# little-little-point-cloud-group/buildingSegment

Hardware: AMD Instinct MI355X
Metric: Mpoints/s segmented (kNN+normal+label) (higher is better)
Workload: dtype int32 coordinates / f64 normals; 1 GPU; urban_50m; points_per_gpu=50000000, k=16, max_nn=50, rg_mode=0, largest_plane=135921, seed_attempts=6951, fallback_queries=0, rg_rounds=25, validation_rejects=0, tie_rows=971975, parallelism=1 GPU, whole path

## Files before the change

### buildingsegment_amd/_lib.py

```python
from __future__ import annotations

import ctypes as C
import os

HERE = os.path.dirname(os.path.abspath(__file__))
LIB_PATH = os.environ.get("BS_LIB_PATH") or os.path.join(HERE, "libbuildingsegment_hip.so")

BS_OK = 0
STATUS = {0: "BS_OK", -1: "BS_ERR_INVALID", -2: "BS_ERR_RANGE", -3: "BS_ERR_NOMEM", -4: "BS_ERR_HIP",
          -5: "BS_ERR_NO_DEVICE", -6: "BS_ERR_INTERNAL", -7: "BS_ERR_UNCERTIFIED"}

EXPORTS = ["bs_api_version", "bs_sizeof_timings", "bs_strerror", "bs_params_default", "bs_create", "bs_destroy", "bs_last_error",
           "bs_set_stream", "bs_get_timings", "bs_knn_normals", "bs_knn_normals_halo", "bs_region_grow", "bs_segment",
           "bs_planes_free", "bs_plane_colors", "bs_knn_normals_dev", "bs_region_grow_dev",
           "bs_segment_dev", "bs_planes_fetch", "bs_shift_to_origin_dev", "bs_plane_colors_dev",
           "bs_selftest_center_div", "bs_selftest_forge_next", "bs_set_audit", "bs_selftest_grow_limits",
           "bs_get_grow_counters", "bs_ingest_dev", "bs_grid_dims", "bs_grid_picture", "bs_grid_picture_dev",
           "bs_cc_hook_dev", "bs_owner_fetch_dev", "bs_labels_from_owner_dev", "bs_remap_rows_dev",
           "bs_plane_seeds_dev", "bs_stream_sync", "bs_comm_rccl", "bs_comm_rccl_unique_id", "bs_comm_rccl_init",
           "bs_comm_rccl_destroy", "bs_comm_local_create", "bs_comm_local_destroy", "bs_segment_sharded",
           "bs_sharded_planes_fetch", "bs_footprints_dev", "bs_footprints", "bs_contours_free",
           "bs_contours_write_obj", "bs_segment_batch", "bs_segment_batch_dev", "bs_batch_planes_fetch",
           "bs_shift_tiles_to_origin_dev", "bs_tile_boxes_dev", "bs_grid_dims_batch", "bs_grid_picture_batch_dev",
           "bs_grid_picture_batch", "bs_footprints_batch_dev", "bs_footprints_batch", "bs_building_map_dev",
           "bs_building_map", "bs_buildings_free", "bs_assign_buildings_dev", "bs_assign_buildings",
           "bs_plane_buildings_dev", "bs_plane_buildings", "bs_buildings_write_obj", "bs_roof_homes", "bs_roofs_dev",
           "bs_roofs", "bs_roofs_free", "bs_roofs_write_obj"]


class Params(C.Structure):
    _fields_ = [("k", C.c_int32), ("max_nn", C.c_int32), ("radius", C.c_double),
                ("th_thickness", C.c_int32), ("th_point_count", C.c_int32), ("cos_th", C.c_double),
                ("cell_size", C.c_int32), ("rg_mode", C.c_int32)]


class Planes(C.Structure):
    _fields_ = [("n_planes", C.c_int32), ("id", C.POINTER(C.c_int32)), ("normal", C.POINTER(C.c_double)),
                ("center", C.POINTER(C.c_int32)), ("offset", C.POINTER(C.c_int64)),
                ("point_idx", C.POINTER(C.c_int32))]


class Timings(C.Structure):
    _fields_ = [("grid_ms", C.c_double), ("knn_ms", C.c_double), ("grow_ms", C.c_double),
                ("total_ms", C.c_double), ("largest_plane", C.c_int64), ("n_seed_attempts", C.c_int64),
                ("n_fallback_queries", C.c_int64), ("rg_rounds", C.c_int64), ("grow_kernel_ms", C.c_double),
                ("grow_kernel_launches", C.c_int64), ("grow_setup_ms", C.c_double),
                ("validation_rejects", C.c_int64), ("forged_seed", C.c_int64), ("forged_refused", C.c_int64),
                ("audit_attempts", C.c_int64), ("audit_mismatches", C.c_int64), ("audit_ms", C.c_double),
                ("tie_rows", C.c_int64), ("rej_v1_robbed", C.c_int64), ("rej_v1_tag", C.c_int64), ("rej_v1_dup", C.c_int64),
                ("rej_v3_state", C.c_int64), ("incons_seed", C.c_int64), ("incons_list", C.c_int64),
                ("incons_log", C.c_int64)]


class GrowLimits(C.Structure):
    _fields_ = [("max_waves", C.c_int64), ("pool_cap", C.c_int64), ("max_pending", C.c_int64), ("pstore_cap", C.c_int64),
                ("retry_max_list", C.c_int32), ("retry_big_round", C.c_int32), ("full_refresh", C.c_int32),
                ("reserved", C.c_int32)]


class GrowCounters(C.Structure):
    _fields_ = [(k, C.c_int64) for k in
                ("rounds", "rounds_capped", "rounds_big", "attempts_nomem", "waves_cut", "max_waves_end", "attempts_stolen",
                 "dropped_pend_count", "dropped_pend_store", "dropped_other", "full_refreshes", "pool_cap")]


API_VERSION = 5


class CommOps(C.Structure):
    _fields_ = [("handle", C.c_void_p), ("rank", C.c_int32), ("world", C.c_int32),
                ("all_reduce", C.c_void_p), ("all_gather", C.c_void_p), ("all_to_all_v", C.c_void_p)]


class ShardInfo(C.Structure):
    _fields_ = [("n_own", C.c_int64), ("n_local", C.c_int64), ("n_grow", C.c_int64), ("components", C.c_int64),
                ("planes_total", C.c_int64), ("cc_iterations", C.c_int32), ("halo_retries", C.c_int32),
                ("halo_mm", C.c_double), ("ms_partition", C.c_double), ("ms_halo", C.c_double), ("ms_knn", C.c_double),
                ("ms_components", C.c_double), ("ms_redistribute", C.c_double), ("ms_grow", C.c_double),
                ("ms_labels", C.c_double)]


class Contours(C.Structure):
    _fields_ = [("n_contours", C.c_int32), ("width", C.c_int32), ("height", C.c_int32),
                ("offset", C.POINTER(C.c_int64)), ("xy", C.POINTER(C.c_int32)), ("area", C.POINTER(C.c_double)),
                ("perimeter", C.POINTER(C.c_double))]


class FootprintInfo(C.Structure):
    _fields_ = [("ms_mask", C.c_double), ("ms_close", C.c_double), ("ms_label", C.c_double), ("ms_trace", C.c_double),
                ("ms_total", C.c_double), ("fg_pixels", C.c_int64), ("border_states", C.c_int64),
                ("components", C.c_int64), ("jump_rounds", C.c_int64)]


class Buildings(C.Structure):
    _fields_ = [("n_buildings", C.c_int32), ("width", C.c_int32), ("height", C.c_int32),
                ("start_xy", C.POINTER(C.c_int32)), ("bbox", C.POINTER(C.c_int32)), ("pixels", C.POINTER(C.c_int64)),
                ("fg_pixels", C.POINTER(C.c_int64)), ("n_points", C.POINTER(C.c_int64)),
                ("n_above", C.POINTER(C.c_int64)), ("z_min", C.POINTER(C.c_int32)), ("z_max", C.POINTER(C.c_int32)),
                ("z_sum", C.POINTER(C.c_int64)), ("ms_label_mask", C.c_double), ("ms_label_fill", C.c_double),
                ("ms_number", C.c_double), ("ms_map", C.c_double), ("ms_assign", C.c_double)]


class Roofs(C.Structure):
    _fields_ = [("n_planes", C.c_int32), ("width", C.c_int32), ("height", C.c_int32), ("fill_rounds", C.c_int32),
                ("seeded_pixels", C.c_int64), ("filled_pixels", C.c_int64), ("unroofed_pixels", C.c_int64),
                ("pixels", C.POINTER(C.c_int64)), ("seed_pixels", C.POINTER(C.c_int64)), ("bbox", C.POINTER(C.c_int32)),
                ("n_support", C.POINTER(C.c_int64)), ("z_min", C.POINTER(C.c_int32)), ("z_max", C.POINTER(C.c_int32)),
                ("z_sum", C.POINTER(C.c_int64)), ("ms_vote", C.c_double), ("ms_fill", C.c_double),
                ("ms_figures", C.c_double), ("ms_height", C.c_double)]


class BsError(RuntimeError):
    def __init__(self, status, detail=""):
        self.status = status
        super().__init__(f"{STATUS.get(status, status)}: {detail}")


_LIB = None


def load():
    global _LIB
    if _LIB is not None:
        return _LIB
    if not os.path.exists(LIB_PATH):
        raise ImportError(f"{LIB_PATH} is missing: build it with `python -m buildingsegment_amd.build` "
                          "(hipcc --offload-arch=gfx950); there is no CPU fallback")
    L = C.CDLL(LIB_PATH)
    L.bs_api_version.restype = C.c_int
    L.bs_sizeof_timings.restype = C.c_int64
    if L.bs_api_version() != API_VERSION or L.bs_sizeof_timings() != C.sizeof(Timings):
        raise ImportError(f"{LIB_PATH} is API version {L.bs_api_version()} (bs_timings: {L.bs_sizeof_timings()} bytes), this "
                          f"loader mirrors version {API_VERSION} ({C.sizeof(Timings)} bytes): rebuild the library")
    vp, ip, dp, lp = C.c_void_p, C.c_void_p, C.c_void_p, C.POINTER(C.c_int64)
    pp = C.POINTER(Params)
    L.bs_api_version.restype = C.c_int
    L.bs_strerror.restype = C.c_char_p
    L.bs_strerror.argtypes = [C.c_int]
    L.bs_params_default.argtypes = [pp]
    L.bs_create.argtypes = [C.c_int, C.POINTER(vp)]
    L.bs_destroy.argtypes = [vp]
    L.bs_destroy.restype = None
    L.bs_last_error.argtypes = [vp]
    L.bs_last_error.restype = C.c_char_p
    L.bs_set_stream.argtypes = [vp, vp]
    L.bs_get_timings.argtypes = [vp, C.POINTER(Timings)]
    L.bs_knn_normals.argtypes = [vp, ip, C.c_int64, pp, ip, dp]
    L.bs_knn_normals_halo.argtypes = [vp, ip, ip, C.c_int64, C.c_int64, pp, ip, dp, C.c_double, lp]
    L.bs_region_grow.argtypes = [vp, ip, dp, ip, C.c_int64, pp, ip, C.POINTER(Planes)]
    L.bs_segment.argtypes = [vp, ip, C.c_int64, pp, ip, dp, ip, C.POINTER(Planes)]
    L.bs_planes_free.argtypes = [C.POINTER(Planes)]
    L.bs_planes_free.restype = None
    L.bs_plane_colors.argtypes = [C.POINTER(Planes), ip, C.c_int64, vp]
    L.bs_knn_normals_dev.argtypes = [vp, ip, ip, C.c_int64, C.c_int64, C.c_int64, pp, ip, dp, C.c_double, lp]
    L.bs_region_grow_dev.argtypes = [vp, ip, dp, ip, C.c_int64, pp, ip]
    L.bs_segment_dev.argtypes = [vp, ip, C.c_int64, pp, ip, dp, ip]
    L.bs_planes_fetch.argtypes = [vp, C.POINTER(Planes)]
    L.bs_shift_to_origin_dev.argtypes = [vp, ip, C.c_int64, ip]
    L.bs_ingest_dev.argtypes = [vp, vp, C.c_int64, C.c_int32, C.c_int32, C.c_int32, C.c_int32, C.c_int32, C.c_double,
                                C.c_int32, ip, ip]
    L.bs_plane_colors_dev.argtypes = [vp, ip, C.c_int32, C.c_int64, vp]
    L.bs_selftest_forge_next.argtypes = [vp, C.c_int]
    L.bs_set_audit.argtypes = [vp, C.c_int]
    L.bs_selftest_grow_limits.argtypes = [vp, C.POINTER(GrowLimits)]
    L.bs_get_grow_counters.argtypes = [vp, C.POINTER(GrowCounters)]
    L.bs_selftest_center_div.argtypes = [vp, ip, vp, ip, C.c_int64]
    L.bs_grid_dims.argtypes = [ip, C.c_int32, ip, ip]
    L.bs_grid_picture.argtypes = [vp, ip, C.c_int64, ip, C.c_int32, C.c_int32, dp, dp]
    L.bs_grid_picture_dev.argtypes = [vp, ip, C.c_int64, ip, C.c_int32, C.c_int32, dp, dp]
    L.bs_cc_hook_dev.argtypes = [vp, ip, ip, C.c_int64, C.c_int32, ip, C.c_int64, lp]
    L.bs_owner_fetch_dev.argtypes = [vp, ip]
    L.bs_plane_seeds_dev.argtypes = [vp, ip, C.c_int64, C.POINTER(C.c_int32)]
    L.bs_stream_sync.argtypes = [vp]
    L.bs_labels_from_owner_dev.argtypes = [vp, ip, C.c_int64, ip, C.c_int32, ip]
    L.bs_remap_rows_dev.argtypes = [vp, ip, C.c_int64, C.c_int32, ip, C.c_int64, ip, C.POINTER(C.c_int32)]
    L.bs_comm_rccl.argtypes = [vp, C.c_int32, C.c_int32, C.POINTER(CommOps)]
    L.bs_comm_rccl_unique_id.argtypes = [C.c_char_p]
    L.bs_comm_rccl_init.argtypes = [vp, C.c_char_p, C.c_int32, C.c_int32, C.POINTER(vp)]
    L.bs_comm_rccl_destroy.argtypes = [vp]
    L.bs_comm_local_create.argtypes = [C.c_int32, C.POINTER(CommOps)]
    L.bs_comm_local_destroy.argtypes = [C.POINTER(CommOps)]
    L.bs_comm_local_destroy.restype = None
    L.bs_segment_sharded.argtypes = [vp, C.POINTER(CommOps), ip, ip, C.c_int64, C.c_int64, pp, C.c_double, ip,
                                     C.POINTER(ShardInfo)]
    L.bs_sharded_planes_fetch.argtypes = [vp, C.POINTER(Planes)]
    cp = C.POINTER(Contours)
    L.bs_footprints_dev.argtypes = [vp, vp, C.c_int32, C.c_int32, C.c_int32, C.c_int32, C.c_int32, vp, cp,
                                    C.POINTER(FootprintInfo)]
    L.bs_footprints.argtypes = [vp, vp, C.c_int32, C.c_int32, C.c_int32, C.c_int32, C.c_int32, vp, cp,
                                C.POINTER(FootprintInfo)]
    L.bs_contours_free.argtypes = [cp]
    L.bs_contours_free.restype = None
    L.bs_contours_write_obj.argtypes = [cp, C.c_char_p]
    L.bs_segment_batch.argtypes = [vp, ip, vp, C.c_int32, pp, ip, dp, ip, C.POINTER(Planes), ip]
    L.bs_segment_batch_dev.argtypes = [vp, ip, vp, C.c_int32, pp, ip, dp, ip]
    L.bs_batch_planes_fetch.argtypes = [vp, C.POINTER(Planes), ip]
    L.bs_shift_tiles_to_origin_dev.argtypes = [vp, ip, vp, C.c_int32, ip]
    L.bs_tile_boxes_dev.argtypes = [vp, ip, vp, C.c_int32, ip]
    L.bs_grid_dims_batch.argtypes = [ip, C.c_int32, C.c_int32, ip, ip, vp]
    L.bs_grid_picture_batch_dev.argtypes = [vp, ip, vp, C.c_int32, ip, C.c_int32, C.c_int32, dp, dp]
    L.bs_grid_picture_batch.argtypes = [vp, ip, vp, C.c_int32, ip, C.c_int32, C.c_int32, dp, dp]
    L.bs_footprints_batch_dev.argtypes = [vp, vp, ip, ip, C.c_int32, C.c_int32, C.c_int32, C.c_int32, vp, cp, ip,
                                          C.POINTER(FootprintInfo)]
    L.bs_footprints_batch.argtypes = [vp, vp, ip, ip, C.c_int32, C.c_int32, C.c_int32, C.c_int32, vp, cp, ip,
                                      C.POINTER(FootprintInfo)]
    bp = C.POINTER(Buildings)
    L.bs_building_map_dev.argtypes = [vp, vp, C.c_int32, C.c_int32, ip, bp]
    L.bs_building_map.argtypes = [vp, vp, C.c_int32, C.c_int32, ip, bp]
    L.bs_buildings_free.argtypes = [bp]
    L.bs_buildings_free.restype = None
    L.bs_assign_buildings_dev.argtypes = [vp, ip, C.c_int64, C.c_int32, C.c_double, ip, C.c_int32, C.c_int32, ip, bp]
    L.bs_assign_buildings.argtypes = [vp, ip, C.c_int64, C.c_int32, C.c_double, ip, C.c_int32, C.c_int32, ip, bp]
    L.bs_plane_buildings_dev.argtypes = [vp, ip, ip, C.c_int64, C.c_int32, C.c_int32, ip, vp, vp, vp]
    L.bs_plane_buildings.argtypes = [vp, ip, ip, C.c_int64, C.c_int32, C.c_int32, ip, vp, vp, vp]
    L.bs_buildings_write_obj.argtypes = [cp, bp, C.c_int32, ip, C.c_double, C.c_double, C.c_double, C.c_char_p]
    rp = C.POINTER(Roofs)
    L.bs_roof_homes.argtypes = [dp, ip, vp, vp, C.c_int32, C.c_double, ip]
    roofs_args = [vp, ip, C.c_int64, C.c_int32, C.c_double, ip, C.c_int32, C.c_int32, ip, C.c_int32, ip, dp, ip, C.c_int32,
                  ip, ip, ip, rp]
    L.bs_roofs_dev.argtypes = roofs_args
    L.bs_roofs.argtypes = roofs_args
    L.bs_roofs_free.argtypes = [rp]
    L.bs_roofs_free.restype = None
    L.bs_roofs_write_obj.argtypes = [ip, ip, C.c_int32, C.c_int32, rp, dp, ip, C.c_int32, ip, C.c_char_p]
    _LIB = L
    return L
```

### buildingsegment_amd/csrc/bs_common.h

```cpp
#pragma once

#include <hip/hip_runtime.h>
#include <stdint.h>

#include <string>
#include <vector>

#include "../../include/bs_api.h"

namespace bs {

struct DevBuf {
  void* p = nullptr;
  size_t cap = 0;
  hipError_t reserve(size_t bytes)
  {
    if (bytes <= cap)
      return hipSuccess;
    if (p)
      (void)hipFree(p);
    p = nullptr;
    cap = 0;
    size_t want = bytes + bytes / 8 + 256;
    hipError_t e = hipMalloc(&p, want);
    if (e == hipSuccess)
      cap = want;
    return e;
  }
  void release()
  {
    if (p)
      (void)hipFree(p);
    p = nullptr;
    cap = 0;
  }
  template <class T>
  T* as() const
  {
    return (T*)p;
  }
};

struct HostBuf {
  void* p = nullptr;
  size_t cap = 0;
  hipError_t reserve(size_t bytes)
  {
    if (bytes <= cap)
      return hipSuccess;
    if (p)
      (void)hipHostFree(p);
    p = nullptr;
    cap = 0;
    size_t want = bytes + bytes / 8 + 256;
    hipError_t e = hipHostMalloc(&p, want, hipHostMallocDefault);
    if (e == hipSuccess)
      cap = want;
    return e;
  }
  void release()
  {
    if (p)
      (void)hipHostFree(p);
    p = nullptr;
    cap = 0;
  }
  template <class T>
  T* as() const
  {
    return (T*)p;
  }
};

struct CellEntry {
  uint64_t key;
  int32_t start;
  int32_t end;
};

struct GridDev {
  int32_t mn[3];
  int32_t dim[3];
  int32_t cell;
  uint32_t hmask;
  const CellEntry* table;
  const int4* spts;
  const int32_t* slocal;
  int64_t n;
};

struct TileDesc {
  int32_t mn[3];
  int32_t dim[3];
};

struct TiledGridDev : GridDev {
  const TileDesc* tiles;
  const int32_t* tile_off;
  int32_t n_tiles;
  int32_t mbits;
};

enum { BT_OFF, BT_BLK, BT_MNMX, BT_DESC, BT_BASE, BT_RECS, BT_LIST, BT_COUNT };

__host__ __device__ inline int32_t tile_of(const int32_t* off, int32_t n_tiles, int64_t i)
{
  int32_t lo = 0, hi = n_tiles - 1;
  while (lo < hi) {
    const int32_t mid = (lo + hi + 1) >> 1;
    if (off[mid] <= i)
      lo = mid;
    else
      hi = mid - 1;
  }
  return lo;
}

__host__ __device__ inline uint64_t spread21(uint64_t v)
{
  v &= 0x1FFFFFull;
  v = (v | (v << 32)) & 0x1F00000000FFFFull;
  v = (v | (v << 16)) & 0x1F0000FF0000FFull;
  v = (v | (v << 8)) & 0x100F00F00F00F00Full;
  v = (v | (v << 4)) & 0x10C30C30C30C30C3ull;
  v = (v | (v << 2)) & 0x1249249249249249ull;
  return v;
}

__host__ __device__ inline uint64_t morton_cell(uint32_t cx, uint32_t cy, uint32_t cz)
{
  return spread21(cx) | (spread21(cy) << 1) | (spread21(cz) << 2);
}

__host__ __device__ inline double* pnorm_of(int32_t* npos, int64_t n, int K)
{
  return reinterpret_cast<double*>(npos + (((int64_t)n * K + 1) & ~(int64_t)1));
}

__host__ __device__ inline uint64_t pack_cell(uint32_t cx, uint32_t cy, uint32_t cz)
{
  return (uint64_t)cx | ((uint64_t)cy << 21) | ((uint64_t)cz << 42);
}

__host__ __device__ inline uint32_t hash_cell(uint64_t k)
{
  k *= 0x9E3779B97F4A7C15ull;
  return (uint32_t)(k >> 32) ^ (uint32_t)k;
}

__device__ inline int64_t xcd_logical_block()
{
  const int64_t b = blockIdx.x, per = gridDim.x >> 3;
  return (b & 7) * per + (b >> 3);
}
inline int xcd_grid(int64_t nblocks) { return (int)((nblocks + 7) & ~(int64_t)7); }

struct PlaneRec {
  double normal[3];
  int64_t list_off;
  int64_t list_n;
  int32_t center[3];
  int32_t id;
  int32_t seed;
  int32_t pad;
};

struct GrowStats {
  int32_t n_planes;
  int32_t error;
  int64_t list_used;
  int64_t seed_attempts;
  int64_t largest;
  int64_t steps;
};

}

struct bs_ctx {
  int device = 0;
  hipStream_t own_stream = nullptr;
  hipStream_t stream = nullptr;
  std::string err;
  bs_timings tm{};
  hipEvent_t ev[10] = {nullptr, nullptr, nullptr, nullptr, nullptr, nullptr, nullptr, nullptr, nullptr, nullptr};

  bs::DevBuf keys_in, keys_out, vals_in, vals_out, cub_tmp, uniq_keys, uniq_cnt, misc;
  bs::DevBuf table, spts, slocal;
  bs::DevBuf fb_list, d_xyz_h, d_neigh_h, d_normals_h, d_plane_h;
  bs::DevBuf seg_neigh, seg_normals;
  bs::DevBuf rg_list, rg_stack, rg_planes, rg_stats, rg_aux, rg_pstore, rg_rec, rg_radj, rg_roff, rg_geo, rg_gs, rg_disp;
  bs::HostBuf rg_hout;
  int64_t rg_n = 0;
  bool rg_valid = false;
  const int32_t* rg_omega = nullptr;
  const int32_t* rg_prio = nullptr;
  const int32_t* rg_seeds = nullptr;
  int32_t rg_nplanes = 0;
  int forge_mode = 0;
  int audit = 0;
  bs_grow_limits lim{0, 0, 0, 0, -1, -1, 0, 0};
  bs_grow_counters gc{};
  hipStream_t side = nullptr;
  hipEvent_t sev[2] = {nullptr, nullptr};
  bs::DevBuf rs_keys_in, rs_keys_out, rs_vals_in, rs_vals_out, rs_cnt, rs_img, rs_tmp;
  int64_t order_n = 0;
  const int32_t* order_xyz = nullptr;
  bs::DevBuf seg_npos;
  bs::DevBuf fp[24];
  bs::DevBuf bd[14];
  bs::DevBuf rf[16];
  bs::DevBuf sh[25];
  std::vector<int32_t> sh_seeds;
  int64_t sh_nloc = 0;
  bool sh_valid = false;
  const int32_t* npos_neigh = nullptr;
  const double* npos_normals = nullptr;
  int npos_k = 0;
  bs::DevBuf bt[bs::BT_COUNT];
  std::vector<int64_t> bt_off;
  bool bt_valid = false;
  bs::DevBuf tile_desc;
};

namespace bs {

int fail(bs_ctx* ctx, int status, const char* what, hipError_t e = hipSuccess);

#define BS_HIP(ctx, call)                                     \
  do {                                                        \
    hipError_t _e = (call);                                   \
    if (_e != hipSuccess)                                     \
      return bs::fail((ctx), BS_ERR_HIP, #call, _e);          \
  } while (0)

int build_grid(bs_ctx* ctx, const int32_t* d_xyz, const int32_t* d_gidx, int64_t n, double radius,
               int k, int cell_hint, GridDev* out);
int build_spatial_order(bs_ctx* ctx, const int32_t* d_xyz, int64_t n);
int bbox_dev(bs_ctx* ctx, const int32_t* d_xyz, int64_t n, int32_t bb[6]);
int tile_bbox_dev(bs_ctx* ctx, const int32_t* d_xyz, const int32_t* d_off, const std::vector<int64_t>& off,
                  int32_t* d_mnmx, std::vector<int32_t>& mnmx);
int build_grid_tiled(bs_ctx* ctx, const int32_t* d_xyz, const int32_t* d_off, const std::vector<int64_t>& off,
                     double radius, int k, int cell_hint, TiledGridDev* out);
int check_tiles(bs_ctx* ctx, const int64_t* off, int32_t n_tiles, int64_t min_pts, int64_t* total);
void launch_tile_shift(bs_ctx* ctx, int32_t* d_xyz, int64_t n, const int32_t* d_off, int32_t n_tiles,
                       const int32_t* d_mnmx);
int launch_knn_normals(bs_ctx* ctx, const GridDev& g, int64_t q_begin, int64_t q_end,
                       const bs_params& p, int32_t* d_neigh, double* d_normals, double cert_radius,
                       int64_t* n_uncertified, int32_t* d_npos = nullptr);
int launch_knn_normals_tiled(bs_ctx* ctx, const TiledGridDev& g, const bs_params& p, int32_t* d_neigh,
                             double* d_normals, int32_t* d_npos);
int region_grow_dev_impl(bs_ctx* ctx, const int32_t* d_xyz, const double* d_normals, const int32_t* d_neigh,
                         int64_t n, const bs_params* p, int32_t* d_plane_idx, bool trusted_neigh);
int check_params(bs_ctx* ctx, const bs_params* p, int64_t n);
int planes_to_host(bs_ctx* ctx, const PlaneRec* d_recs, const int32_t* d_list, int np, int64_t list_used,
                   bs_planes* out);
int launch_region_grow_seq(bs_ctx* ctx, const int32_t* d_xyz, const double* d_normals,
                           const int32_t* d_neigh, int64_t n, const bs_params& p,
                           int32_t* d_plane_idx);
int launch_region_grow_spec(bs_ctx* ctx, const int32_t* d_xyz, const double* d_normals,
                            const int32_t* d_neigh, int64_t n, const bs_params& p,
                            int32_t* d_plane_idx);

}
```

### buildingsegment_amd/csrc/bs_grow_spec.hip

```cpp
#include <hipcub/hipcub.hpp>

#include <algorithm>
#include <cstdio>
#include <cstdlib>
#include <type_traits>
#include <chrono>
#include <vector>

#include "bs_centerdiv.h"
#include "bs_common.h"

namespace bs {

namespace {

constexpr int32_t INF = 0x7fffffff;
constexpr int32_t LOWER_BIT = (int32_t)0x80000000;
constexpr int32_t POS_MASK = 0x7fffffff;
constexpr int MAX_WAVES = 1 << 18;
constexpr int MAX_PENDING = 32768;

enum : int32_t { ST_NONE = 0, ST_DONE = 1, ST_FAILED0 = 2, ST_NOMEM = 3, ST_WATCHDOG = 4, ST_STOLEN = 5 };

struct SpecArgs {
  const int32_t* xyz;
  const double* normals;
  const int32_t* neigh;
  int64_t n;
  int K;
  double th;
  double cos_th;
  int64_t th_count;
  int32_t F;
  int32_t pad;
};

struct PlaneOut {
  double normal[3];
  int64_t list_off;
  int64_t list_n;
  int64_t log_off;
  int64_t log_n;
  int64_t steps;
  int32_t center[3];
  int32_t seed;
  int32_t status;
  int32_t keep;
  int32_t consistent;
  int32_t pad;
  int32_t thief;
  int32_t seed_pos;
  int32_t v3ok;
  int32_t pad4;
  int64_t t_start, t_end;
  int32_t w;
  int32_t pad5;
};

struct KeepForHost {
  __device__ bool operator()(const PlaneOut& o) const { return o.status == ST_DONE || o.status == ST_NOMEM || o.status == ST_WATCHDOG; }
};

struct Pool {
  int32_t* base;
  unsigned long long* top;
  unsigned long long cap;
};

struct Slab {
  int64_t off;
  int32_t cap;
};

__device__ inline int ld_i32(const int32_t* p)
{
  return __hip_atomic_load(p, __ATOMIC_RELAXED, __HIP_MEMORY_SCOPE_AGENT);
}

__device__ inline unsigned long long ballot64(bool pred)
{
  return __builtin_amdgcn_ballot_w64(pred);
}

__device__ inline int readlane_i32(int v, int lane)
{
  return __builtin_amdgcn_readlane(v, __builtin_amdgcn_readfirstlane(lane));
}

__device__ inline double readlane_f64(double v, int lane)
{
  int lo = __double2loint(v), hi = __double2hiint(v);
  lo = readlane_i32(lo, lane);
  hi = readlane_i32(hi, lane);
  return __hiloint2double(hi, lo);
}

__device__ inline bool slab_ensure(const Pool& pool, Slab& s, int32_t used, int64_t need, int lane)
{
  if (need <= s.cap)
    return true;
  if (need > 0x7ffffff0ll)
    return false;
  int64_t ncap = (int64_t)s.cap * 2;
  if (ncap < need)
    ncap = need;
  if (ncap < 256)
    ncap = 256;
  if (ncap > 0x7ffffff0ll)
    ncap = 0x7ffffff0ll;
  ncap = (ncap + 3) & ~(int64_t)3;
  unsigned long long off = 0;
  if (lane == 0)
    off = atomicAdd(pool.top, (unsigned long long)ncap);
  off = ((unsigned long long)(uint32_t)readlane_i32((int)(off >> 32), 0) << 32) |
        (uint32_t)readlane_i32((int)(off & 0xffffffffu), 0);
  if (off + (unsigned long long)ncap > pool.cap)
    return false;
  for (int32_t t0 = 0; t0 < used; t0 += 64) {
    const int32_t t = t0 + lane;
    if (t < used)
      pool.base[off + t] = ld_i32(pool.base + s.off + t);
  }
  s.off = (int64_t)off;
  s.cap = (int32_t)ncap;
  return true;
}

constexpr int RW_PAD = 896;
constexpr int RW_WIN = 256 + 2 * RW_PAD;
constexpr int GW_PAD = 192;
constexpr int GW_WIN = 256 + 2 * GW_PAD;

__global__ __launch_bounds__(256) void static_mask_kernel(SpecArgs a, const int32_t* __restrict__ rows, int row_stride,
                                                          const int4* __restrict__ geo, uint32_t* __restrict__ hmask,
                                                          int32_t* __restrict__ rcnt, uint32_t* __restrict__ lmask)
{
  __shared__ int lcnt[RW_WIN];
  __shared__ int4 lgeo[GW_WIN * 3];
  const int64_t b0 = xcd_logical_block() * (int64_t)blockDim.x;
  const int64_t i = b0 + threadIdx.x;
  const int64_t w0 = b0 > RW_PAD ? b0 - RW_PAD : 0;
  const int64_t g0 = b0 > GW_PAD ? b0 - GW_PAD : 0;
  for (int d = threadIdx.x; d < RW_WIN; d += 256)
    lcnt[d] = 0;
  {
    const int64_t gend = (g0 + GW_WIN < a.n ? g0 + GW_WIN : a.n) - g0;
    const int4* src = geo + 3 * g0;
    for (int64_t t = threadIdx.x; t < 3 * gend; t += 256)
      lgeo[t] = src[t];
  }
  __syncthreads();
  if (i < a.n) {
    const int4* own = lgeo + 3 * (i - g0);
    const int4 s0 = own[0], s1 = own[1], s2 = own[2];
    const double cnx = __hiloint2double(s1.y, s1.x), cny = __hiloint2double(s1.w, s1.z),
                 cnz = __hiloint2double(s2.y, s2.x);
    const int ccx = s0.x, ccy = s0.y, ccz = s0.z;
    const int32_t* row = rows + i * row_stride;
    uint32_t m = 0, lm = 0;
    for (int t = 1; t < a.K; t++) {
      const int32_t c = row[t];
      if (c < 0)
        continue;
      const int64_t gd = (int64_t)c - g0;
      int4 q0, q1, q2;
      if (gd >= 0 && gd < GW_WIN) {
        q0 = lgeo[3 * gd];
        q1 = lgeo[3 * gd + 1];
        q2 = lgeo[3 * gd + 2];
      } else {
        const int4* rc = geo + 3 * (int64_t)c;
        q0 = rc[0];
        q1 = rc[1];
        q2 = rc[2];
      }
      const int dx = (int)((uint32_t)q0.x - (uint32_t)ccx);
      const int dy = (int)((uint32_t)q0.y - (uint32_t)ccy);
      const int dz = (int)((uint32_t)q0.z - (uint32_t)ccz);
      const double dist = __builtin_fabs((double)dx * cnx + (double)dy * cny + (double)dz * cnz);
      const double dt = cnx * __hiloint2double(q1.y, q1.x) + cny * __hiloint2double(q1.w, q1.z) +
                        cnz * __hiloint2double(q2.y, q2.x);
      if (dist <= a.th && dt >= a.cos_th) {
        m |= 1u << (t - 1);
        lm |= (s0.w < q0.w ? 1u : 0u) << (t - 1);
        const int64_t d = (int64_t)c - w0;
        if (d >= 0 && d < RW_WIN)
          atomicAdd(&lcnt[d], 1);
        else
          atomicAdd(&rcnt[c], 1);
      }
    }
    hmask[i] = m;
    lmask[i] = lm;
  }
  __syncthreads();
  for (int d = threadIdx.x; d < RW_WIN; d += 256) {
    const int v = lcnt[d];
    if (v)
      atomicAdd(&rcnt[w0 + d], v);
  }
}

__global__ __launch_bounds__(256) void rev_fill_kernel(const uint32_t* __restrict__ hmask, const int32_t* __restrict__ rows,
                                                       int row_stride, int64_t n, unsigned long long* __restrict__ rcur,
                                                       int32_t* __restrict__ radj, const uint32_t* __restrict__ lmask)
{
  __shared__ int lcnt[RW_WIN];
  __shared__ unsigned long long lbase[RW_WIN];
  const int64_t b0 = xcd_logical_block() * (int64_t)blockDim.x;
  const int64_t i = b0 + threadIdx.x;
  const int64_t w0 = b0 > RW_PAD ? b0 - RW_PAD : 0;
  for (int d = threadIdx.x; d < RW_WIN; d += 256)
    lcnt[d] = 0;
  __syncthreads();
  const uint32_t m0 = i < n ? hmask[i] : 0u;
  const uint32_t lm0 = i < n ? lmask[i] : 0u;
  const int32_t* row = rows + (i < n ? i : 0) * row_stride;
  for (uint32_t m = m0; m;) {
    const int t = __ffs(m) - 1;
    m &= m - 1;
    const int64_t d = (int64_t)row[t + 1] - w0;
    if (d >= 0 && d < RW_WIN)
      atomicAdd(&lcnt[d], 1);
  }
  __syncthreads();
  for (int d = threadIdx.x; d < RW_WIN; d += 256) {
    const int v = lcnt[d];
    if (v) {
      lbase[d] = atomicAdd(&rcur[w0 + d], (unsigned long long)v);
      lcnt[d] = 0;
    }
  }
  __syncthreads();
  for (uint32_t m = m0; m;) {
    const int t = __ffs(m) - 1;
    m &= m - 1;
    const int32_t c = row[t + 1];
    const int64_t d = (int64_t)c - w0;
    if (d >= 0 && d < RW_WIN)
      radj[lbase[d] + (unsigned)atomicAdd(&lcnt[d], 1)] = (int32_t)i | (((lm0 >> t) & 1u) ? LOWER_BIT : 0);
    else
      radj[atomicAdd(&rcur[c], 1ull)] = (int32_t)i | (((lm0 >> t) & 1u) ? LOWER_BIT : 0);
  }
}

constexpr int OWN_TRIP = 16;
constexpr int WL_CAP = 1024;
constexpr int WL_WAVE = 256;

__device__ __forceinline__ void wl_flush(const int* l_buf, int* l_base, int staged, int32_t* list, int* cnt)
{
  if (threadIdx.x == 0)
    *l_base = atomicAdd(cnt, staged);
  __syncthreads();
  const int b = *l_base;
  for (int i = threadIdx.x; i < staged; i += blockDim.x)
    list[b + i] = l_buf[i];
  __syncthreads();
}

__global__ __launch_bounds__(256) void wl_compact_kernel(uint8_t* bdirty, int nb, uint32_t* gflag, int32_t* list, int* cnt)
{
  __shared__ int l_buf[WL_CAP];
  __shared__ int l_base;
  __shared__ int wsum[4];
  int staged = 0;
  for (int j = 0; j < WL_CAP / 256; j++) {
    const int g = blockIdx.x * WL_CAP + j * 256 + threadIdx.x;
    bool add = false;
    if (g < nb && bdirty[g]) {
      bdirty[g] = 0;
      add = atomicExch(gflag + g, 1u) == 0u;
    }
    const unsigned long long am = ballot64(add);
    if ((threadIdx.x & 63) == 0)
      wsum[threadIdx.x >> 6] = __popcll(am);
    __syncthreads();
    int before = __popcll(am & ((1ull << (threadIdx.x & 63)) - 1ull)), total = 0;
    for (int w = 0; w < 4; w++) {
      before += w < (int)(threadIdx.x >> 6) ? wsum[w] : 0;
      total += wsum[w];
    }
    if (add)
      l_buf[staged + before] = g;
    staged += total;
    __syncthreads();
  }
  if (staged)
    wl_flush(l_buf, &l_base, staged, list, cnt);
}

__device__ __forceinline__ void wl_wave_flush(int* wbuf, int& staged, int32_t* list, int* cnt)
{
  const int lane = threadIdx.x & 63;
  __builtin_amdgcn_fence(__ATOMIC_RELEASE, "workgroup");
  __builtin_amdgcn_wave_barrier();
  int b = 0;
  if (lane == 0)
    b = atomicAdd(cnt, staged);
  b = __shfl(b, 0);
  for (int i = lane; i < staged; i += 64)
    list[b + i] = wbuf[i];
  __builtin_amdgcn_fence(__ATOMIC_ACQ_REL, "workgroup");
  __builtin_amdgcn_wave_barrier();
  staged = 0;
}

__device__ __forceinline__ void wl_add(bool want, int32_t g, uint32_t* gflag, int* wbuf, int& staged, int32_t* list, int* cnt)
{
  if (!ballot64(want))
    return;
  const bool added = want && atomicExch(gflag + g, 1u) == 0u;
  const unsigned long long am = ballot64(added);
  if (am == 0)
    return;
  if (added)
    wbuf[staged + __popcll(am & ((1ull << (threadIdx.x & 63)) - 1ull))] = g;
  staged += __popcll(am);
  if (staged > WL_WAVE - 64)
    wl_wave_flush(wbuf, staged, list, cnt);
}

struct PullEval {
  bool flip;
  bool walked;
  uint32_t m0;
};

__device__ __forceinline__ PullEval pull_eval(int64_t c, const uint32_t* __restrict__ hmask, const int32_t* __restrict__ prio,
                                              const uint8_t* __restrict__ ps, const int32_t* __restrict__ base,
                                              const int64_t* __restrict__ roff, const int32_t* __restrict__ radj,
                                              int32_t* __restrict__ omega, uint32_t* occ, int4* rec, int quads,
                                              const int32_t* __restrict__ minr)
{
  int32_t v = base[c];
  const int32_t mr = minr[c];
  const int64_t e0 = roff[c], e1 = roff[c + 1];
  const uint32_t m0 = hmask[c];
  const uint8_t psc = ps[c];
  const int32_t pc = prio[c];
  const uint32_t cbit = 1u << (c & 31);
  const uint32_t oword = __hip_atomic_load(occ + (c >> 5), __ATOMIC_RELAXED, __HIP_MEMORY_SCOPE_AGENT);
  const bool walk = v > mr;
  if (walk) {
    for (int64_t e = e0; e < e1; e += OWN_TRIP) {
      int32_t j[OWN_TRIP];
      uint32_t ow[OWN_TRIP];
      int32_t pj[OWN_TRIP];
#pragma unroll
      for (int i = 0; i < OWN_TRIP; i++)
        j[i] = radj[e + i < e1 ? e + i : e1 - 1] & POS_MASK;
#pragma unroll
      for (int i = 0; i < OWN_TRIP; i++)
        ow[i] = __hip_atomic_load(occ + (j[i] >> 5), __ATOMIC_RELAXED, __HIP_MEMORY_SCOPE_AGENT);
#pragma unroll
      for (int i = 0; i < OWN_TRIP; i++) {
        const bool o = ((ow[i] >> (j[i] & 31)) & 1u) != 0;
        pj[i] = prio[o ? (int64_t)j[i] : c];
        pj[i] = o ? pj[i] : INF;
      }
#pragma unroll
      for (int i = 0; i < OWN_TRIP; i++)
        v = pj[i] < v ? pj[i] : v;
    }
  }
  omega[c] = v;
  reinterpret_cast<int32_t*>(rec + c * quads)[3] = v;
  const bool want = m0 != 0 && !(psc & 1) && v >= pc;
  const bool have = (oword & cbit) != 0;
  if (want != have) {
    if (want)
      __hip_atomic_fetch_or(occ + (c >> 5), cbit, __ATOMIC_RELAXED, __HIP_MEMORY_SCOPE_AGENT);
    else
      __hip_atomic_fetch_and(occ + (c >> 5), ~cbit, __ATOMIC_RELAXED, __HIP_MEMORY_SCOPE_AGENT);
  }
  return {want != have, walk, m0};
}

__device__ __forceinline__ void pull_stats(int* dbg, bool dirty, bool walked)
{
  const int nd = __popcll(ballot64(dirty)), nw = __popcll(ballot64(walked));
  if ((threadIdx.x & 63) == 0 && nd) {
    atomicAdd(dbg + 1, nd);
    atomicAdd(dbg + 2, nw);
  }
}

__global__ void pull_pass_kernel(int64_t n, int K, int sub, const uint32_t* __restrict__ hmask,
                                 const int32_t* __restrict__ prio, const uint8_t* __restrict__ ps,
                                 const int32_t* __restrict__ base, const int64_t* __restrict__ roff,
                                 const int32_t* __restrict__ radj, int32_t* __restrict__ omega, uint32_t* occ,
                                 uint8_t* dirty_cur, uint8_t* dirty_next, uint8_t* bdirty_cur, uint8_t* bdirty_next,
                                 int4* rec, int quads, int* any, const int32_t* __restrict__ minr, const int* prev_any, int* dbg)
{
  if (prev_any && *prev_any == 0)
    return;
  __shared__ unsigned long long sub_mask;
  const int64_t nb256 = (n + 255) >> 8;
  const int64_t g0 = (int64_t)blockIdx.x * sub;
  if (threadIdx.x < 64) {
    const int64_t gidx = g0 + threadIdx.x;
    const bool d = (int)threadIdx.x < sub && gidx < nb256 && bdirty_cur[gidx] != 0;
    if (d)
      bdirty_cur[gidx] = 0;
    const unsigned long long m = ballot64(d);
    if (threadIdx.x == 0)
      sub_mask = m;
  }
  __syncthreads();
  unsigned long long gm = sub_mask;
  if (dbg && threadIdx.x == 0 && gm) {
    atomicAdd(dbg, __popcll(gm));
    atomicMax(dbg + 3, __popcll(gm));
  }
  bool flipped = false;
  while (gm) {
    const int t = __ffsll(gm) - 1;
    gm &= gm - 1;
    const int64_t c = ((g0 + t) << 8) + threadIdx.x;
    const bool d = c < n && dirty_cur[c] != 0;
    PullEval r = {false, false, 0u};
    if (d) {
      dirty_cur[c] = 0;
      r = pull_eval(c, hmask, prio, ps, base, roff, radj, omega, occ, rec, quads, minr);
    }
    if (dbg)
      pull_stats(dbg, d, r.walked);
    if (r.flip) {
      const int32_t* row = reinterpret_cast<const int32_t*>(rec + c * quads + 4);
      uint32_t m = r.m0;
      while (m) {
        const int b = __ffs(m) - 1;
        m &= m - 1;
        const int32_t q = row[b + 1];
        dirty_next[q] = 1;
        bdirty_next[q >> 8] = 1;
      }
      flipped = true;
    }
  }
  if (flipped)
    *any = 1;
}

__global__ __launch_bounds__(256) void pull_list_kernel(int64_t n, int K, const uint32_t* __restrict__ hmask,
                                                        const int32_t* __restrict__ prio, const uint8_t* __restrict__ ps,
                                                        const int32_t* __restrict__ base, const int64_t* __restrict__ roff,
                                                        const int32_t* __restrict__ radj, int32_t* __restrict__ omega,
                                                        uint32_t* occ, uint8_t* dirty_cur, uint8_t* dirty_next,
                                                        const int32_t* __restrict__ list_cur, int32_t* list_next,
                                                        uint32_t* gflag_cur, uint32_t* gflag_next, int* cnt, int s_cur,
                                                        int s_nxt, int s_clr, int4* rec, int quads, int* any,
                                                        const int32_t* __restrict__ minr, int* dbg)
{
  __shared__ int l_buf[4][WL_WAVE];
  int* const wbuf = l_buf[threadIdx.x >> 6];
  const int lane = threadIdx.x & 63;
  const int ncur = cnt[s_cur];
  if (blockIdx.x == 0 && threadIdx.x == 0) {
    cnt[s_clr] = 0;
    if (dbg && ncur) {
      dbg[0] = ncur;
      dbg[3] = (ncur + (int)gridDim.x - 1) / (int)gridDim.x;
    }
  }
  if (ncur == 0)
    return;
  int staged = 0;
  bool flipped = false;
  const int per = (ncur + (int)gridDim.x - 1) / (int)gridDim.x;
  const int i0 = blockIdx.x * per, i1 = min(ncur, i0 + per);
  if (i0 >= i1)
    return;
  int32_t g_next = list_cur[i0];
  for (int idx = i0; idx < i1; idx++) {
    const int32_t g = g_next;
    if (idx + 1 < i1)
      g_next = list_cur[idx + 1];
    const int64_t c = ((int64_t)g << 8) + threadIdx.x;
    if (threadIdx.x == 0)
      gflag_cur[g] = 0;
    const bool d = c < n && dirty_cur[c] != 0;
    PullEval r = {false, false, 0u};
    if (d) {
      dirty_cur[c] = 0;
      r = pull_eval(c, hmask, prio, ps, base, roff, radj, omega, occ, rec, quads, minr);
    }
    if (dbg)
      pull_stats(dbg, d, r.walked);
    if (!ballot64(r.flip))
      continue;
    flipped = flipped || r.flip;
    const int32_t* row = reinterpret_cast<const int32_t*>(rec + (d ? c : 0) * quads + 4);
    for (int b0 = 0; b0 + 1 < K; b0 += OWN_TRIP) {
      int32_t gq[OWN_TRIP];
      uint32_t fl[OWN_TRIP];
      bool rep[OWN_TRIP];
#pragma unroll
      for (int i = 0; i < OWN_TRIP; i++) {
        const int b = b0 + i;
        gq[i] = -1;
        if (r.flip && b + 1 < K && ((r.m0 >> b) & 1u)) {
          const int32_t q = row[b + 1];
          dirty_next[q] = 1;
          gq[i] = q >> 8;
        }
      }
#pragma unroll
      for (int i = 0; i < OWN_TRIP; i++) {
        const int32_t left = __shfl_up(gq[i], 1);
        rep[i] = gq[i] >= 0 && (lane == 0 || left != gq[i]) && (i == 0 || gq[i - 1] != gq[i]);
        fl[i] = __hip_atomic_load(gflag_next + (rep[i] ? gq[i] : g), __ATOMIC_RELAXED, __HIP_MEMORY_SCOPE_AGENT);
      }
#pragma unroll
      for (int i = 0; i < OWN_TRIP; i++)
        wl_add(rep[i] && fl[i] == 0u, gq[i], gflag_next, wbuf, staged, list_next, cnt + s_nxt);
    }
  }
  if (staged)
    wl_wave_flush(wbuf, staged, list_next, cnt + s_nxt);
  if (flipped)
    *any = 1;
}

__global__ void decide_init_kernel(const uint32_t* __restrict__ hmask, int64_t n, uint8_t* __restrict__ st,
                                   uint8_t* __restrict__ bund)
{
  const int64_t c = blockIdx.x * (int64_t)blockDim.x + threadIdx.x;
  const bool maker = c < n && hmask[c] != 0;
  if (c < n)
    st[c] = maker ? 0 : 2;
  const int anym = __syncthreads_or(maker);
  if (threadIdx.x == 0)
    bund[blockIdx.x] = anym ? 1 : 0;
}

__global__ void decide_pass_kernel(int64_t n, int sub, const int32_t* __restrict__ prio,
                                   const int64_t* __restrict__ roff, const int32_t* __restrict__ radj, uint8_t* st,
                                   uint8_t* bund, int* any, const int* prev_any)
{
  if (prev_any && *prev_any == 0)
    return;
  __shared__ unsigned long long sub_mask;
  __shared__ int left[64];
  const int64_t nb256 = (n + 255) >> 8;
  const int64_t g0 = (int64_t)blockIdx.x * sub;
  if (threadIdx.x < 64) {
    const int64_t gidx = g0 + threadIdx.x;
    const bool d = (int)threadIdx.x < sub && gidx < nb256 && bund[gidx] != 0;
    left[threadIdx.x] = 0;
    const unsigned long long m = ballot64(d);
    if (threadIdx.x == 0)
      sub_mask = m;
  }
  __syncthreads();
  unsigned long long gm = sub_mask;
  bool undecided_left = false;
  while (gm) {
    const int t = __ffsll(gm) - 1;
    gm &= gm - 1;
    const int64_t c = ((g0 + t) << 8) + threadIdx.x;
    bool mine_left = false;
    if (c < n && __hip_atomic_load(st + c, __ATOMIC_RELAXED, __HIP_MEMORY_SCOPE_AGENT) == 0) {
      bool lower_occ = false, lower_und = false;
      const int64_t e1 = roff[c + 1];
      for (int64_t e = roff[c]; e < e1; e += 4) {
        int32_t rj[4];
        uint8_t sj[4];
#pragma unroll
        for (int q = 0; q < 4; q++)
          rj[q] = e + q < e1 ? radj[e + q] : 0;
#pragma unroll
        for (int q = 0; q < 4; q++)
          sj[q] = rj[q] < 0 ? __hip_atomic_load(st + (rj[q] & POS_MASK), __ATOMIC_RELAXED, __HIP_MEMORY_SCOPE_AGENT) : (uint8_t)2;
#pragma unroll
        for (int q = 0; q < 4; q++) {
          lower_occ = lower_occ || sj[q] == 1;
          lower_und = lower_und || sj[q] == 0;
        }
      }
      if (lower_occ)
        __hip_atomic_store(st + c, (uint8_t)2, __ATOMIC_RELAXED, __HIP_MEMORY_SCOPE_AGENT);
      else if (!lower_und)
        __hip_atomic_store(st + c, (uint8_t)1, __ATOMIC_RELAXED, __HIP_MEMORY_SCOPE_AGENT);
      else
        mine_left = true;
    }
    if (mine_left)
      left[t] = 1;
    undecided_left = undecided_left || mine_left;
  }
  __syncthreads();
  if (threadIdx.x < 64 && (int)threadIdx.x < sub && g0 + threadIdx.x < nb256)
    bund[g0 + threadIdx.x] = left[threadIdx.x] ? 1 : 0;
  if (undecided_left)
    *any = 1;
}

__global__ void decide_finish_kernel(int64_t n, const int32_t* __restrict__ prio, const int64_t* __restrict__ roff,
                                     const int32_t* __restrict__ radj, const uint8_t* __restrict__ st,
                                     int32_t* __restrict__ omega, uint32_t* __restrict__ occ, int4* rec, int quads,
                                     int32_t* __restrict__ minr)
{
  const int64_t c = blockIdx.x * (int64_t)blockDim.x + threadIdx.x;
  bool oc = false;
  if (c < n) {
    int32_t v = INF, vall = INF;
    const int64_t e1 = roff[c + 1];
    for (int64_t e = roff[c]; e < e1; e++) {
      const int32_t j = radj[e] & POS_MASK;
      const int32_t pj = prio[j];
      vall = pj < vall ? pj : vall;
      if (st[j] == 1)
        v = pj < v ? pj : v;
    }
    minr[c] = vall;
    omega[c] = v;
    reinterpret_cast<int32_t*>(rec + c * quads)[3] = v;
    oc = st[c] == 1;
  }
  const unsigned long long m = ballot64(oc);
  const int lane = threadIdx.x & 63;
  const int64_t w0 = (c - lane) >> 5;
  if (lane == 0 && (c - lane) < n)
    occ[w0] = (uint32_t)m;
  if (lane == 32 && (c - lane + 32) < n)
    occ[w0 + 1] = (uint32_t)(m >> 32);
}

__global__ void verify_fixpoint_kernel(int64_t n, const uint32_t* __restrict__ hmask, const int32_t* __restrict__ prio,
                                       const uint8_t* __restrict__ ps,
                                       const int32_t* __restrict__ base, const int64_t* __restrict__ roff,
                                       const int32_t* __restrict__ radj, const int32_t* __restrict__ omega,
                                       const uint32_t* __restrict__ occ, int* nbad)
{
  const int64_t c = blockIdx.x * (int64_t)blockDim.x + threadIdx.x;
  if (c >= n)
    return;
  int32_t v = base[c];
  for (int64_t e = roff[c]; e < roff[c + 1]; e++) {
    const int32_t j = radj[e] & POS_MASK;
    const bool oj = hmask[j] != 0 && !(ps[j] & 1) && omega[j] >= prio[j];
    if (oj && prio[j] < v)
      v = prio[j];
  }
  const bool oc = hmask[c] != 0 && !(ps[c] & 1) && omega[c] >= prio[c];
  if (v != omega[c] || (oc ? 1u : 0u) != ((occ[c >> 5] >> (c & 31)) & 1u))
    atomicAdd(nbad, 1);
}

__global__ void seed_flags_kernel(const uint32_t* __restrict__ hmask, int64_t n, int K, uint8_t* __restrict__ ps)
{
  const int64_t i = blockIdx.x * (int64_t)blockDim.x + threadIdx.x;
  const uint32_t full = (K - 1 >= 32) ? 0xffffffffu : ((1u << (K - 1)) - 1u);
  if (i < n)
    ps[i] = hmask[i] == full ? 0 : 2;
}

__global__ void cand_flag_kernel(const int4* __restrict__ rec, int quads, int K,
                                 int64_t n, int32_t F, const int32_t* __restrict__ prio, const uint8_t* __restrict__ ps,
                                 int all_seeds, const int32_t* __restrict__ omega, int32_t* min_idx,
                                 unsigned long long* __restrict__ cand_out, int32_t* cand_count, uint8_t* __restrict__ bcand,
                                 int sub)
{
  __shared__ unsigned long long sub_mask;
  const int64_t nb256 = (n + 255) >> 8;
  const int64_t g0 = (int64_t)blockIdx.x * sub;
  if (threadIdx.x < 64) {
    const int64_t gidx = g0 + threadIdx.x;
    const bool live = (int)threadIdx.x < sub && gidx < nb256 && bcand[gidx] != 0;
    const unsigned long long m = ballot64(live);
    if (threadIdx.x == 0)
      sub_mask = m;
  }
  __syncthreads();
  unsigned long long gm = sub_mask;
  while (gm) {
    const int t = __ffsll(gm) - 1;
    gm &= gm - 1;
    const int64_t i = ((g0 + t) << 8) + threadIdx.x;
    bool c = false, alive = false;
    const uint8_t f = i < n ? ps[i] : (uint8_t)2;
    int32_t pi = 0;
    if (!(f & 2)) {
      pi = prio[i];
      const int32_t oi = omega[i];
      alive = !(oi < F);
      if (pi >= F && oi >= pi && (all_seeds || !(f & 1))) {
        c = true;
        const int32_t* row = reinterpret_cast<const int32_t*>(rec + i * quads + 4);
        for (int u = 1; u < K; u += OWN_TRIP) {
          int32_t nb[OWN_TRIP];
          int32_t ov[OWN_TRIP];
#pragma unroll
          for (int q = 0; q < OWN_TRIP; q++)
            nb[q] = row[u + q < K ? u + q : K - 1];
#pragma unroll
          for (int q = 0; q < OWN_TRIP; q++)
            ov[q] = omega[nb[q]];
#pragma unroll
          for (int q = 0; q < OWN_TRIP; q++)
            c = c && ov[q] >= pi;
        }
      }
    }
    const int any_alive = __syncthreads_or(alive);
    if (threadIdx.x == 0 && !any_alive)
      bcand[g0 + t] = 0;
    if (c && min_idx)
      atomicMin(min_idx, pi);
    if (c && cand_out)
      cand_out[atomicAdd(cand_count, 1)] = ((unsigned long long)(uint32_t)pi << 32) | (uint32_t)i;
  }
}

template <int KC>
struct RecLayout {
  static constexpr int QUADS = 4 + KC / 4;
};

__device__ inline int32_t* rec_tag(int4* rec, int quads, int64_t i)
{
  return reinterpret_cast<int32_t*>(rec + i * quads + 2) + 2;
}

__global__ void invert_order_kernel(const int32_t* __restrict__ order, int64_t n, int32_t* __restrict__ pos)
{
  const int64_t s = blockIdx.x * (int64_t)blockDim.x + threadIdx.x;
  if (s < n)
    pos[order[s]] = (int32_t)s;
}

template <int KC>
__global__ __launch_bounds__(256) void build_records_kernel(SpecArgs a, const int32_t* __restrict__ order, const int32_t* __restrict__ pos,
                                     const int32_t* __restrict__ npos, int4* __restrict__ rec, int32_t* __restrict__ prio,
                                     int4* __restrict__ geo, const int4* __restrict__ spts, const double* __restrict__ pnorm)
{
  constexpr int Q = RecLayout<KC>::QUADS;
  __shared__ int4 srec[256 * Q];
  __shared__ int4 sgeo[256 * 3];
  const int64_t b0 = blockIdx.x * (int64_t)blockDim.x;
  const int64_t s = b0 + threadIdx.x;
  if (s < a.n) {
  int64_t i;
  int px, py, pz;
  if (spts) {
    const int4 p = spts[s];
    px = p.x;
    py = p.y;
    pz = p.z;
    i = p.w;
  } else {
    i = order ? order[s] : s;
    px = a.xyz[3 * i];
    py = a.xyz[3 * i + 1];
    pz = a.xyz[3 * i + 2];
  }
  int4* r = srec + threadIdx.x * Q;
  const double* nsrc = pnorm ? pnorm + 3 * s : a.normals + 3 * i;
  const double nx = nsrc[0], ny = nsrc[1], nz = nsrc[2];
  r[0] = make_int4(px, py, pz, INF);
  r[1] = make_int4(__double2loint(nx), __double2hiint(nx), __double2loint(ny), __double2hiint(ny));
  r[2] = make_int4(__double2loint(nz), __double2hiint(nz), INF, 0);
  r[3] = make_int4(0, 0, 0, 0);
  sgeo[3 * threadIdx.x] = make_int4(px, py, pz, (int32_t)i);
  sgeo[3 * threadIdx.x + 1] = r[1];
  sgeo[3 * threadIdx.x + 2] = r[2];
  prio[s] = (int32_t)i;
  int row[KC];
#pragma unroll
  for (int j = 0; j < KC; j++) {
    int v = 0;
    if (j < a.K) {
      if (npos) {
        v = npos[s * a.K + j];
      } else {
        v = a.neigh[i * a.K + j];
        v = pos ? pos[v] : v;
      }
    }
    row[j] = v;
  }
  if (!npos) {
#pragma unroll
    for (int j = 2; j < KC; j++) {
      bool rep = false;
#pragma unroll
      for (int t = 1; t < j; t++)
        rep = rep || (j < a.K && row[t] == row[j]);
      row[j] = rep ? -1 : row[j];
    }
  }
#pragma unroll
  for (int j = 0; j < KC; j += 4)
    r[4 + j / 4] = make_int4(row[j], row[j + 1], row[j + 2], row[j + 3]);
  }
  __syncthreads();
  const int64_t nv = a.n - b0 < 256 ? a.n - b0 : 256;
  int4* rout = rec + b0 * Q;
  for (int t = threadIdx.x; t < nv * Q; t += 256)
    rout[t] = srec[t];
  int4* gout = geo + 3 * b0;
  for (int t = threadIdx.x; t < nv * 3; t += 256)
    gout[t] = sgeo[t];
}

__global__ void refresh_records_kernel(const int32_t* __restrict__ omega, int4* __restrict__ rec, int quads, int64_t n)
{
  const int64_t i = blockIdx.x * (int64_t)blockDim.x + threadIdx.x;
  if (i >= n)
    return;
  reinterpret_cast<int32_t*>(rec + i * quads)[3] = omega[i];
  *rec_tag(rec, quads, i) = INF;
}

__device__ __forceinline__ void plane_state_lanes(int lane, double Sx, double Sy, double Sz, uint32_t Cx, uint32_t Cy, uint32_t Cz,
                                                  uint32_t n, double& cnx, double& cny, double& cnz, int& ccx, int& ccy, int& ccz)
{
  const double nrm = __builtin_sqrt((Sx * Sx) + (Sy * Sy) + (Sz * Sz));
  const double Sv = lane == 0 ? Sx : (lane == 1 ? Sy : Sz);
  const double qn = Sv / nrm;
  const CenterDiv cd = center_div_prepare(n);
  const int32_t Cv = lane == 0 ? (int32_t)Cx : (lane == 1 ? (int32_t)Cy : (int32_t)Cz);
  const int32_t qc = center_div(Cv, cd);
  cnx = readlane_f64(qn, 0);
  cny = readlane_f64(qn, 1);
  cnz = readlane_f64(qn, 2);
  ccx = readlane_i32(qc, 0);
  ccy = readlane_i32(qc, 1);
  ccz = readlane_i32(qc, 2);
}

constexpr int LDS_STACK = 256;
constexpr int LDS_REFILL = 128;
constexpr int MAX_RETRY_LONG = 3;
constexpr int MAX_RETRY = 12;
constexpr int RETRY_MAX_LIST = 16384;

template <int KC>
__global__ __launch_bounds__(64) void grow_spec_kernel(SpecArgs a, const unsigned long long* __restrict__ cand, int ncand,
                                                       int4* rec, int32_t* dead, Pool pool,
                                                       PlaneOut* __restrict__ out, int64_t step_cap, int retry_max_list,
                                                       const uint32_t* __restrict__ order)
{
  __shared__ __attribute__((aligned(16))) int lds_stack[LDS_STACK * KC];
  constexpr int Q = RecLayout<KC>::QUADS;
  constexpr int NG = 64 / KC;
  if ((int)blockIdx.x >= ncand)
    return;
  const int w = order ? (int)(order[blockIdx.x] & (MAX_WAVES - 1)) : (int)blockIdx.x;
  const int lane = threadIdx.x;
  const int g = lane / KC, j = lane % KC;
  const unsigned long long gmask0 = (KC == 32) ? 0xffffffffull : 0xffffull;
  const int K = a.K, nc = K - 1;
  const bool act = j < nc;
  const int64_t t_start = (int64_t)wall_clock64();
  const int32_t seed = (int32_t)(cand[w] >> 32);
  const int32_t seed_s = (int32_t)(uint32_t)cand[w];
  Slab list = {0, 0}, stack = {0, 0}, log = {0, 0};
  int long_tries = 0;
  int ln = 1, sp = 0, lds_lo = 0, logn = 0;
  uint32_t iters = 0;
  const uint32_t iter_cap = step_cap > 0xFFFFFFF0ll ? 0xFFFFFFF0u : (uint32_t)step_cap;
  int status = ST_DONE;
  bool pendv = false;
  const int32_t* vptr = dead;
  bool need_state = false;
  const int4* srec = rec + (int64_t)seed_s * Q;
  const int4 s0 = srec[0], s1 = srec[1], s2 = srec[2];
  double cnx, cny, cnz, Sx, Sy, Sz;
  int ccx, ccy, ccz;
  uint32_t Cx, Cy, Cz;
  unsigned long long d_am = 0;
  double d_mx = 0, d_my = 0, d_mz = 0;
  int d_px = 0, d_py = 0, d_pz = 0;
  auto update_state = [&]() {
    unsigned long long mm = d_am;
    while (mm) {
      const int l = __ffsll(mm) - 1;
      mm &= mm - 1;
      Sx += readlane_f64(d_mx, l);
      Sy += readlane_f64(d_my, l);
      Sz += readlane_f64(d_mz, l);
      Cx += (uint32_t)readlane_i32(d_px, l);
      Cy += (uint32_t)readlane_i32(d_py, l);
      Cz += (uint32_t)readlane_i32(d_pz, l);
    }
    plane_state_lanes(lane, Sx, Sy, Sz, Cx, Cy, Cz, (uint32_t)ln, cnx, cny, cnz, ccx, ccy, ccz);
    need_state = false;
  };
  const bool have_mem = slab_ensure(pool, list, 0, 256, lane) && slab_ensure(pool, stack, 0, 32 * (int64_t)KC, lane) &&
                        slab_ensure(pool, log, 0, 256, lane);
  for (int attempt = 0;; attempt++) {
  status = ST_DONE;
  pendv = false;
  ln = 1;
  sp = 0;
  lds_lo = 0;
  logn = 0;
  cnx = __hiloint2double(s1.y, s1.x);
  cny = __hiloint2double(s1.w, s1.z);
  cnz = __hiloint2double(s2.y, s2.x);
  ccx = s0.x;
  ccy = s0.y;
  ccz = s0.z;
  Sx = 0.0 + cnx;
  Sy = 0.0 + cny;
  Sz = 0.0 + cnz;
  Cx = (uint32_t)ccx;
  Cy = (uint32_t)ccy;
  Cz = (uint32_t)ccz;
  if (!have_mem) {
    status = ST_NOMEM;
  } else {
    if (lane == 0)
      pool.base[list.off] = seed_s;
    if (lane < KC)
      lds_stack[lane] = reinterpret_cast<const int32_t*>(srec + 4)[lane];
    sp = 1;
    bool depth0 = true;
    int stack_entries = stack.cap / KC;
    need_state = false;
    __builtin_amdgcn_s_waitcnt(0x0F70);
    auto step = [&](auto mode) -> int {
      if (__builtin_expect(sp == 0, 0))
        return 2;
      if (__builtin_expect(++iters > iter_cap, 0)) {
        status = ST_WATCHDOG;
        return 2;
      }
      const int e = sp - 1 - g;
      const bool valid = e >= 0;
      const int ngv = (sp < NG) ? sp : NG;
      const int need_lo = (sp - NG > 0) ? sp - NG : 0;
      if (__builtin_expect(need_lo < lds_lo, 0)) {
        const int new_lo = lds_lo > LDS_REFILL ? lds_lo - LDS_REFILL : 0;
        const int nw = (lds_lo - new_lo) * KC;
        for (int t = lane; t < nw; t += 64) {
          const int ee = new_lo + t / KC;
          lds_stack[(ee & (LDS_STACK - 1)) * KC + (t % KC)] = ld_i32(pool.base + stack.off + (int64_t)new_lo * KC + t);
        }
        lds_lo = new_lo;
      }
      int cand_id = 0;
      if (valid && act)
        cand_id = lds_stack[(e & (LDS_STACK - 1)) * KC + j + 1];
      const bool live = cand_id >= 0;
      cand_id = live ? cand_id : 0;
      const int killed = ld_i32(dead + seed);
      const int vt = ld_i32(pendv ? vptr : dead + seed);
      int own = 0, tg = INF, px = 0, py = 0, pz = 0;
      double mx = 0, my = 0, mz = 0;
      int row[KC];
      {
        const int4* r = rec + (int64_t)cand_id * Q;
        const int4 q0 = r[0], q1 = r[1], q2 = r[2];
        tg = ld_i32(reinterpret_cast<const int32_t*>(r + 2) + 2);
        px = q0.x;
        py = q0.y;
        pz = q0.z;
        own = q0.w;
        mx = __hiloint2double(q1.y, q1.x);
        my = __hiloint2double(q1.w, q1.z);
        mz = __hiloint2double(q2.y, q2.x);
#pragma unroll
        for (int t = 0; t < KC; t += 4) {
          const int4 v = r[4 + t / 4];
          row[t] = v.x;
          row[t + 1] = v.y;
          row[t + 2] = v.z;
          row[t + 3] = v.w;
        }
      }
      if constexpr (decltype(mode)::value == 1)
        update_state();
      else if constexpr (decltype(mode)::value == 2) {
        if (__builtin_expect(need_state, 1))
          update_state();
      }
      bool geo = false;
      if (valid && act && live && tg != seed) {
        const int dx = (int)((uint32_t)px - (uint32_t)ccx);
        const int dy = (int)((uint32_t)py - (uint32_t)ccy);
        const int dz = (int)((uint32_t)pz - (uint32_t)ccz);
        const double dist = __builtin_fabs((double)dx * cnx + (double)dy * cny + (double)dz * cnz);
        const double dt = cnx * mx + cny * my + cnz * mz;
        geo = dist <= a.th && dt >= a.cos_th;
      }
      const bool lost = pendv && vt != seed;
      pendv = false;
      if (__builtin_expect(killed || ballot64(lost), 0)) {
        status = ST_STOLEN;
        return 2;
      }
      bool assume = geo && own < seed && !(own < a.F);
      const bool contender = geo && !(own < seed);
      const unsigned long long cm = ballot64(contender);
      unsigned long long am = 0;
      int gstar = -1;
      bool ok = false;
      if (__builtin_expect(cm != 0, 1)) {
        const int g1 = (__ffsll(cm) - 1) / KC;
        const unsigned long long gm1 = gmask0 << (g1 * KC);
        const unsigned long long earlier = ballot64(contender && tg < seed);
        if (__builtin_expect((earlier & gm1) == 0, 1)) {
          ok = contender && g == g1;
          if (ok) {
            int32_t* tp = rec_tag(rec, Q, cand_id);
            __hip_atomic_fetch_min(tp, seed, __ATOMIC_RELAXED, __HIP_MEMORY_SCOPE_AGENT);
            if (tg != INF)
              __hip_atomic_store(dead + tg, seed + 1, __ATOMIC_RELAXED, __HIP_MEMORY_SCOPE_AGENT);
            vptr = tp;
            pendv = true;
          }
          am = cm & gm1;
          gstar = g1;
        } else {
        for (int gg = g1; gg < ngv; gg++) {
          const unsigned long long gm = gmask0 << (gg * KC);
          if (cm & gm) {
            if (g == gg && contender) {
              int32_t* tp = rec_tag(rec, Q, cand_id);
              int cur_tag = tg;
              bool mine = false;
              for (int tries = 0; tries < 8 && !ok && !assume && !mine; tries++) {
                if (cur_tag < seed) {
                  if (ld_i32(dead + cur_tag) < 0) {
                    const int old = atomicCAS(tp, cur_tag, seed);
                    if (old == cur_tag)
                      ok = true;
                    else
                      cur_tag = old;
                  } else {
                    assume = true;
                  }
                } else if (cur_tag == seed) {
                  mine = true;
                } else {
                  const int old = atomicMin(tp, seed);
                  if (old > seed) {
                    if (old != INF)
                      __hip_atomic_store(dead + old, seed + 1, __ATOMIC_RELAXED, __HIP_MEMORY_SCOPE_AGENT);
                    ok = true;
                  } else if (old == seed) {
                    mine = true;
                  } else {
                    cur_tag = old;
                  }
                }
              }
              if (!ok && !mine)
                assume = true;
            }
            am = ballot64(ok);
            if (am) {
              gstar = gg;
              break;
            }
          }
        }
        }
      }
      const int last = gstar >= 0 ? gstar : ngv - 1;
      const unsigned long long lm = ballot64(assume && g <= last);
      const int lcnt = __popcll(lm);
      if (__builtin_expect(lcnt != 0, 0)) {
        if (!slab_ensure(pool, log, logn, logn + lcnt, lane)) {
          status = ST_NOMEM;
          return 2;
        }
        if (assume && g <= last)
          pool.base[log.off + logn + __popcll(lm & ((1ull << lane) - 1ull))] = cand_id;
        logn += lcnt;
      }
      const int cnt = __popcll(am);
      if (__builtin_expect(depth0 && cnt < nc, 0)) {
        status = ST_FAILED0;
        return 2;
      }
      depth0 = false;
      sp -= last + 1;
      if (sp < lds_lo)
        lds_lo = sp;
      if (__builtin_expect(gstar < 0, 0))
        return 0;
      if (__builtin_expect(ln + cnt > list.cap || sp + cnt > stack_entries, 0)) {
        if (!slab_ensure(pool, list, ln, ln + cnt, lane) ||
            !slab_ensure(pool, stack, sp > 0x7ffffff0 / KC ? 0x7ffffff0 : sp * KC, (int64_t)(sp + cnt) * KC, lane)) {
          status = ST_NOMEM;
          return 2;
        }
        stack_entries = stack.cap / KC;
      }
      const int rank = __popcll(am & ((1ull << lane) - 1ull));
      if (ok)
        pool.base[list.off + ln + rank] = cand_id;
      d_am = am;
      d_mx = mx;
      d_my = my;
      d_mz = mz;
      d_px = px;
      d_py = py;
      d_pz = pz;
      ln += cnt;
      need_state = true;
      if (ok) {
        const int pe = sp + (cnt - 1 - rank);
        int4* lslot = reinterpret_cast<int4*>(lds_stack + (pe & (LDS_STACK - 1)) * KC);
        row[0] = cand_id;
#pragma unroll
        for (int t = 0; t < KC; t += 4)
          lslot[t / 4] = make_int4(row[t], row[t + 1], row[t + 2], row[t + 3]);
        if (rank > 0) {
          int4* slot = reinterpret_cast<int4*>(pool.base + stack.off + (int64_t)pe * KC);
#pragma unroll
          for (int t = 0; t < KC; t += 4)
            slot[t / 4] = make_int4(row[t], row[t + 1], row[t + 2], row[t + 3]);
        }
      }
      sp += cnt;
      if (__builtin_expect(sp - lds_lo > LDS_STACK, 0))
        lds_lo = sp - LDS_STACK;
      return 1;
    };
    if constexpr (KC == 32) {
      int r = step(std::integral_constant<int, 0>{});
      while (r == 0)
        r = step(std::integral_constant<int, 0>{});
      while (r == 1) {
        r = step(std::integral_constant<int, 1>{});
        while (r == 0)
          r = step(std::integral_constant<int, 0>{});
      }
    } else {
      while (step(std::integral_constant<int, 2>{}) != 2) {
      }
    }
  }
  if (need_state)
    update_state();
  if (status == ST_DONE) {
    const bool lost = pendv && ld_i32(vptr) != seed;
    if (ballot64(lost))
      status = ST_STOLEN;
  }
  bool seed_taken = false;
  if (status == ST_STOLEN) {
    const int t0 = ld_i32(rec_tag(rec, Q, seed_s));
    seed_taken = t0 < seed && ld_i32(dead + t0) >= 0;
  }
  if (status != ST_STOLEN || seed_taken || attempt >= MAX_RETRY || ln > retry_max_list ||
      (ln > RETRY_MAX_LIST && ++long_tries > MAX_RETRY_LONG))
    break;
  for (int t = 1 + lane; t < ln; t += 64)
    atomicCAS(rec_tag(rec, Q, ld_i32(pool.base + list.off + t)), seed, INF);
  __hip_atomic_store(dead + seed, 0, __ATOMIC_RELAXED, __HIP_MEMORY_SCOPE_AGENT);
  }
  if (lane == 0 && status == ST_STOLEN) {
    const int t = ld_i32(dead + seed);
    __hip_atomic_store(dead + seed, t > 0 ? -t : (t == 0 ? -0x40000000 : t), __ATOMIC_RELAXED, __HIP_MEMORY_SCOPE_AGENT);
  }
  if (lane == 0) {
    PlaneOut o;
    o.normal[0] = cnx;
    o.normal[1] = cny;
    o.normal[2] = cnz;
    o.center[0] = ccx;
    o.center[1] = ccy;
    o.center[2] = ccz;
    o.list_off = list.off;
    o.list_n = ln;
    o.log_off = log.off;
    o.log_n = logn;
    o.steps = iters;
    o.seed = seed;
    o.status = status;
    o.keep = (status == ST_DONE && ln > a.th_count) ? 1 : 0;
    o.consistent = 0;
    o.pad = 0;
    const int dflag = ld_i32(dead + seed);
    o.thief = (dflag < 0 ? -dflag : dflag) - 1;
    o.seed_pos = seed_s;
    o.v3ok = 1;
    o.pad4 = 0;
    o.t_start = t_start;
    o.t_end = (int64_t)wall_clock64();
    o.w = w;
    o.pad5 = (int32_t)((__builtin_amdgcn_s_getreg((15 << 11) | (0 << 6) | 4) & 0xffff) |
                       ((__builtin_amdgcn_s_getreg((3 << 11) | (0 << 6) | 20) & 0xf) << 16));
    out[w] = o;
  }
}

constexpr int LBUF = 256;
#ifdef BS_PROBE
__device__ unsigned long long g_prof2[32];
#define PROBE(i)                    \
  do {                              \
    const long long _t = clock64(); \
    pacc[i] += _t - tlast;          \
    tlast = _t;                     \
  } while (0)
#else
#define PROBE(i) \
  do {           \
  } while (0)
#endif

typedef int v4i __attribute__((ext_vector_type(4)));

#ifdef BS_PROBE
__device__ unsigned long long g_exit2[16];
#define EXIT_COUNT(i) (nexit[i]++)
#else
#define EXIT_COUNT(i) \
  do {                \
  } while (0)
#endif
constexpr int LOGB = 128;

template <int KC>
__global__ __launch_bounds__(64) void grow_spec2_kernel(SpecArgs a, const unsigned long long* __restrict__ cand, int ncand,
                                                        int4* rec, int32_t* dead, Pool pool,
                                                        PlaneOut* __restrict__ out, int64_t step_cap, int retry_max_list,
                                                        const uint32_t* __restrict__ order)
{
  static_assert(KC == 16, "k > 16 runs on grow_spec_kernel");
  __shared__ int logbuf[LOGB];
  __shared__ __attribute__((aligned(16))) int lds_stack[LDS_STACK * KC];
  __shared__ int lbuf[LBUF];
  constexpr int Q = RecLayout<KC>::QUADS;
  constexpr int NG = 64 / KC;
  constexpr int CH = KC / 4;
  if ((int)blockIdx.x >= ncand)
    return;
  const int w = order ? (int)(order[blockIdx.x] & (MAX_WAVES - 1)) : (int)blockIdx.x;
  const int lane = threadIdx.x;
  const int g = lane / KC, j = lane % KC;
  const unsigned long long gmask0 = 0xffffull;
  const int K = a.K, nc = K - 1;
  const bool act = j < nc;
  const int64_t t_start = (int64_t)wall_clock64();
  const int32_t seed = (int32_t)(cand[w] >> 32);
  const int32_t seed_s = (int32_t)(uint32_t)cand[w];
  Slab list = {0, 0}, stack = {0, 0}, log = {0, 0};
  int long_tries = 0;
  int ln = 1, lflushed = 0, sp = 0, lds_lo = 0, logn = 0;
  int lgflushed = 0;
  uint32_t iters = 0;
  const uint32_t iter_cap = step_cap > 0xFFFFFFF0ll ? 0xFFFFFFF0u : (uint32_t)step_cap;
  int status = ST_DONE;
  bool pendv = false;
  const int32_t* vptr = dead;
  bool need_state = false;
  const int4* srec = rec + (int64_t)seed_s * Q;
  const int4 s0 = srec[0], s1 = srec[1], s2 = srec[2];
  double cnx, cny, cnz, Sx, Sy, Sz;
  int ccx, ccy, ccz;
  uint32_t Cx, Cy, Cz;
  unsigned long long d_am = 0;
  double d_mx = 0, d_my = 0, d_mz = 0;
  int d_px = 0, d_py = 0, d_pz = 0;
  const bool have_mem = slab_ensure(pool, list, 0, 256, lane) && slab_ensure(pool, stack, 0, 32 * (int64_t)KC, lane) &&
                        slab_ensure(pool, log, 0, 256, lane);
  auto flush_list = [&](int upto) -> bool {
    if (upto <= lflushed)
      return true;
    if (!slab_ensure(pool, list, lflushed, upto, lane))
      return false;
    for (int t0 = lflushed; t0 < upto; t0 += 64) {
      const int t = t0 + lane;
      if (t < upto)
        pool.base[list.off + t] = lbuf[t & (LBUF - 1)];
    }
    lflushed = upto;
    return true;
  };
  auto flush_log = [&](int upto) -> bool {
    if (upto <= lgflushed)
      return true;
    if (!slab_ensure(pool, log, lgflushed, upto, lane))
      return false;
    for (int t0 = lgflushed; t0 < upto; t0 += 64) {
      const int t = t0 + lane;
      if (t < upto)
        pool.base[log.off + t] = logbuf[t & (LOGB - 1)];
    }
    lgflushed = upto;
    return true;
  };
  for (int attempt = 0;; attempt++) {
    status = ST_DONE;
    pendv = false;
    ln = 1;
    lflushed = 0;
    sp = 0;
    lds_lo = 0;
    logn = 0;
    lgflushed = 0;
    cnx = __hiloint2double(s1.y, s1.x);
    cny = __hiloint2double(s1.w, s1.z);
    cnz = __hiloint2double(s2.y, s2.x);
    ccx = s0.x;
    ccy = s0.y;
    ccz = s0.z;
    Sx = 0.0 + cnx;
    Sy = 0.0 + cny;
    Sz = 0.0 + cnz;
    Cx = (uint32_t)ccx;
    Cy = (uint32_t)ccy;
    Cz = (uint32_t)ccz;
    need_state = false;
    if (!have_mem) {
      status = ST_NOMEM;
    } else {
      if (lane == 0)
        lbuf[0] = seed_s;
      if (lane < KC)
        lds_stack[lane] = reinterpret_cast<const int32_t*>(srec + 4)[lane];
      sp = 1;
      bool depth0 = true;
      __builtin_amdgcn_s_waitcnt(0x0F70);
#ifdef BS_PROBE
      long long pacc[12] = {0};
      long long ncalls = 0, nexp = 0;
      long long tlast = clock64();
      long long nexit[11] = {0};
#endif
      struct Ev {
        int cand_id, px, py, pz, own, tg;
        double mx, my, mz;
        bool geo, valid;
        int ngv;
        int killed_v, vt;
        bool lost_any;
        v4i rows[CH];
      };
      auto eval = [&](Ev& E) {
        E.ngv = (sp < NG) ? sp : NG;
        const int e = sp - 1 - g;
        E.valid = e >= 0;
        {
          const int v = lds_stack[(e & (LDS_STACK - 1)) * KC + ((j + 1) & (KC - 1))];
          E.valid = E.valid && v >= 0;
          E.cand_id = (E.valid && act) ? v : 0;
        }
        v4i q0, q1, q2;
        {
          const int32_t* kp = dead + seed;
          const int32_t* vp = pendv ? vptr : dead + seed;
          const int4* r = rec + (int64_t)E.cand_id * Q;
          asm volatile("global_load_dwordx4 %0, %5, off\n\t"
                       "global_load_dwordx4 %1, %5, off offset:16\n\t"
                       "global_load_dwordx4 %2, %5, off offset:32 sc1\n\t"
                       "global_load_dword %3, %6, off sc1\n\t"
                       "global_load_dword %4, %7, off sc1"
                       : "=&v"(q0), "=&v"(q1), "=&v"(q2), "=&v"(E.killed_v), "=&v"(E.vt)
                       : "v"(r), "v"(kp), "v"(vp)
                       : "memory");
#pragma unroll
          for (int t = 0; t < CH; t++) {
            const int4* rp = r + 4 + t;
            asm volatile("global_load_dwordx4 %0, %1, off" : "=&v"(E.rows[t]) : "v"(rp) : "memory");
          }
        }
        PROBE(0);
        if (__builtin_expect(need_state, 1)) {
          unsigned long long mm = d_am;
          while (mm) {
            const int l = __ffsll(mm) - 1;
            mm &= mm - 1;
            Sx += readlane_f64(d_mx, l);
            Sy += readlane_f64(d_my, l);
            Sz += readlane_f64(d_mz, l);
            Cx += (uint32_t)readlane_i32(d_px, l);
            Cy += (uint32_t)readlane_i32(d_py, l);
            Cz += (uint32_t)readlane_i32(d_pz, l);
          }
          plane_state_lanes(lane, Sx, Sy, Sz, Cx, Cy, Cz, (uint32_t)ln, cnx, cny, cnz, ccx, ccy, ccz);
          need_state = false;
        }
        PROBE(1);
        asm volatile("s_waitcnt vmcnt(6)" : "+v"(q0), "+v"(q1), "+v"(q2)::"memory");
        PROBE(2);
        E.px = q0.x;
        E.py = q0.y;
        E.pz = q0.z;
        E.own = q0.w;
        E.tg = q2.z;
        E.mx = __hiloint2double(q1.y, q1.x);
        E.my = __hiloint2double(q1.w, q1.z);
        E.mz = __hiloint2double(q2.y, q2.x);
        {
          const int dx = (int)((uint32_t)E.px - (uint32_t)ccx);
          const int dy = (int)((uint32_t)E.py - (uint32_t)ccy);
          const int dz = (int)((uint32_t)E.pz - (uint32_t)ccz);
          const double dist = __builtin_fabs((double)dx * cnx + (double)dy * cny + (double)dz * cnz);
          const double dt = cnx * E.mx + cny * E.my + cnz * E.mz;
          const bool okd = dist <= a.th, okn = dt >= a.cos_th;
          E.geo = E.valid & act & (E.tg != seed) & okd & okn;
        }
      };
      auto rows_wait = [&](Ev& E) {
        asm volatile("s_waitcnt vmcnt(0)"
                     : "+v"(E.rows[0]), "+v"(E.rows[1]), "+v"(E.rows[2]), "+v"(E.rows[3]), "+v"(E.killed_v), "+v"(E.vt)::"memory");
        const bool lost = pendv && E.vt != seed;
        E.lost_any = __builtin_amdgcn_readfirstlane(E.killed_v) != 0 || ballot64(lost) != 0;
      };
      auto expand = [&](const Ev& E, bool ok, unsigned long long am, int gstar, int cnt) {
        const int rank = __popcll(am & ((1ull << lane) - 1ull));
        if (ok)
          lbuf[(ln + rank) & (LBUF - 1)] = E.cand_id;
        d_am = am;
        d_mx = E.mx;
        d_my = E.my;
        d_mz = E.mz;
        d_px = E.px;
        d_py = E.py;
        d_pz = E.pz;
        ln += cnt;
        need_state = true;
        PROBE(7);
        if (ok) {
          const int pe = sp + (cnt - 1 - rank);
          v4i* lslot = reinterpret_cast<v4i*>(lds_stack + (pe & (LDS_STACK - 1)) * KC);
#pragma unroll
          for (int t = 0; t < CH; t++) {
            v4i v = E.rows[t];
            if (t == 0)
              v.x = E.cand_id;
            lslot[t] = v;
          }
        }
        (void)gstar;
        sp += cnt;
      };
      auto step_complete = [&]() -> int {
        if (__builtin_expect(sp == 0, 0))
          return 2;
        EXIT_COUNT(10);
        if (__builtin_expect(++iters > iter_cap, 0)) {
          status = ST_WATCHDOG;
          return 2;
        }
        const int need_lo = (sp - NG > 0) ? sp - NG : 0;
        if (__builtin_expect(need_lo < lds_lo, 0)) {
          const int new_lo = lds_lo > LDS_REFILL ? lds_lo - LDS_REFILL : 0;
          const int nw = (lds_lo - new_lo) * KC;
          for (int t0 = 0; t0 < nw; t0 += 64) {
            const int t = t0 + lane;
            const int ee = new_lo + t / KC;
            if (t < nw)
              lds_stack[(ee & (LDS_STACK - 1)) * KC + (t % KC)] = ld_i32(pool.base + stack.off + (int64_t)new_lo * KC + t);
          }
          lds_lo = new_lo;
        }
        Ev E;
        eval(E);
        rows_wait(E);
        pendv = false;
        if (__builtin_expect(E.lost_any, 0)) {
          status = ST_STOLEN;
          return 2;
        }
        bool assume = E.geo && E.own < seed && !(E.own < a.F);
        const bool contender = E.geo && !(E.own < seed);
        const unsigned long long cm = ballot64(contender);
        unsigned long long am = 0;
        int gstar = -1;
        bool ok = false;
        const int cand_id = E.cand_id, tg = E.tg, ngv = E.ngv;
        if (cm != 0) {
          const int g1 = (__ffsll(cm) - 1) / KC;
          const unsigned long long gm1 = gmask0 << (g1 * KC);
          const unsigned long long earlier = ballot64(contender && tg < seed);
          if ((earlier & gm1) == 0) {
            ok = contender && g == g1;
            if (ok) {
              int32_t* tp = rec_tag(rec, Q, cand_id);
              __hip_atomic_fetch_min(tp, seed, __ATOMIC_RELAXED, __HIP_MEMORY_SCOPE_AGENT);
              if (tg != INF)
                __hip_atomic_store(dead + tg, seed + 1, __ATOMIC_RELAXED, __HIP_MEMORY_SCOPE_AGENT);
              vptr = tp;
              pendv = true;
            }
            am = cm & gm1;
            gstar = g1;
          } else {
            for (int gg = g1; gg < ngv; gg++) {
              const unsigned long long gm = gmask0 << (gg * KC);
              if (cm & gm) {
                if (g == gg && contender) {
                  int32_t* tp = rec_tag(rec, Q, cand_id);
                  int cur_tag = tg;
                  bool mine = false;
                  for (int tries = 0; tries < 8 && !ok && !assume && !mine; tries++) {
                    if (cur_tag < seed) {
                      if (ld_i32(dead + cur_tag) < 0) {
                        const int old = atomicCAS(tp, cur_tag, seed);
                        if (old == cur_tag)
                          ok = true;
                        else
                          cur_tag = old;
                      } else {
                        assume = true;
                      }
                    } else if (cur_tag == seed) {
                      mine = true;
                    } else {
                      const int old = atomicMin(tp, seed);
                      if (old > seed) {
                        if (old != INF)
                          __hip_atomic_store(dead + old, seed + 1, __ATOMIC_RELAXED, __HIP_MEMORY_SCOPE_AGENT);
                        ok = true;
                      } else if (old == seed) {
                        mine = true;
                      } else {
                        cur_tag = old;
                      }
                    }
                  }
                  if (!ok && !mine)
                    assume = true;
                }
                am = ballot64(ok);
                if (am) {
                  gstar = gg;
                  break;
                }
              }
            }
          }
        }
        const int last = gstar >= 0 ? gstar : ngv - 1;
        const unsigned long long lm = ballot64(assume && g <= last);
        if (lm != 0) {
          const int lcnt = __popcll(lm);
          if (logn + lcnt - lgflushed > LOGB && !flush_log(logn)) {
            status = ST_NOMEM;
            return 2;
          }
          if (assume && g <= last)
            logbuf[(logn + __popcll(lm & ((1ull << lane) - 1ull))) & (LOGB - 1)] = cand_id;
          logn += lcnt;
        }
        const int cnt = __popcll(am);
        if (depth0 && cnt < nc) {
          status = ST_FAILED0;
          return 2;
        }
        depth0 = false;
        sp -= last + 1;
        if (gstar < 0)
          return 0;
        if (ln + cnt - lflushed > LBUF) {
          if (!flush_list(ln)) {
            status = ST_NOMEM;
            return 2;
          }
        }
        if (sp + cnt - lds_lo > LDS_STACK) {
          const int upto = lds_lo + LDS_STACK / 2;
          if (!slab_ensure(pool, stack, lds_lo > 0x7ffffff0 / KC ? 0x7ffffff0 : lds_lo * KC, (int64_t)upto * KC, lane)) {
            status = ST_NOMEM;
            return 2;
          }
          for (int t0 = 0; t0 < (LDS_STACK / 2) * KC; t0 += 64) {
            const int t = t0 + lane;
            const int ee = lds_lo + t / KC;
            pool.base[stack.off + (int64_t)lds_lo * KC + t] = lds_stack[(ee & (LDS_STACK - 1)) * KC + (t % KC)];
          }
          lds_lo = upto;
        }
        expand(E, ok, am, gstar, cnt);
        return 0;
      };
      auto uniform_state = [&]() {
        sp = __builtin_amdgcn_readfirstlane(sp);
        ln = __builtin_amdgcn_readfirstlane(ln);
        lds_lo = __builtin_amdgcn_readfirstlane(lds_lo);
        lflushed = __builtin_amdgcn_readfirstlane(lflushed);
        logn = __builtin_amdgcn_readfirstlane(logn);
        iters = (uint32_t)__builtin_amdgcn_readfirstlane((int)iters);
        status = __builtin_amdgcn_readfirstlane(status);
        d_am = ((unsigned long long)(uint32_t)__builtin_amdgcn_readfirstlane((int)(d_am >> 32)) << 32) |
               (uint32_t)__builtin_amdgcn_readfirstlane((int)(uint32_t)d_am);
      };
      for (;;) {
        const int r = __builtin_amdgcn_readfirstlane(step_complete());
        uniform_state();
        if (r == 2)
          break;
        bool leave = false;
        __builtin_amdgcn_s_waitcnt(0x0F70);
        for (;;) {
          if (__builtin_expect(sp == 0, 0)) {
            EXIT_COUNT(0);
            leave = true;
            break;
          }
          PROBE(9);
#ifdef BS_PROBE
          ncalls++;
#endif
          if (__builtin_expect(iters >= iter_cap, 0)) {
            EXIT_COUNT(1);
            break;
          }
          if (__builtin_expect(((sp - NG > 0) ? sp - NG : 0) < lds_lo, 0)) {
            EXIT_COUNT(2);
            break;
          }
          Ev E;
          eval(E);
          const bool assume = E.geo && E.own < seed && !(E.own < a.F);
          const bool contender = E.geo && !(E.own < seed);
          const unsigned long long cm = ballot64(contender);
          PROBE(3);
          int gstar = -1, cnt = 0;
          unsigned long long am = 0, lm = 0;
          bool slow = false;
          if (__builtin_expect(cm != 0, 1)) {
            gstar = (__ffsll(cm) - 1) / KC;
            const unsigned long long gm1 = gmask0 << (gstar * KC);
            am = cm & gm1;
            cnt = __popcll(am);
            lm = ballot64(assume && g <= gstar);
            slow = (ballot64(contender && E.tg < seed) & gm1) != 0 || ln + cnt - lflushed > LBUF ||
                   sp - (gstar + 1) + cnt - lds_lo > LDS_STACK;
          } else {
            lm = ballot64(assume);
          }
          slow = slow || logn + __popcll(lm) - lgflushed > LOGB;
          rows_wait(E);
          if (__builtin_expect(E.lost_any, 0)) {
            EXIT_COUNT(3);
            pendv = false;
            status = ST_STOLEN;
            leave = true;
            break;
          }
          if (__builtin_expect(slow, 0)) {
#ifdef BS_PROBE
            const unsigned long long gmp = gstar >= 0 ? gmask0 << (gstar * KC) : 0;
            if ((ballot64(contender && E.tg < seed) & gmp) != 0)
              EXIT_COUNT(4);
            else if (ln + cnt - lflushed > LBUF)
              EXIT_COUNT(6);
            else if (gstar >= 0 && sp - (gstar + 1) + cnt - lds_lo > LDS_STACK)
              EXIT_COUNT(7);
            else
              EXIT_COUNT(8);
#endif
            break;
          }
          EXIT_COUNT(9);
          iters++;
          pendv = false;
          if (lm != 0) {
            if (assume && (gstar < 0 || g <= gstar))
              logbuf[(logn + __popcll(lm & ((1ull << lane) - 1ull))) & (LOGB - 1)] = E.cand_id;
            logn += __popcll(lm);
          }
          const bool ok = contender && g == gstar;
          if (ok) {
            int32_t* tp = rec_tag(rec, Q, E.cand_id);
            asm volatile("global_atomic_smin %0, %1, off" ::"v"(tp), "v"(seed) : "memory");
            if (E.tg != INF) {
              int32_t* dp = dead + E.tg;
              const int thief = seed + 1;
              asm volatile("global_store_dword %0, %1, off sc1" ::"v"(dp), "v"(thief) : "memory");
            }
            vptr = tp;
            pendv = true;
          }
          PROBE(4);
          sp -= (gstar >= 0 ? gstar : E.ngv - 1) + 1;
          PROBE(5);
          if (gstar >= 0) {
#ifdef BS_PROBE
            nexp++;
#endif
            PROBE(6);
            expand(E, ok, am, gstar, cnt);
            PROBE(8);
          }
        }
        if (leave)
          break;
      }
#ifdef BS_PROBE
      if (lane == 0 && ln > 20000) {
        for (int i = 0; i < 10; i++)
          atomicAdd(&g_prof2[i], (unsigned long long)pacc[i]);
        atomicAdd(&g_prof2[10], (unsigned long long)ncalls);
        atomicAdd(&g_prof2[11], (unsigned long long)nexp);
      }
      if (lane == 0)
        for (int i = 0; i < 11; i++)
          if (nexit[i])
            atomicAdd(&g_exit2[i], (unsigned long long)nexit[i]);
#endif
    }
    if (need_state) {
      unsigned long long mm = d_am;
      while (mm) {
        const int l = __ffsll(mm) - 1;
        mm &= mm - 1;
        Sx += readlane_f64(d_mx, l);
        Sy += readlane_f64(d_my, l);
        Sz += readlane_f64(d_mz, l);
        Cx += (uint32_t)readlane_i32(d_px, l);
        Cy += (uint32_t)readlane_i32(d_py, l);
        Cz += (uint32_t)readlane_i32(d_pz, l);
      }
      plane_state_lanes(lane, Sx, Sy, Sz, Cx, Cy, Cz, (uint32_t)ln, cnx, cny, cnz, ccx, ccy, ccz);
      need_state = false;
    }
    if (have_mem && status != ST_NOMEM && !flush_list(ln))
      status = ST_NOMEM;
    if (have_mem && status != ST_NOMEM && !flush_log(logn))
      status = ST_NOMEM;
    if (status == ST_DONE) {
      const bool lost = pendv && ld_i32(vptr) != seed;
      if (ballot64(lost))
        status = ST_STOLEN;
    }
    bool seed_taken = false;
    if (status == ST_STOLEN) {
      const int t0 = __builtin_amdgcn_readfirstlane(ld_i32(rec_tag(rec, Q, seed_s)));
      seed_taken = t0 < seed && __builtin_amdgcn_readfirstlane(ld_i32(dead + (t0 < seed ? t0 : seed))) >= 0;
    }
    if (status != ST_STOLEN || seed_taken || attempt >= MAX_RETRY || ln > retry_max_list ||
        (ln > RETRY_MAX_LIST && ++long_tries > MAX_RETRY_LONG))
      break;
    for (int t0 = 1; t0 < ln; t0 += 64) {
      const int t = t0 + lane;
      if (t < ln)
        atomicCAS(rec_tag(rec, Q, ld_i32(pool.base + list.off + t)), seed, INF);
    }
    __hip_atomic_store(dead + seed, 0, __ATOMIC_RELAXED, __HIP_MEMORY_SCOPE_AGENT);
  }
  if (lane == 0 && status == ST_STOLEN) {
    const int t = ld_i32(dead + seed);
    __hip_atomic_store(dead + seed, t > 0 ? -t : (t == 0 ? -0x40000000 : t), __ATOMIC_RELAXED, __HIP_MEMORY_SCOPE_AGENT);
  }
  if (lane == 0) {
    PlaneOut o;
    o.normal[0] = cnx;
    o.normal[1] = cny;
    o.normal[2] = cnz;
    o.center[0] = ccx;
    o.center[1] = ccy;
    o.center[2] = ccz;
    o.list_off = list.off;
    o.list_n = ln;
    o.log_off = log.off;
    o.log_n = logn;
    o.steps = iters;
    o.seed = seed;
    o.status = status;
    o.keep = (status == ST_DONE && ln > a.th_count) ? 1 : 0;
    o.consistent = 0;
    o.pad = 0;
    const int dflag = ld_i32(dead + seed);
    o.thief = (dflag < 0 ? -dflag : dflag) - 1;
    o.seed_pos = seed_s;
    o.v3ok = 1;
    o.pad4 = 0;
    o.t_start = t_start;
    o.t_end = (int64_t)wall_clock64();
    o.w = w;
    o.pad5 = (int32_t)((__builtin_amdgcn_s_getreg((15 << 11) | (0 << 6) | 4) & 0xffff) |
                       ((__builtin_amdgcn_s_getreg((3 << 11) | (0 << 6) | 20) & 0xf) << 16));
    out[w] = o;
  }
}

constexpr int VT = 1024;

__global__ __launch_bounds__(VT) void validate1_kernel(PlaneOut* out, int ncand, const int32_t* __restrict__ pool,
                                                       int4* rec, int quads, const int32_t* __restrict__ dead, int64_t n,
                                                       int32_t* __restrict__ vmark, int32_t round_key, int* rejects)
{
  const int w = blockIdx.x;
  if (w >= ncand || out[w].status != ST_DONE)
    return;
  const PlaneOut o = out[w];
  const bool robbed = dead[o.seed] != 0 || o.list_n > n + 1;
  bool bad = robbed, bad_tag = false, bad_dup = false;
  const int32_t key = round_key + w + 1;
  for (int64_t t = 1 + threadIdx.x; t < o.list_n; t += VT) {
    const int32_t p = pool[o.list_off + t];
    const bool tagbad = *rec_tag(rec, quads, p) != o.seed;
    bad_tag = bad_tag || tagbad;
    const bool dup = atomicExch(&vmark[p], key) == key;
    if (dup)
      atomicAdd(rejects, 1);
    bad_dup = bad_dup || dup;
    bad = bad || tagbad || dup;
  }
  const int b = __syncthreads_or(bad);
  const int bt = __syncthreads_or(bad_tag), bd = __syncthreads_or(bad_dup);
  if (threadIdx.x == 0) {
    if (b) {
      atomicAdd(rejects + (robbed ? 8 : (bd ? 10 : 9)), 1);
      (void)bt;
      out[w].status = ST_STOLEN;
      if (rejects[1] == o.seed + 1)
        rejects[2] = 1;
    } else {
      out[w].pad = 1;
    }
  }
}

constexpr int V3T = 256;
constexpr int V3C = 1024;
__global__ __launch_bounds__(V3T) void validate3_kernel(PlaneOut* out, int ncand, const int32_t* __restrict__ pool,
                                                        const int4* __restrict__ rec, int quads, int* rejects)
{
  __shared__ double sn[2][V3C][3];
  __shared__ uint32_t sc[V3T / 64][3];
  const int w = blockIdx.x;
  if (w >= ncand || out[w].status != ST_DONE || out[w].pad != 1)
    return;
  const PlaneOut o = out[w];
  const int tid = threadIdx.x, lane = tid & 63, wv = tid >> 6;
  uint32_t cx = 0, cy = 0, cz = 0;
  double rr[V3C / V3T][3];
  auto fetch = [&](int64_t c) {
#pragma unroll
    for (int u = 0; u < V3C / V3T; u++) {
      const int64_t t = c * V3C + u * V3T + tid;
      if (t < o.list_n) {
        const int4* r = rec + (int64_t)pool[o.list_off + t] * quads;
        const int4 q0 = r[0], q1 = r[1], q2 = r[2];
        cx += (uint32_t)q0.x;
        cy += (uint32_t)q0.y;
        cz += (uint32_t)q0.z;
        rr[u][0] = __hiloint2double(q1.y, q1.x);
        rr[u][1] = __hiloint2double(q1.w, q1.z);
        rr[u][2] = __hiloint2double(q2.y, q2.x);
      }
    }
  };
  auto put = [&](int buf) {
#pragma unroll
    for (int u = 0; u < V3C / V3T; u++) {
      sn[buf][u * V3T + tid][0] = rr[u][0];
      sn[buf][u * V3T + tid][1] = rr[u][1];
      sn[buf][u * V3T + tid][2] = rr[u][2];
    }
  };
  const int64_t chunks = (o.list_n + V3C - 1) / V3C;
  double acc = 0.0;
  fetch(0);
  put(0);
  __syncthreads();
  for (int64_t c = 0; c < chunks; c++) {
    const int buf = (int)(c & 1);
    if (c + 1 < chunks)
      fetch(c + 1);
    if (wv == 0) {
      const int cnt = (int)((o.list_n - c * V3C < V3C) ? o.list_n - c * V3C : V3C);
      const double* src = &sn[buf][0][lane % 3];
      int e0 = 0;
      if (cnt == V3C) {
        double va[16], vb[16];
#pragma unroll
        for (int i = 0; i < 16; i++)
          va[i] = src[i * 3];
        for (int b = 0; b < V3C / 16; b += 2) {
#pragma unroll
          for (int i = 0; i < 16; i++)
            vb[i] = src[((b + 1) * 16 + i) * 3];
          __builtin_amdgcn_sched_barrier(0);
#pragma unroll
          for (int i = 0; i < 16; i++)
            acc += va[i];
          __builtin_amdgcn_sched_barrier(0);
          if (b + 2 < V3C / 16) {
#pragma unroll
            for (int i = 0; i < 16; i++)
              va[i] = src[((b + 2) * 16 + i) * 3];
          }
          __builtin_amdgcn_sched_barrier(0);
#pragma unroll
          for (int i = 0; i < 16; i++)
            acc += vb[i];
          __builtin_amdgcn_sched_barrier(0);
        }
        e0 = V3C;
      }
      for (; e0 < cnt; e0++)
        acc += src[e0 * 3];
    }
    if (c + 1 < chunks)
      put(buf ^ 1);
    __syncthreads();
  }
  for (int off = 32; off > 0; off >>= 1) {
    cx += (uint32_t)__shfl_xor((int)cx, off);
    cy += (uint32_t)__shfl_xor((int)cy, off);
    cz += (uint32_t)__shfl_xor((int)cz, off);
  }
  if (lane == 0) {
    sc[wv][0] = cx;
    sc[wv][1] = cy;
    sc[wv][2] = cz;
  }
  const double Sx = __shfl(acc, 0), Sy = __shfl(acc, 1), Sz = __shfl(acc, 2);
  __syncthreads();
  if (tid == 0) {
    uint32_t Cx = 0, Cy = 0, Cz = 0;
    for (int k = 0; k < V3T / 64; k++) {
      Cx += sc[k][0];
      Cy += sc[k][1];
      Cz += sc[k][2];
    }
    bool same;
    if (o.list_n == 1) {
      same = true;
    } else {
      const double nrm = __builtin_sqrt((Sx * Sx) + (Sy * Sy) + (Sz * Sz));
      const double nx = Sx / nrm, ny = Sy / nrm, nz = Sz / nrm;
      const CenterDiv cd = center_div_prepare((uint32_t)o.list_n);
      const int32_t ex = center_div((int32_t)Cx, cd), ey = center_div((int32_t)Cy, cd), ez = center_div((int32_t)Cz, cd);
      same = __double_as_longlong(nx) == __double_as_longlong(o.normal[0]) &&
             __double_as_longlong(ny) == __double_as_longlong(o.normal[1]) &&
             __double_as_longlong(nz) == __double_as_longlong(o.normal[2]) && ex == o.center[0] && ey == o.center[1] &&
             ez == o.center[2];
    }
    if (!same) {
      out[w].v3ok = 0;
      atomicAdd(rejects, 1);
      atomicAdd(rejects + 11, 1);
      if (rejects[1] == o.seed + 1)
        rejects[2] = 1;
    }
  }
}

__global__ void forge_kernel(PlaneOut* out, int ncand, int32_t* pool, int mode, int* forged)
{
  if (blockIdx.x != 0 || threadIdx.x != 0)
    return;
  for (int w = 0; w < ncand; w++) {
    const int64_t ln = out[w].list_n;
    if (out[w].status != ST_DONE || ln < 64 || (ln & (ln - 1)) == 0)
      continue;
    if (mode == 1) {
      pool[out[w].list_off + ln] = pool[out[w].list_off + 20];
      out[w].list_n = ln + 1;
    } else
      out[w].normal[2] = __longlong_as_double(__double_as_longlong(out[w].normal[2]) ^ 1ll);
    *forged = out[w].seed + 1;
    return;
  }
}

__global__ __launch_bounds__(VT) void plane_apply_kernel(const PlaneOut* __restrict__ arr, int cnt,
                                                         const int32_t* __restrict__ pool, int32_t* base,
                                                         uint8_t* ps, uint8_t* dirty, uint8_t* bdirty, int32_t* omega,
                                                         const uint32_t* __restrict__ occ, int4* rec, int quads)
{
  const int w = blockIdx.x;
  if (w >= cnt)
    return;
  const PlaneOut o = arr[w];
  if (o.status != ST_DONE || o.pad == 0)
    return;
  const bool ins = o.pad == 1;
  if (threadIdx.x == 0) {
    ps[o.seed_pos] = ins ? 1 : 0;
    dirty[o.seed_pos] = 1;
    bdirty[o.seed_pos >> 8] = 1;
  }
  if (!o.keep)
    return;
  for (int64_t t = 1 + threadIdx.x; t < o.list_n; t += VT) {
    const int32_t p = pool[o.list_off + t];
    if (ins) {
      atomicMin(&base[p], o.seed);
      const int32_t old = atomicMin(&omega[p], o.seed);
      if (old > o.seed)
        reinterpret_cast<int32_t*>(rec + (int64_t)p * quads)[3] = o.seed;
      if ((occ[p >> 5] >> (p & 31)) & 1u) {
        dirty[p] = 1;
        bdirty[p >> 8] = 1;
      }
    } else {
      atomicCAS(&base[p], o.seed, INF);
      dirty[p] = 1;
      bdirty[p >> 8] = 1;
    }
  }
}

__global__ __launch_bounds__(VT) void reset_tags_kernel(const PlaneOut* __restrict__ out, int ncand,
                                                        const int32_t* __restrict__ pool, int4* rec, int quads, int K)
{
  const int w = blockIdx.x;
  if (w >= ncand)
    return;
  const PlaneOut o = out[w];
  for (int64_t t = 1 + threadIdx.x; t < o.list_n; t += VT) {
    int32_t* tg = rec_tag(rec, quads, pool[o.list_off + t]);
    if (*tg == o.seed)
      *tg = INF;
  }
  if (threadIdx.x >= 1 && threadIdx.x < K) {
    int32_t* tg = rec_tag(rec, quads, reinterpret_cast<const int32_t*>(rec + (int64_t)o.seed_pos * quads + 4)[threadIdx.x]);
    if (*tg == o.seed)
      *tg = INF;
  }
}

__global__ void verify_records_kernel(const int32_t* __restrict__ omega, int4* rec, int quads, int64_t n, int* nbad)
{
  const int64_t i = blockIdx.x * (int64_t)blockDim.x + threadIdx.x;
  if (i >= n)
    return;
  if (reinterpret_cast<int32_t*>(rec + i * quads)[3] != omega[i] || *rec_tag(rec, quads, i) != INF)
    atomicAdd(nbad, 1);
}

__global__ __launch_bounds__(VT) void validate2_kernel(PlaneOut* out, int ncand, const int32_t* __restrict__ pool,
                                                       const int32_t* __restrict__ omega, const int4* __restrict__ rec,
                                                       int quads, int K)
{
  const int w = blockIdx.x;
  if (w >= ncand || out[w].status != ST_DONE)
    return;
  const PlaneOut o = out[w];
  const int32_t s = o.seed;
  bool bad1 = false, bad2 = false, bad3 = false;
  if (threadIdx.x == 0)
    bad1 = omega[o.seed_pos] < s;
  if (threadIdx.x >= 1 && threadIdx.x < K)
    bad1 = omega[reinterpret_cast<const int32_t*>(rec + (int64_t)o.seed_pos * quads + 4)[threadIdx.x]] < s;
  for (int64_t t = 1 + threadIdx.x; t < o.list_n; t += VT)
    bad2 = bad2 || omega[pool[o.list_off + t]] < s;
  for (int64_t t = threadIdx.x; t < o.log_n; t += VT)
    bad3 = bad3 || !(omega[pool[o.log_off + t]] < s);
  const int b = __syncthreads_or((bad1 ? 1 : 0) | (bad2 ? 2 : 0) | (bad3 ? 4 : 0));
  const int b2 = __syncthreads_or(bad2), b3 = __syncthreads_or(bad3);
  if (threadIdx.x == 0) {
    out[w].consistent = b ? 0 : 1;
    out[w].pad4 = (b && !b2 && !b3 ? 1 : 0) | (b2 ? 2 : 0) | (b3 ? 4 : 0);
  }
}

__global__ __launch_bounds__(VT) void audit_compare_kernel(const PlaneOut* __restrict__ out, int na,
                                                           const int32_t* __restrict__ pool, const int32_t* __restrict__ prio,
                                                           const int32_t* __restrict__ seeds, const PlaneRec* __restrict__ planes,
                                                           int np, const int32_t* __restrict__ lists, int64_t th_count, int* stats,
                                                           const int32_t* __restrict__ dead, int32_t* __restrict__ retry)
{
  const int w = blockIdx.x;
  if (w >= na)
    return;
  const PlaneOut o = out[w];
  if (retry) {
    const bool interfered = o.status != ST_DONE || o.log_n != 0 || dead[o.seed] != 0;
    if (threadIdx.x == 0)
      retry[w] = interfered ? 1 : 0;
    if (interfered)
      return;
  }
  int lo = 0, hi = np;
  while (lo < hi) {
    const int mid = (lo + hi) >> 1;
    if (seeds[mid] < o.seed)
      lo = mid + 1;
    else
      hi = mid;
  }
  const bool committed = lo < np && seeds[lo] == o.seed;
  bool bad = o.status != ST_DONE;
  if (!bad && committed) {
    const PlaneRec r = planes[lo];
    bad = r.list_n != o.list_n || r.center[0] != o.center[0] || r.center[1] != o.center[1] || r.center[2] != o.center[2] ||
          __double_as_longlong(r.normal[0]) != __double_as_longlong(o.normal[0]) ||
          __double_as_longlong(r.normal[1]) != __double_as_longlong(o.normal[1]) ||
          __double_as_longlong(r.normal[2]) != __double_as_longlong(o.normal[2]);
    if (!bad)
      for (int64_t t = threadIdx.x; t < o.list_n; t += VT)
        bad = bad || lists[r.list_off + t] != prio[pool[o.list_off + t]];
  } else if (!bad) {
    bad = o.list_n > th_count;
  }
  const int b = __syncthreads_or(bad);
  if (threadIdx.x == 0) {
    if (b)
      atomicAdd(stats, 1);
    if (committed)
      atomicAdd(stats + 1, 1);
  }
}

struct CopyDesc {
  const int32_t* src;
  int32_t* dst;
  int64_t cnt;
  const int32_t* map;
};

__global__ void copy_lists_kernel(const CopyDesc* __restrict__ d, int nd)
{
  const int w = blockIdx.x;
  if (w >= nd)
    return;
  const CopyDesc c = d[w];
  for (int64_t i = blockIdx.y * (int64_t)blockDim.x + threadIdx.x; i < c.cnt; i += (int64_t)gridDim.y * blockDim.x)
    c.dst[i] = c.map ? c.map[c.src[i]] : c.src[i];
}

__global__ void label_kernel(const int32_t* __restrict__ owner, int64_t n, const int32_t* __restrict__ seeds,
                             int np, const int32_t* __restrict__ prio, int32_t* __restrict__ plane_idx)
{
  const int64_t i = blockIdx.x * (int64_t)blockDim.x + threadIdx.x;
  if (i >= n)
    return;
  const int32_t o = owner[i];
  const int64_t dst = prio[i];
  if (o == INF) {
    plane_idx[dst] = -1;
    return;
  }
  int lo = 0, hi = np;
  while (lo < hi) {
    const int mid = (lo + hi) >> 1;
    if (seeds[mid] < o)
      lo = mid + 1;
    else
      hi = mid;
  }
  plane_idx[dst] = 1 + lo;
}

constexpr int TILE1 = 12, TILE2 = 16;
__global__ void tile_min_kernel(const unsigned long long* __restrict__ cand, int ncand, unsigned long long* __restrict__ tmin1,
                                unsigned long long* __restrict__ tmin2)
{
  const int w = blockIdx.x * blockDim.x + threadIdx.x;
  if (w >= ncand)
    return;
  const unsigned long long c = cand[w];
  const uint32_t pos = (uint32_t)c;
  atomicMin(&tmin1[pos >> TILE1], c);
  atomicMin(&tmin2[pos >> TILE2], c);
}

__global__ void dispatch_key_kernel(const unsigned long long* __restrict__ cand, int ncand, const unsigned long long* __restrict__ tmin1,
                                    const unsigned long long* __restrict__ tmin2, uint32_t* __restrict__ keys)
{
  const int w = blockIdx.x * blockDim.x + threadIdx.x;
  if (w >= ncand)
    return;
  const unsigned long long c = cand[w];
  const uint32_t pos = (uint32_t)c;
  const uint32_t lvl = tmin2[pos >> TILE2] == c ? 0u : (tmin1[pos >> TILE1] == c ? 1u : 2u);
  keys[w] = lvl * (uint32_t)MAX_WAVES + (uint32_t)w;
}

__global__ void reset_dead_kernel(const unsigned long long* __restrict__ cand, int ncand, int32_t* __restrict__ dead)
{
  const int w = blockIdx.x * blockDim.x + threadIdx.x;
  if (w < ncand)
    dead[(int32_t)(cand[w] >> 32)] = 0;
}

__global__ void fill_i32_kernel(int32_t* p, int64_t n, int32_t v)
{
  const int64_t i = blockIdx.x * (int64_t)blockDim.x + threadIdx.x;
  if (i < n)
    p[i] = v;
}

inline int nblk(int64_t n, int b) { return (int)((n + b - 1) / b); }

struct ToI64 {
  __host__ __device__ int64_t operator()(int32_t v) const { return (int64_t)v; }
};

}

int launch_region_grow_spec(bs_ctx* ctx, const int32_t* d_xyz, const double* d_normals, const int32_t* d_neigh,
                            int64_t n, const bs_params& p, int32_t* d_plane_idx)
{
  hipStream_t st = ctx->stream;
  ctx->rg_valid = false;
  ctx->bt_valid = false;
  ctx->rg_omega = nullptr;
  ctx->rg_prio = nullptr;
  ctx->rg_seeds = nullptr;
  ctx->rg_nplanes = 0;
  const int K = p.k;
  const int64_t list_cap = 2 * n + 64;
  const int64_t planes_cap = n / std::max(1, p.th_point_count) + 64;
  const bs_grow_limits lim = ctx->lim;
  bs_grow_counters& gc = ctx->gc;
  gc = bs_grow_counters{};
  int retry_max_list = RETRY_MAX_LIST;
  bool retry_env = false;
  if (const char* e = getenv("BS_RETRY_MAX_LIST")) {
    retry_max_list = atoi(e);
    retry_env = true;
  }
  if (lim.retry_max_list >= 0) {
    retry_max_list = lim.retry_max_list;
    retry_env = true;
  }
  int retry_big_round = 1024;
  if (const char* e = getenv("BS_RETRY_BIG_ROUND"))
    retry_big_round = atoi(e);
  if (lim.retry_big_round >= 0)
    retry_big_round = lim.retry_big_round;
  int max_waves = MAX_WAVES;
  if (const char* e = getenv("BS_MAX_WAVES"))
    max_waves = atoi(e);
  if (lim.max_waves > 0)
    max_waves = (int)std::min<int64_t>(lim.max_waves, MAX_WAVES);
  const int wave_cap = (int)std::max<int64_t>(1, std::min<int64_t>(MAX_WAVES, n / 8 + 64));
  max_waves = (int)std::max<int64_t>(1, std::min<int64_t>(max_waves, wave_cap));
  const unsigned long long pool_cap = (unsigned long long)std::max<int64_t>(
      std::min<int64_t>(64 * n, (int64_t)3 << 30), 8 * n + (int64_t)(2 * 256 + 32 * 32) * 2 * wave_cap);
  const unsigned long long pool_cap_eff = lim.pool_cap > 0 ? std::min<unsigned long long>(pool_cap, (unsigned long long)lim.pool_cap) : pool_cap;
  gc.pool_cap = (int64_t)pool_cap_eff;
  gc.max_waves_end = max_waves;
  BS_HIP(ctx, ctx->rg_list.reserve(sizeof(int32_t) * list_cap));
  BS_HIP(ctx, ctx->rg_planes.reserve(sizeof(PlaneRec) * planes_cap));
  BS_HIP(ctx, ctx->rg_stats.reserve(sizeof(GrowStats)));
  const size_t n_i32 = (size_t)(7 * n + planes_cap + 1024 + 128);
  const size_t nb256 = (size_t)((n + 255) / 256);
  const size_t aux_bytes = sizeof(int32_t) * n_i32 + (size_t)5 * n + 3 * nb256 + 16 * nb256 + 8192 +
                           sizeof(PlaneOut) * ((size_t)wave_cap + MAX_PENDING) +
                           sizeof(CopyDesc) * ((size_t)wave_cap + MAX_PENDING);
  BS_HIP(ctx, ctx->rg_aux.reserve(aux_bytes));
  BS_HIP(ctx, ctx->rg_stack.reserve(sizeof(int32_t) * pool_cap));
  BS_HIP(ctx, ctx->rg_radj.reserve(sizeof(int32_t) * (size_t)(n * (K - 1) + 16)));
  BS_HIP(ctx, ctx->rg_roff.reserve(sizeof(int64_t) * (size_t)(n + 2)));
  int64_t* roff = ctx->rg_roff.as<int64_t>();
  int32_t* aux = ctx->rg_aux.as<int32_t>();
  int32_t* d_misc = aux;
  uint32_t* hmask = (uint32_t*)(aux + 1024);
  int32_t* omega = aux + 1024 + n;
  int32_t* base = aux + 1024 + 2 * n;
  int32_t* dead = aux + 1024 + 3 * n;
  int32_t* prio = aux + 1024 + 4 * n;
  int32_t* rpos = aux + 1024 + 5 * n;
  int32_t* vmark = aux + 1024 + 6 * n + 64;
  int32_t* d_seeds = aux + 1024 + 7 * n + 64;
  uint8_t* flags = (uint8_t*)(aux + n_i32);
  uint8_t* ps = flags + n;
  uint32_t* occ = (uint32_t*)(((uintptr_t)(ps + n) + 15) & ~(uintptr_t)15);
  uint8_t* dirty0 = (uint8_t*)occ + ((n + 31) / 32) * 4 + 16;
  uint8_t* dirty1 = dirty0 + n;
  uint8_t* bdirty0 = dirty1 + n;
  uint8_t* bdirty1 = bdirty0 + nb256;
  uint8_t* bcand = bdirty1 + nb256;
  int32_t* wl_list[2];
  uint32_t* wl_flag[2];
  wl_list[0] = (int32_t*)(((uintptr_t)(bcand + nb256) + 15) & ~(uintptr_t)15);
  wl_list[1] = wl_list[0] + nb256;
  wl_flag[0] = (uint32_t*)(wl_list[1] + nb256);
  wl_flag[1] = wl_flag[0] + nb256;
  PlaneOut* d_out = (PlaneOut*)(((uintptr_t)(wl_flag[1] + nb256) + 255) & ~(uintptr_t)255);
  PlaneOut* d_pend = d_out + wave_cap;
  CopyDesc* d_copy = (CopyDesc*)(d_pend + MAX_PENDING);
  int32_t* radj = ctx->rg_radj.as<int32_t>();
  unsigned long long* d_pool_top = (unsigned long long*)(d_misc + 16);
  Pool pool = {ctx->rg_stack.as<int32_t>(), d_pool_top, pool_cap_eff};

  SpecArgs a;
  a.xyz = d_xyz;
  a.normals = d_normals;
  a.neigh = d_neigh;
  a.n = n;
  a.K = K;
  a.th = (double)p.th_thickness;
  a.cos_th = p.cos_th;
  a.th_count = p.th_point_count;
  a.F = 0;
  a.pad = 0;

  const int KC = K <= 16 ? 16 : 32;
  const int quads = 4 + KC / 4;
  BS_HIP(ctx, ctx->rg_rec.reserve(sizeof(int4) * (size_t)quads * n));
  int4* rec = ctx->rg_rec.as<int4>();
  BS_HIP(ctx, ctx->rg_geo.reserve(sizeof(unsigned long long) * 2 * (size_t)(n + 64)));
  unsigned long long* cand_raw = ctx->rg_geo.as<unsigned long long>();
  BS_HIP(ctx, ctx->rg_gs.reserve(sizeof(int4) * 3 * (size_t)(n + 1)));
  int4* gs = ctx->rg_gs.as<int4>();
  unsigned long long* d_cand = cand_raw + n + 64;
  const size_t nt1 = (size_t)(n >> TILE1) + 2, nt2 = (size_t)(n >> TILE2) + 2;
  BS_HIP(ctx, ctx->rg_disp.reserve(sizeof(unsigned long long) * (nt1 + nt2) + sizeof(uint32_t) * 2 * (size_t)wave_cap + 64 +
                                    sizeof(PlaneOut) * (size_t)wave_cap));
  unsigned long long* tmin1 = ctx->rg_disp.as<unsigned long long>();
  unsigned long long* tmin2 = tmin1 + nt1;
  uint32_t* dkeys_in = reinterpret_cast<uint32_t*>(tmin2 + nt2);
  uint32_t* dkeys_out = dkeys_in + wave_cap;
  PlaneOut* d_outc = reinterpret_cast<PlaneOut*>(((uintptr_t)(dkeys_out + wave_cap) + 15) & ~(uintptr_t)15);
  const bool dispatch_order = getenv("BS_NO_DISPATCH_ORDER") == nullptr;
  const int32_t* order = (ctx->order_n == n && ctx->order_xyz == d_xyz) ? ctx->vals_out.as<int32_t>() : nullptr;
  int32_t* pos = nullptr;
  const int32_t* npos = (order && ctx->npos_neigh == d_neigh && ctx->npos_k == K) ? ctx->seg_npos.as<int32_t>() : nullptr;
  (void)hipEventRecord(ctx->ev[8], st);
  if (!npos) {
    static const bool identity = getenv("BS_FOREIGN_ORDER_IDENTITY") != nullptr;
    order = nullptr;
    if (!identity) {
      const int orc = build_spatial_order(ctx, d_xyz, n);
      if (orc != BS_OK)
        return orc;
      order = ctx->vals_out.as<int32_t>();
    }
  }
  const int4* spts_in = npos ? ctx->spts.as<int4>() : nullptr;
  const double* pnorm_in = (npos && ctx->npos_normals == d_normals) ? pnorm_of(ctx->seg_npos.as<int32_t>(), n, K) : nullptr;
  if (order && !npos) {
    pos = vmark;
    invert_order_kernel<<<nblk(n, 256), 256, 0, st>>>(order, n, pos);
  }
  if (KC == 16)
    build_records_kernel<16><<<nblk(n, 256), 256, 0, st>>>(a, order, pos, npos, rec, prio, gs, spts_in, pnorm_in);
  else
    build_records_kernel<32><<<nblk(n, 256), 256, 0, st>>>(a, order, pos, npos, rec, prio, gs, spts_in, pnorm_in);
  BS_HIP(ctx, hipMemsetAsync(rpos, 0, sizeof(int32_t) * (n + 1), st));
  uint32_t* lmask = reinterpret_cast<uint32_t*>(vmark);
  const int32_t* rows = npos ? npos : reinterpret_cast<const int32_t*>(rec) + 16;
  const int row_stride = npos ? K : quads * 4;
  static_mask_kernel<<<xcd_grid(nblk(n, 256)), 256, 0, st>>>(a, rows, row_stride, gs, hmask, rpos, lmask);
  {
    hipcub::TransformInputIterator<int64_t, ToI64, const int32_t*> in(rpos, ToI64());
    size_t tb = 0;
    BS_HIP(ctx, hipcub::DeviceScan::ExclusiveScan(nullptr, tb, in, roff, hipcub::Sum(), (int64_t)0, (int)(n + 1), st));
    BS_HIP(ctx, ctx->cub_tmp.reserve(tb));
    BS_HIP(ctx, hipcub::DeviceScan::ExclusiveScan(ctx->cub_tmp.p, tb, in, roff, hipcub::Sum(), (int64_t)0, (int)(n + 1), st));
  }
  unsigned long long* rcur = cand_raw;
  BS_HIP(ctx, hipMemcpyAsync(rcur, roff, sizeof(int64_t) * n, hipMemcpyDeviceToDevice, st));
  rev_fill_kernel<<<xcd_grid(nblk(n, 256)), 256, 0, st>>>(hmask, rows, row_stride, n, rcur, radj, lmask);
  fill_i32_kernel<<<nblk(n, 256), 256, 0, st>>>(base, n, INF);
  seed_flags_kernel<<<nblk(n, 256), 256, 0, st>>>(hmask, n, K, ps);
  BS_HIP(ctx, hipMemsetAsync(vmark, 0, sizeof(int32_t) * n, st));
  BS_HIP(ctx, hipMemsetAsync(occ, 0, sizeof(uint32_t) * (size_t)((n + 31) / 32 + 2), st));
  int64_t passes = 0;
  const int pull_sub = (int)std::max<int64_t>(1, std::min<int64_t>(64, (int64_t)nb256 / 4096));
  const int cand_sub = std::max(1, pull_sub / 8);
  const bool use_wl = !(getenv("BS_OWNER_WORKLIST") && atoi(getenv("BS_OWNER_WORKLIST")) == 0);
  int own_grid = (int)std::min<size_t>(nb256, 4096);
  if (const char* e = getenv("BS_OWNER_GRID"))
    own_grid = std::max(1, std::min(own_grid, atoi(e)));
  constexpr int PULL_GROUP = 16;
  int own_group = PULL_GROUP;
  if (const char* e = getenv("BS_OWNER_GROUP"))
    own_group = std::max(2, std::min(PULL_GROUP, atoi(e)));
  int* const wl_cnt = d_misc + 64;
  int64_t wl_pass = 0;
  bool wl_marked = false;
  const bool dbg = getenv("BS_DEBUG") != nullptr;
  BS_HIP(ctx, ctx->rg_hout.reserve(sizeof(PlaneOut) * ((size_t)wave_cap + MAX_PENDING) + 256));
  PlaneOut* const h_out = ctx->rg_hout.as<PlaneOut>();
  PlaneOut* const h_pend = h_out + wave_cap;
  int32_t* const h_flags = reinterpret_cast<int32_t*>(h_pend + MAX_PENDING);
  int32_t* const h_cnt = h_flags + 48;
  {
    uint8_t* state = dirty1;
    uint8_t* bund = bdirty1;
    int32_t* const d_any = d_misc + 32;
    decide_init_kernel<<<nblk(n, 256), 256, 0, st>>>(hmask, n, state, bund);
    for (int it = 0;; it++) {
      BS_HIP(ctx, hipMemsetAsync(d_any, 0, sizeof(int32_t) * PULL_GROUP, st));
      for (int g = 0; g < own_group; g++, passes++)
        decide_pass_kernel<<<(int)((nb256 + pull_sub - 1) / pull_sub), 256, 0, st>>>(n, pull_sub, prio, roff, radj, state, bund,
                                                                                    d_any + g, g ? d_any + g - 1 : nullptr);
      BS_HIP(ctx, hipMemcpyAsync(h_cnt, d_any + own_group - 1, sizeof(int32_t), hipMemcpyDeviceToHost, st));
      BS_HIP(ctx, hipStreamSynchronize(st));
      if (h_cnt[0] == 0)
        break;
      if (it > 4 * 1000 * 1000)
        return fail(ctx, BS_ERR_INTERNAL, "orphan fixed point (decided states) did not converge");
    }
    decide_finish_kernel<<<nblk(n, 256), 256, 0, st>>>(n, prio, roff, radj, state, omega, occ, rec, quads, rpos);
    BS_HIP(ctx, hipMemsetAsync(wl_cnt, 0, 3 * sizeof(int), st));
    BS_HIP(ctx, hipMemsetAsync(wl_flag[0], 0, sizeof(uint32_t) * 2 * nb256, st));
  }
  BS_HIP(ctx, hipMemsetAsync(dirty0, 0, n, st));
  BS_HIP(ctx, hipMemsetAsync(dirty1, 0, n, st));
  BS_HIP(ctx, hipMemsetAsync(bdirty0, 0, nb256, st));
  BS_HIP(ctx, hipMemsetAsync(bdirty1, 0, nb256, st));
  BS_HIP(ctx, hipMemsetAsync(bcand, 1, nb256, st));
  BS_HIP(ctx, hipMemsetAsync(dead, 0, sizeof(int32_t) * n, st));
  uint8_t* dcur = dirty0;
  uint8_t* dnext = dirty1;
  uint8_t* bcur = bdirty0;
  uint8_t* bnext = bdirty1;
  int32_t* const d_flip = d_misc + 32;
  int32_t* const h_flip = h_flags + 32;
  int32_t* const d_pstat = d_misc + 128;
  auto propagate = [&]() -> int {
    if (use_wl && wl_marked)
      wl_compact_kernel<<<(int)((nb256 + WL_CAP - 1) / WL_CAP), 256, 0, st>>>(bcur, (int)nb256, wl_flag[wl_pass & 1], wl_list[wl_pass & 1],
                                                                      wl_cnt + wl_pass % 3);
    wl_marked = false;
    for (int it = 0; it < 1000000; it++) {
      BS_HIP(ctx, hipMemsetAsync(d_flip, 0, sizeof(int32_t) * PULL_GROUP, st));
      if (dbg)
        BS_HIP(ctx, hipMemsetAsync(d_pstat, 0, sizeof(int32_t) * 4 * PULL_GROUP, st));
      for (int g = 0; g < own_group; g++) {
        if (use_wl) {
          const int cur = (int)(wl_pass & 1);
          pull_list_kernel<<<own_grid, 256, 0, st>>>(n, K, hmask, prio, ps, base, roff, radj, omega, occ, dcur, dnext, wl_list[cur],
                                                    wl_list[cur ^ 1], wl_flag[cur], wl_flag[cur ^ 1], wl_cnt, (int)(wl_pass % 3),
                                                    (int)((wl_pass + 1) % 3), (int)((wl_pass + 2) % 3), rec, quads, d_flip + g,
                                                    rpos , dbg ? d_pstat + 4 * g : nullptr);
          wl_pass++;
        } else {
          pull_pass_kernel<<<(int)((nb256 + pull_sub - 1) / pull_sub), 256, 0, st>>>(n, K, pull_sub, hmask, prio, ps, base, roff, radj,
                                                                                    omega, occ, dcur, dnext, bcur, bnext, rec, quads,
                                                                                    d_flip + g, rpos ,
                                                                                    g ? d_flip + g - 1 : nullptr,
                                                                                    dbg ? d_pstat + 4 * g : nullptr);
        }
        passes++;
        std::swap(dcur, dnext);
        std::swap(bcur, bnext);
      }
      BS_HIP(ctx, hipMemcpyAsync(h_flip, d_flip, sizeof(int32_t) * PULL_GROUP, hipMemcpyDeviceToHost, st));
      if (dbg) {
        int32_t hs[4 * PULL_GROUP];
        BS_HIP(ctx, hipMemcpyAsync(hs, d_pstat, sizeof hs, hipMemcpyDeviceToHost, st));
        BS_HIP(ctx, hipStreamSynchronize(st));
        for (int g = 0; g < own_group; g++)
          if (hs[4 * g])
            fprintf(stderr, "[bs] owner pass %ld: dirty groups %d, dirty points %d, walked their list %d, most groups in one workgroup %d\n",
                    (long)(passes - own_group + g), hs[4 * g], hs[4 * g + 1], hs[4 * g + 2], hs[4 * g + 3]);
      }
      BS_HIP(ctx, hipStreamSynchronize(st));
      if (!h_flip[own_group - 1]) {
        if (getenv("BS_VERIFY")) {
          BS_HIP(ctx, hipMemsetAsync(d_misc + 3, 0, sizeof(int), st));
          verify_fixpoint_kernel<<<nblk(n, 256), 256, 0, st>>>(n, hmask, prio, ps, base, roff, radj, omega, occ, d_misc + 3);
          int nb = 0;
          BS_HIP(ctx, hipMemcpyAsync(&nb, d_misc + 3, sizeof nb, hipMemcpyDeviceToHost, st));
          BS_HIP(ctx, hipStreamSynchronize(st));
          if (nb)
            fprintf(stderr, "[bs] VERIFY: owner structure is not a fixed point at %d points (pass %ld)\n", nb, (long)passes);
        }
        return BS_OK;
      }
    }
    return fail(ctx, BS_ERR_INTERNAL, "orphan fixed point did not converge");
  };
  int rc = propagate();
  if (rc != BS_OK)
    return rc;
  (void)hipEventRecord(ctx->ev[9], st);

  const int64_t pstore_cap = 6 * n + 65536;
  BS_HIP(ctx, ctx->rg_pstore.reserve(sizeof(int32_t) * pstore_cap));
  const int64_t pstore_lim = lim.pstore_cap > 0 ? std::min<int64_t>(pstore_cap, lim.pstore_cap) : pstore_cap;
  const int pend_lim = lim.max_pending > 0 ? (int)std::min<int64_t>(MAX_PENDING, lim.max_pending) : MAX_PENDING;
  int32_t* pstore = ctx->rg_pstore.as<int32_t>();
  int64_t pstore_top = 0;
  std::vector<PlaneOut> pending;

  std::vector<PlaneRec> recs;
  std::vector<int32_t> seeds;
  std::vector<CopyDesc> copies;
  int64_t list_used = 0, largest = 0, attempts = 0, rounds = 0, grow_launches = 0;
  double grow_ms = 0.0;
  bool timed_round = false;
  const bool force_full_refresh = lim.full_refresh != 0 || getenv("BS_FULL_REFRESH") != nullptr;
  bool full_refresh = force_full_refresh;
  int32_t F = 0;
  auto commit_plane = [&](const PlaneOut& o, const int32_t* src_pool) -> int {
    attempts++;
    if (!o.keep)
      return BS_OK;
    if (list_used + o.list_n > list_cap || (int64_t)recs.size() >= planes_cap)
      return fail(ctx, BS_ERR_INTERNAL, "region grow (speculative): list pool overflow");
    copies.push_back({src_pool + o.list_off, ctx->rg_list.as<int32_t>() + list_used, o.list_n, prio});
    PlaneRec r;
    for (int c = 0; c < 3; c++) {
      r.normal[c] = o.normal[c];
      r.center[c] = o.center[c];
    }
    r.list_off = list_used;
    r.list_n = o.list_n;
    r.id = (int32_t)recs.size() + 1;
    r.seed = o.seed;
    r.pad = 0;
    recs.push_back(r);
    seeds.push_back(o.seed);
    list_used += o.list_n;
    largest = std::max<int64_t>(largest, o.list_n);
    return BS_OK;
  };
  auto flush_copies = [&]() -> int {
    for (size_t off = 0; off < copies.size(); off += (size_t)wave_cap + MAX_PENDING) {
      const int nd = (int)std::min<size_t>(copies.size() - off, (size_t)wave_cap + MAX_PENDING);
      BS_HIP(ctx, hipMemcpyAsync(d_copy, copies.data() + off, sizeof(CopyDesc) * nd, hipMemcpyHostToDevice, st));
      copy_lists_kernel<<<dim3(nd, 8), 256, 0, st>>>(d_copy, nd);
      BS_HIP(ctx, hipStreamSynchronize(st));
    }
    copies.clear();
    return BS_OK;
  };
  bool cand_listed = false;
  int32_t ncand_all = 0;
  bool v3_pending = false;
  struct SideGuard {
    bs_ctx* c;
    bool* pending;
    ~SideGuard()
    {
      if (*pending && c->side)
        (void)hipStreamSynchronize(c->side);
    }
  } side_guard{ctx, &v3_pending};
  bool dead_dirty = false;
  if (!ctx->side) {
    BS_HIP(ctx, hipStreamCreateWithFlags(&ctx->side, hipStreamNonBlocking));
    BS_HIP(ctx, hipEventCreateWithFlags(&ctx->sev[0], hipEventDisableTiming));
    BS_HIP(ctx, hipEventCreateWithFlags(&ctx->sev[1], hipEventDisableTiming));
  }
  int32_t rejects_seen = 0;
  int refused_rounds = 0;
  int64_t incons[3] = {0, 0, 0};
  int forge_mode = ctx->forge_mode;
  ctx->forge_mode = 0;
  const bool do_validate3 = getenv("BS_NO_VALIDATE3") == nullptr;
  const bool use_spec2 = KC == 16 && !(getenv("BS_GROW_V2") && atoi(getenv("BS_GROW_V2")) == 0);
  auto launch_grow = [&](int cnt, const unsigned long long* cd, PlaneOut* o, int rml, const uint32_t* ord) {
    const int64_t cap = 512 * n + 4096;
    if (use_spec2)
      grow_spec2_kernel<16><<<cnt, 64, 0, st>>>(a, cd, cnt, rec, dead, pool, o, cap, rml, ord);
    else if (KC == 16)
      grow_spec_kernel<16><<<cnt, 64, 0, st>>>(a, cd, cnt, rec, dead, pool, o, cap, rml, ord);
    else
      grow_spec_kernel<32><<<cnt, 64, 0, st>>>(a, cd, cnt, rec, dead, pool, o, cap, rml, ord);
  };
  BS_HIP(ctx, hipMemsetAsync(d_misc + 4, 0, 12 * sizeof(int), st));
  for (;;) {
    rounds++;
    gc.rounds = rounds;
    a.F = F;
    const int npend = (int)pending.size();
    if (!cand_listed) {
      BS_HIP(ctx, hipMemsetAsync(d_misc + 1, 0, sizeof(int32_t), st));
      cand_flag_kernel<<<(int)((nb256 + cand_sub - 1) / cand_sub), 256, 0, st>>>(rec, quads, K, n, F, prio, ps, 0, omega, nullptr, cand_raw, d_misc + 1, bcand, cand_sub);
      BS_HIP(ctx, hipMemcpyAsync(h_flags + 11, d_misc + 1, sizeof(int32_t), hipMemcpyDeviceToHost, st));
      BS_HIP(ctx, hipStreamSynchronize(st));
      ncand_all = h_flags[11];
    }
    cand_listed = false;
    if (ncand_all == 0 && npend == 0)
      break;
    if (ncand_all > 0) {
      size_t tb = 0;
      BS_HIP(ctx, hipcub::DeviceRadixSort::SortKeys(nullptr, tb, cand_raw, d_cand, ncand_all, 0, 64, st));
      BS_HIP(ctx, ctx->cub_tmp.reserve(tb));
      BS_HIP(ctx, hipcub::DeviceRadixSort::SortKeys(ctx->cub_tmp.p, tb, cand_raw, d_cand, ncand_all, 0, 64, st));
    }
    const int ncand = std::min<int>(ncand_all, max_waves);
    gc.rounds_capped += ncand_all > max_waves ? 1 : 0;
    gc.rounds_big += ncand >= 4096 ? 1 : 0;
    if (npend)
      BS_HIP(ctx, hipMemcpyAsync(d_pend, pending.data(), sizeof(PlaneOut) * npend, hipMemcpyHostToDevice, st));
    if (ncand > 0) {
      if (full_refresh) {
        refresh_records_kernel<<<nblk(n, 256), 256, 0, st>>>(omega, rec, quads, n);
        gc.full_refreshes++;
        full_refresh = force_full_refresh;
      } else if (getenv("BS_VERIFY")) {
        BS_HIP(ctx, hipMemsetAsync(d_misc + 3, 0, sizeof(int), st));
        verify_records_kernel<<<nblk(n, 256), 256, 0, st>>>(omega, rec, quads, n, d_misc + 3);
        int nb = 0;
        BS_HIP(ctx, hipMemcpyAsync(&nb, d_misc + 3, sizeof nb, hipMemcpyDeviceToHost, st));
        BS_HIP(ctx, hipStreamSynchronize(st));
        if (nb)
          fprintf(stderr, "[bs] VERIFY: %d records differ from a full refresh (round %ld)\n", nb, (long)rounds);
      }
      if (dead_dirty) {
        BS_HIP(ctx, hipMemsetAsync(dead, 0, sizeof(int32_t) * n, st));
        dead_dirty = false;
      }
      BS_HIP(ctx, hipMemsetAsync(d_pool_top, 0, sizeof(unsigned long long), st));
      const uint32_t* d_order = nullptr;
      if (dispatch_order && ncand >= 4096) {
        BS_HIP(ctx, hipMemsetAsync(tmin1, 0xff, sizeof(unsigned long long) * (nt1 + nt2), st));
        tile_min_kernel<<<nblk(ncand, 256), 256, 0, st>>>(d_cand, ncand, tmin1, tmin2);
        dispatch_key_kernel<<<nblk(ncand, 256), 256, 0, st>>>(d_cand, ncand, tmin1, tmin2, dkeys_in);
        size_t tb = 0;
        BS_HIP(ctx, hipcub::DeviceRadixSort::SortKeys(nullptr, tb, dkeys_in, dkeys_out, ncand, 0, 20, st));
        BS_HIP(ctx, ctx->cub_tmp.reserve(tb));
        BS_HIP(ctx, hipcub::DeviceRadixSort::SortKeys(ctx->cub_tmp.p, tb, dkeys_in, dkeys_out, ncand, 0, 20, st));
        d_order = dkeys_out;
      }
      (void)hipEventRecord(ctx->ev[6], st);
      const int rml = (ncand >= retry_big_round && !retry_env) ? 0x7fffffff : retry_max_list;
      launch_grow(ncand, d_cand, d_out, rml, d_order);
      (void)hipEventRecord(ctx->ev[7], st);
      grow_launches++;
      timed_round = true;
      if (forge_mode) {
        forge_kernel<<<1, 64, 0, st>>>(d_out, ncand, pool.base, forge_mode, d_misc + 5);
        forge_mode = 0;
      }
      validate1_kernel<<<ncand, VT, 0, st>>>(d_out, ncand, pool.base, rec, quads, dead, n, vmark,
                                             (int32_t)((rounds & 0x3ff) << 20), d_misc + 4);
      if (do_validate3) {
        BS_HIP(ctx, hipEventRecord(ctx->sev[0], st));
        BS_HIP(ctx, hipStreamWaitEvent(ctx->side, ctx->sev[0], 0));
        validate3_kernel<<<ncand, V3T, 0, ctx->side>>>(d_out, ncand, pool.base, rec, quads, d_misc + 4);
        BS_HIP(ctx, hipEventRecord(ctx->sev[1], ctx->side));
        v3_pending = true;
      }
      reset_tags_kernel<<<ncand, VT, 0, st>>>(d_out, ncand, pool.base, rec, quads, K);
      reset_dead_kernel<<<nblk(ncand, 256), 256, 0, st>>>(d_cand, ncand, dead);
      plane_apply_kernel<<<ncand, VT, 0, st>>>(d_out, ncand, pool.base, base, ps, dcur, bcur, omega, occ, rec, quads);
      wl_marked = true;
      rc = propagate();
      if (rc != BS_OK)
        return rc;
      validate2_kernel<<<ncand, VT, 0, st>>>(d_out, ncand, pool.base, omega, rec, quads, K);
    }
    if (npend)
      validate2_kernel<<<npend, VT, 0, st>>>(d_pend, npend, pstore, omega, rec, quads, K);
    const int32_t init2[2] = {0, INF};
    BS_HIP(ctx, hipMemcpyAsync(d_misc + 1, init2, sizeof init2, hipMemcpyHostToDevice, st));
    cand_flag_kernel<<<(int)((nb256 + cand_sub - 1) / cand_sub), 256, 0, st>>>(rec, quads, K, n, F, prio, ps, 0, omega, d_misc + 2, cand_raw, d_misc + 1, bcand, cand_sub);
    BS_HIP(ctx, hipMemcpyAsync(h_flags + 8, d_misc + 1, 2 * sizeof(int32_t), hipMemcpyDeviceToHost, st));
    if (v3_pending) {
      BS_HIP(ctx, hipStreamWaitEvent(st, ctx->sev[1], 0));
      v3_pending = false;
    }
    BS_HIP(ctx, hipMemcpyAsync(h_flags + 10, d_misc + 4, sizeof(int32_t), hipMemcpyDeviceToHost, st));
    const bool compact = ncand >= 4096 && !dbg;
    int nh = ncand;
    PlaneOut* d_outh = d_out;
    if (compact) {
      size_t tb = 0;
      BS_HIP(ctx, hipcub::DeviceSelect::If(nullptr, tb, d_out, d_outc, d_misc + 20, ncand, KeepForHost(), st));
      BS_HIP(ctx, ctx->cub_tmp.reserve(tb));
      BS_HIP(ctx, hipcub::DeviceSelect::If(ctx->cub_tmp.p, tb, d_out, d_outc, d_misc + 20, ncand, KeepForHost(), st));
      BS_HIP(ctx, hipMemcpyAsync(h_flags + 14, d_misc + 20, sizeof(int32_t), hipMemcpyDeviceToHost, st));
      BS_HIP(ctx, hipStreamSynchronize(st));
      nh = h_flags[14];
      d_outh = d_outc;
    }
    if (nh)
      BS_HIP(ctx, hipMemcpyAsync(h_out, d_outh, sizeof(PlaneOut) * nh, hipMemcpyDeviceToHost, st));
    if (npend)
      BS_HIP(ctx, hipMemcpyAsync(h_pend, d_pend, sizeof(PlaneOut) * npend, hipMemcpyDeviceToHost, st));
    BS_HIP(ctx, hipStreamSynchronize(st));
    const int32_t next_ncand_all = h_flags[8], new_min = h_flags[9], rejects_now = h_flags[10];
    if (timed_round) {
      float ms = 0.f;
      if (hipEventElapsedTime(&ms, ctx->ev[6], ctx->ev[7]) == hipSuccess)
        grow_ms += ms;
      timed_round = false;
    }
    int32_t first_bad = new_min;
    bool nomem_lowest = false;
    for (int w = 0; w < nh; w++) {
      const PlaneOut& o = h_out[w];
      if (dbg && o.list_n > n + 1)
        fprintf(stderr, "[bs] IMPOSSIBLE list: round %ld w=%d seed=%d status=%d consistent=%d list_n=%ld steps=%ld log=%ld thief=%d\n",
                (long)rounds, w, o.seed, o.status, o.consistent, (long)o.list_n, (long)o.steps, (long)o.log_n, o.thief);
      if (o.status == ST_WATCHDOG)
        return fail(ctx, BS_ERR_INTERNAL, "region grow (speculative): watchdog");
      if (o.status == ST_DONE && (!o.consistent || !o.v3ok))
        first_bad = std::min(first_bad, o.seed);
      if (o.status == ST_DONE && !o.consistent) {
        incons[0] += (o.pad4 & 1) ? 1 : 0;
        incons[1] += (o.pad4 & 2) ? 1 : 0;
        incons[2] += (o.pad4 & 4) ? 1 : 0;
      }
      if (o.w == 0 && o.status == ST_NOMEM)
        nomem_lowest = true;
      if (o.status == ST_NOMEM) {
        full_refresh = true;
        dead_dirty = true;
        gc.attempts_nomem++;
      }
      gc.attempts_stolen += o.status == ST_STOLEN ? 1 : 0;
    }
    for (int w = 0; w < npend; w++)
      if (!h_pend[w].consistent)
        first_bad = std::min(first_bad, h_pend[w].seed);
    if (nomem_lowest) {
      if (max_waves == 1)
        return fail(ctx, BS_ERR_NOMEM, "region grow (speculative): round pool exhausted");
      max_waves = std::max(1, max_waves / 8);
      gc.waves_cut++;
      gc.max_waves_end = max_waves;
    }
#ifdef BS_PROBE
    if (dbg) {
      unsigned long long hp[32];
      (void)hipMemcpyFromSymbol(hp, HIP_SYMBOL(g_prof2), sizeof(hp));
      const double nstep = (double)hp[10] + 1.0;
      fprintf(stderr, "[prof2] steps=%llu expansions=%llu | pop+issue=%.0f state=%.0f wait=%.0f test+classify=%.0f claims+walk=%.0f log+counters=%.0f "
                      "flushchk=%.0f list+defer=%.0f push=%.0f top=%.0f (cycles per step, cumulative over rounds)\n",
              hp[10], hp[11], hp[0] / nstep, hp[1] / nstep, hp[2] / nstep, hp[3] / nstep, hp[4] / nstep, hp[5] / nstep, hp[6] / nstep,
              hp[7] / nstep, hp[8] / nstep, hp[9] / nstep);
      unsigned long long he[16];
      (void)hipMemcpyFromSymbol(he, HIP_SYMBOL(g_exit2), sizeof(he));
      fprintf(stderr, "[exits] round %ld attempts %d engine %d | hot steps %llu complete steps %llu | lifo-empty %llu watchdog %llu "
                      "refill %llu stolen %llu earlier-claim %llu list-ring %llu lifo-window %llu log-ring %llu\n",
              (long)rounds, ncand, use_spec2 ? 3 : 1, he[9], he[10], he[0], he[1], he[2], he[3], he[4], he[6], he[7], he[8]);
      memset(he, 0, sizeof(he));
      (void)hipMemcpyToSymbol(HIP_SYMBOL(g_exit2), he, sizeof(he));
    }
#endif
    if (dbg) {
      int cnt[6] = {0, 0, 0, 0, 0, 0}, cons = 0, pcons = 0;
      int64_t maxsteps = 0, sumsteps = 0, maxlist = 0;
      for (int w = 0; w < ncand; w++) {
        cnt[h_out[w].status]++;
        cons += h_out[w].status == ST_DONE && h_out[w].consistent;
        maxsteps = std::max(maxsteps, h_out[w].steps);
        sumsteps += h_out[w].steps;
        maxlist = std::max(maxlist, h_out[w].list_n);
      }
      for (int w = 0; w < npend; w++)
        pcons += h_pend[w].consistent;
      {
        int64_t t0 = INT64_MAX, t1 = 0;
        std::vector<int> idx;
        for (int w = 0; w < ncand; w++) {
          t0 = std::min(t0, h_out[w].t_start);
          t1 = std::max(t1, h_out[w].t_end);
          if (h_out[w].steps > 2000)
            idx.push_back(w);
        }
        std::sort(idx.begin(), idx.end(), [&](int x, int y) { return h_out[x].steps > h_out[y].steps; });
        fprintf(stderr, "[bs]   launch span %.2f ms; longest attempts (w, steps, status, start ms, end ms, us/step):", (t1 - t0) / 1e5);
        for (size_t q = 0; q < std::min<size_t>(idx.size(), 12); q++) {
          const PlaneOut& o = h_out[idx[q]];
          fprintf(stderr, " [%d %ld %d %.2f %.2f %.3f xcc%d se%d cu%d simd%d]", idx[q], (long)o.steps, o.status, (o.t_start - t0) / 1e5,
                  (o.t_end - t0) / 1e5, (o.t_end - o.t_start) / 100.0 / (double)o.steps, (o.pad5 >> 16) & 0xf, (o.pad5 >> 13) & 7,
                  (o.pad5 >> 8) & 0xf, (o.pad5 >> 4) & 3);
        }
        fprintf(stderr, "\n");
        if (ncand > 20000) {
          fprintf(stderr, "[bs]   start ms by w:");
          for (int w = 0; w < ncand; w += 8192)
            fprintf(stderr, " %d:%.2f", w, (h_out[w].t_start - t0) / 1e5);
          double life0 = 0, lifep = 0;
          int64_t n0 = 0, npl = 0;
          for (int w = 0; w < ncand; w++) {
            if (h_out[w].status == ST_FAILED0) {
              life0 += (h_out[w].t_end - h_out[w].t_start) / 100.0;
              n0++;
            } else {
              lifep += (h_out[w].t_end - h_out[w].t_start) / 100.0;
              npl++;
            }
          }
          fprintf(stderr, "\n[bs]   mean lifetime: failed0 %.1f us (%ld), others %.1f us (%ld); wave-time total %.1f ms\n", life0 / std::max<int64_t>(n0, 1),
                  (long)n0, lifep / std::max<int64_t>(npl, 1), (long)npl, (life0 + lifep) / 1e3);
        }
      }
      int why[8] = {0, 0, 0, 0, 0, 0, 0, 0};
      for (int w = 0; w < ncand; w++)
        if (h_out[w].status == ST_DONE && !h_out[w].consistent)
          why[h_out[w].pad4 & 7]++;
      fprintf(stderr, "[bs]   inconsistent new planes by failed test (1 seed row, 2 list, 4 log; sums): 1:%d 2:%d 3:%d 4:%d 5:%d 6:%d 7:%d\n",
              why[1], why[2], why[3], why[4], why[5], why[6], why[7]);
      fprintf(stderr,
              "[bs] round %ld F=%d ncand_all=%d grown=%d done=%d (consistent %d) failed0=%d nomem=%d stolen=%d "
              "pending=%d (consistent %d) first_bad=%d new_min=%d maxsteps=%ld sumsteps=%ld maxlist=%ld passes=%ld\n",
              (long)rounds, F, ncand_all, ncand, cnt[ST_DONE], cons, cnt[ST_FAILED0], cnt[ST_NOMEM], cnt[ST_STOLEN],
              npend, pcons, first_bad, new_min, (long)maxsteps, (long)sumsteps, (long)maxlist, (long)passes);
      if (getenv("BS_DEBUG_PLANES"))
        for (int w = 0; w < ncand; w++)
          fprintf(stderr, "[bs]   plane seed=%d status=%d consistent=%d steps=%ld list=%ld log=%ld thief=%d\n",
                  h_out[w].seed, h_out[w].status, h_out[w].consistent, (long)h_out[w].steps, (long)h_out[w].list_n,
                  (long)h_out[w].log_n, h_out[w].thief);
    }
    std::vector<PlaneOut> next_pending;
    int finals = 0, dropped = 0;
    int pend_room = pend_lim;
    for (int w = 0; w < npend; w++)
      pend_room -= (h_pend[w].consistent && h_pend[w].seed >= first_bad) ? 1 : 0;
    {
      int ip = 0, iw = 0;
      while (ip < npend || iw < nh) {
        const bool take_p = (iw >= nh) || (ip < npend && h_pend[ip].seed < h_out[iw].seed);
        PlaneOut& o = take_p ? h_pend[ip] : h_out[iw];
        const int32_t* src = take_p ? pstore : pool.base;
        if (take_p)
          ip++;
        else
          iw++;
        o.pad = 0;
        if (o.status != ST_DONE)
          continue;
        if (!o.consistent || !o.v3ok) {
          o.pad = 2;
          dropped++;
          gc.dropped_other++;
          continue;
        }
        if (o.seed < first_bad) {
          finals++;
          if (dbg && o.keep)
            fprintf(stderr, "[bs]   commit seed=%d n=%ld log=%ld steps=%ld from=%s round=%ld first_bad=%d\n", o.seed,
                    (long)o.list_n, (long)o.log_n, (long)o.steps, take_p ? "pending" : "new", (long)rounds, first_bad);
          rc = commit_plane(o, src);
          if (rc != BS_OK)
            return rc;
        } else if (take_p) {
          next_pending.push_back(o);
        } else if (pend_room > 0 && pstore_top + o.list_n + o.log_n + 8 <= pstore_lim) {
          pend_room--;
          PlaneOut q = o;
          q.list_off = pstore_top;
          copies.push_back({pool.base + o.list_off, pstore + q.list_off, o.list_n, nullptr});
          pstore_top += (o.list_n + 3) & ~(int64_t)3;
          q.log_off = pstore_top;
          if (o.log_n)
            copies.push_back({pool.base + o.log_off, pstore + q.log_off, o.log_n, nullptr});
          pstore_top += (o.log_n + 3) & ~(int64_t)3;
          next_pending.push_back(q);
        } else {
          o.pad = 2;
          dropped++;
          if (pend_room > 0)
            gc.dropped_pend_store++;
          else
            gc.dropped_pend_count++;
        }
      }
    }
    rc = flush_copies();
    if (rc != BS_OK)
      return rc;
    if (dropped) {
      if (nh) {
        BS_HIP(ctx, hipMemcpyAsync(d_outh, h_out, sizeof(PlaneOut) * nh, hipMemcpyHostToDevice, st));
        plane_apply_kernel<<<nh, VT, 0, st>>>(d_outh, nh, pool.base, base, ps, dcur, bcur, omega, occ, rec, quads);
        wl_marked = true;
      }
      if (npend) {
        BS_HIP(ctx, hipMemcpyAsync(d_pend, h_pend, sizeof(PlaneOut) * npend, hipMemcpyHostToDevice, st));
        plane_apply_kernel<<<npend, VT, 0, st>>>(d_pend, npend, pstore, base, ps, dcur, bcur, omega, occ, rec, quads);
        wl_marked = true;
      }
      rc = propagate();
      if (rc != BS_OK)
        return rc;
    } else {
      cand_listed = true;
      ncand_all = next_ncand_all;
    }
    pending.swap(next_pending);
    if (pending.empty())
      pstore_top = 0;
    if (first_bad == INF)
      break;
    const bool refused = rejects_now > rejects_seen;
    rejects_seen = rejects_now;
    refused_rounds = refused ? refused_rounds + 1 : 0;
    if (finals == 0 && dropped == 0 && !nomem_lowest && first_bad <= F && (!refused || refused_rounds > 8))
      return fail(ctx, BS_ERR_INTERNAL, refused ? "region grow (speculative): the validation keeps refusing a plane"
                                                : "region grow (speculative): no progress");
    F = first_bad;
    if (rounds > 4 * n + 16)
      return fail(ctx, BS_ERR_INTERNAL, "region grow (speculative): round limit");
  }
  int32_t* owner_final = omega;
  const int np = (int)recs.size();
  if (np > 0) {
    BS_HIP(ctx, hipMemcpyAsync(d_seeds, seeds.data(), sizeof(int32_t) * np, hipMemcpyHostToDevice, st));
    BS_HIP(ctx, hipMemcpyAsync(ctx->rg_planes.p, recs.data(), sizeof(PlaneRec) * np, hipMemcpyHostToDevice, st));
  }
  label_kernel<<<nblk(n, 256), 256, 0, st>>>(owner_final, n, d_seeds, np, prio, d_plane_idx);
  int32_t vstat[12] = {0};
  BS_HIP(ctx, hipMemcpyAsync(vstat, d_misc + 4, sizeof vstat, hipMemcpyDeviceToHost, st));
  GrowStats hs;
  hs.n_planes = np;
  hs.error = 0;
  hs.list_used = list_used;
  hs.seed_attempts = attempts;
  hs.largest = largest;
  hs.steps = passes;
  BS_HIP(ctx, hipMemcpyAsync(ctx->rg_stats.p, &hs, sizeof hs, hipMemcpyHostToDevice, st));
  BS_HIP(ctx, hipStreamSynchronize(st));
  BS_HIP(ctx, hipGetLastError());
  ctx->rg_n = n;
  ctx->rg_valid = true;
  ctx->rg_omega = owner_final;
  ctx->rg_prio = prio;
  ctx->rg_seeds = d_seeds;
  ctx->rg_nplanes = np;
  ctx->tm.largest_plane = largest;
  ctx->tm.n_seed_attempts = attempts;
  ctx->tm.rg_rounds = rounds;
  ctx->tm.grow_kernel_ms = grow_ms;
  ctx->tm.grow_kernel_launches = grow_launches;
  ctx->tm.validation_rejects = vstat[0];
  ctx->tm.forged_seed = vstat[1] - 1;
  ctx->tm.forged_refused = vstat[2];
  ctx->tm.rej_v1_robbed = vstat[8];
  ctx->tm.rej_v1_tag = vstat[9];
  ctx->tm.rej_v1_dup = vstat[10];
  ctx->tm.rej_v3_state = vstat[11];
  ctx->tm.incons_seed = incons[0];
  ctx->tm.incons_list = incons[1];
  ctx->tm.incons_log = incons[2];
  {
    float ms = 0.f;
    ctx->tm.grow_setup_ms = hipEventElapsedTime(&ms, ctx->ev[8], ctx->ev[9]) == hipSuccess ? (double)ms : 0.0;
  }
  ctx->tm.audit_attempts = -1;
  ctx->tm.audit_mismatches = 0;
  ctx->tm.audit_ms = 0.0;
  if (ctx->audit || getenv("BS_AUDIT")) {
    const auto t0 = std::chrono::steady_clock::now();
    pool.cap = pool_cap;
    BS_HIP(ctx, hipMemsetAsync(bcand, 1, nb256, st));
    BS_HIP(ctx, hipMemsetAsync(d_misc + 1, 0, sizeof(int32_t), st));
    BS_HIP(ctx, hipMemsetAsync(d_misc + 8, 0, 2 * sizeof(int32_t), st));
    cand_flag_kernel<<<(int)((nb256 + cand_sub - 1) / cand_sub), 256, 0, st>>>(rec, quads, K, n, 0, prio, ps, 1, omega, nullptr,
                                                                              cand_raw, d_misc + 1, bcand, cand_sub);
    BS_HIP(ctx, hipMemcpyAsync(h_flags + 11, d_misc + 1, sizeof(int32_t), hipMemcpyDeviceToHost, st));
    BS_HIP(ctx, hipStreamSynchronize(st));
    const int na = h_flags[11];
    std::vector<unsigned long long> hc((size_t)na), hc_sorted;
    if (na > 0)
      BS_HIP(ctx, hipMemcpy(hc.data(), cand_raw, sizeof(unsigned long long) * na, hipMemcpyDeviceToHost));
    std::sort(hc.begin(), hc.end());
    int n_committed = 0;
    {
      std::vector<unsigned long long> rest;
      for (const unsigned long long c : hc) {
        const int32_t sd = (int32_t)(c >> 32);
        if (std::binary_search(seeds.begin(), seeds.end(), sd))
          hc_sorted.push_back(c);
        else
          rest.push_back(c);
      }
      n_committed = (int)hc_sorted.size();
      hc_sorted.insert(hc_sorted.end(), rest.begin(), rest.end());
    }
    if (na > 0)
      BS_HIP(ctx, hipMemcpyAsync(d_cand, hc_sorted.data(), sizeof(unsigned long long) * na, hipMemcpyHostToDevice, st));
    a.F = INF;
    auto grow_n = [&](int off, int cnt, PlaneOut* o) { launch_grow(cnt, d_cand + off, o, 0, nullptr); };
    auto compare_n = [&](int cnt, int32_t* retry) {
      audit_compare_kernel<<<cnt, VT, 0, st>>>(d_out, cnt, pool.base, prio, d_seeds, ctx->rg_planes.as<PlaneRec>(), np,
                                               ctx->rg_list.as<int32_t>(), a.th_count, d_misc + 8, dead, retry);
    };
    for (int off = 0; off < n_committed; off += wave_cap) {
      const int cnt = std::min(n_committed - off, wave_cap);
      BS_HIP(ctx, hipMemsetAsync(d_pool_top, 0, sizeof(unsigned long long), st));
      grow_n(off, cnt, d_out);
      compare_n(cnt, nullptr);
      reset_tags_kernel<<<cnt, VT, 0, st>>>(d_out, cnt, pool.base, rec, quads, K);
    }
    {
      std::vector<unsigned long long> pend(hc_sorted.begin() + n_committed, hc_sorted.end()), next;
      int32_t* d_retry = reinterpret_cast<int32_t*>(dkeys_in);
      std::vector<int32_t> h_retry;
      int batches = 0;
      while (!pend.empty()) {
        next.clear();
        for (size_t off = 0; off < pend.size(); off += (size_t)wave_cap) {
          const int cnt = (int)std::min<size_t>(pend.size() - off, (size_t)wave_cap);
          BS_HIP(ctx, hipMemcpyAsync(d_cand, pend.data() + off, sizeof(unsigned long long) * cnt, hipMemcpyHostToDevice, st));
          BS_HIP(ctx, hipMemsetAsync(d_pool_top, 0, sizeof(unsigned long long), st));
          reset_dead_kernel<<<nblk(cnt, 256), 256, 0, st>>>(d_cand, cnt, dead);
          grow_n(0, cnt, d_out);
          compare_n(cnt, d_retry);
          reset_tags_kernel<<<cnt, VT, 0, st>>>(d_out, cnt, pool.base, rec, quads, K);
          reset_dead_kernel<<<nblk(cnt, 256), 256, 0, st>>>(d_cand, cnt, dead);
          h_retry.resize((size_t)cnt);
          BS_HIP(ctx, hipMemcpyAsync(h_retry.data(), d_retry, sizeof(int32_t) * cnt, hipMemcpyDeviceToHost, st));
          BS_HIP(ctx, hipStreamSynchronize(st));
          for (int i = 0; i < cnt; i++)
            if (h_retry[i])
              next.push_back(pend[off + i]);
        }
        if (next.size() == pend.size()) {
          const size_t last_off = (pend.size() - 1) / (size_t)wave_cap * (size_t)wave_cap;
          const int nshow = (int)std::min<size_t>(pend.size() - last_off, 3);
          std::vector<PlaneOut> ho((size_t)nshow);
          BS_HIP(ctx, hipMemcpy(ho.data(), d_out, sizeof(PlaneOut) * nshow, hipMemcpyDeviceToHost));
          std::string msg = "audit: a batch of rolled-back attempts made no progress (" + std::to_string(pend.size()) + " left;";
          for (const PlaneOut& o : ho)
            msg += " seed " + std::to_string(o.seed) + " status " + std::to_string(o.status) + " list " + std::to_string(o.list_n) +
                   " log " + std::to_string(o.log_n) + " thief " + std::to_string(o.thief) + ";";
          msg += ")";
          return fail(ctx, BS_ERR_INTERNAL, msg.c_str());
        }
        pend.swap(next);
        batches++;
      }
      if (dbg)
        fprintf(stderr, "[bs] audit: %d rolled-back attempts replayed in %d batches\n", na - n_committed, batches);
    }
    BS_HIP(ctx, hipMemcpyAsync(h_flags + 12, d_misc + 8, 2 * sizeof(int32_t), hipMemcpyDeviceToHost, st));
    BS_HIP(ctx, hipStreamSynchronize(st));
    BS_HIP(ctx, hipGetLastError());
    ctx->tm.audit_attempts = na;
    ctx->tm.audit_mismatches = (int64_t)h_flags[12] + (h_flags[13] != np ? 1 : 0);
    ctx->tm.audit_ms = std::chrono::duration<double, std::milli>(std::chrono::steady_clock::now() - t0).count();
    if (dbg || ctx->tm.audit_mismatches)
      fprintf(stderr, "[bs] audit: %d attempts replayed, %d of %d committed planes met, %d mismatches, %.1f ms\n", na, h_flags[13], np,
              h_flags[12], ctx->tm.audit_ms);
  }
  return BS_OK;
}

}
```

### include/bs_api.h

```cpp
#ifndef BS_API_H
#define BS_API_H

#include <stdint.h>

#ifdef __cplusplus
extern "C" {
#endif

#define BS_API_VERSION 5

typedef enum bs_status {
  BS_OK = 0,
  BS_ERR_INVALID = -1,
  BS_ERR_RANGE = -2,
  BS_ERR_NOMEM = -3,
  BS_ERR_HIP = -4,
  BS_ERR_NO_DEVICE = -5,
  BS_ERR_INTERNAL = -6,
  BS_ERR_UNCERTIFIED = -7
} bs_status;

typedef struct bs_params {
  int32_t k;
  int32_t max_nn;
  double radius;
  int32_t th_thickness;
  int32_t th_point_count;
  double cos_th;
  int32_t cell_size;
  int32_t rg_mode;
} bs_params;

typedef struct bs_planes {
  int32_t n_planes;
  int32_t* id;
  double* normal;
  int32_t* center;
  int64_t* offset;
  int32_t* point_idx;
} bs_planes;

typedef struct bs_timings {
  double grid_ms;
  double knn_ms;
  double grow_ms;
  double total_ms;
  int64_t largest_plane;
  int64_t n_seed_attempts;
  int64_t n_fallback_queries;
  int64_t rg_rounds;
  double grow_kernel_ms;
  int64_t grow_kernel_launches;
  double grow_setup_ms;
  int64_t validation_rejects;
  int64_t forged_seed;
  int64_t forged_refused;
  int64_t audit_attempts;
  int64_t audit_mismatches;
  double audit_ms;
  int64_t tie_rows;
  int64_t rej_v1_robbed, rej_v1_tag, rej_v1_dup, rej_v3_state;
  int64_t incons_seed, incons_list, incons_log;
} bs_timings;

int64_t bs_sizeof_timings(void);

typedef struct bs_ctx bs_ctx;

int bs_api_version(void);
const char* bs_strerror(int status);
void bs_params_default(bs_params* p);

int bs_create(int device, bs_ctx** out);
void bs_destroy(bs_ctx* ctx);
const char* bs_last_error(const bs_ctx* ctx);
int bs_set_stream(bs_ctx* ctx, void* hip_stream);
int bs_get_timings(const bs_ctx* ctx, bs_timings* out);


int bs_knn_normals(bs_ctx* ctx, const int32_t* xyz, int64_t n, const bs_params* p,
                   int32_t* neigh , double* normals );

int bs_region_grow(bs_ctx* ctx, const int32_t* xyz, const double* normals,
                   const int32_t* neigh, int64_t n, const bs_params* p,
                   int32_t* plane_idx , bs_planes* planes );

int bs_segment(bs_ctx* ctx, const int32_t* xyz, int64_t n, const bs_params* p,
               int32_t* neigh , double* normals ,
               int32_t* plane_idx, bs_planes* planes );

int bs_knn_normals_halo(bs_ctx* ctx, const int32_t* xyz, const int32_t* gidx, int64_t n, int64_t n_query,
                        const bs_params* p, int32_t* neigh , double* normals ,
                        double cert_radius, int64_t* n_uncertified);

void bs_planes_free(bs_planes* planes);

int bs_plane_colors(const bs_planes* planes, const int32_t* plane_rgb, int64_t n,
                    uint16_t* colors );


int bs_knn_normals_dev(bs_ctx* ctx, const int32_t* d_xyz, const int32_t* d_gidx, int64_t n,
                       int64_t q_begin, int64_t q_end, const bs_params* p,
                       int32_t* d_neigh, double* d_normals, double cert_radius,
                       int64_t* n_uncertified);

int bs_region_grow_dev(bs_ctx* ctx, const int32_t* d_xyz, const double* d_normals,
                       const int32_t* d_neigh, int64_t n, const bs_params* p,
                       int32_t* d_plane_idx);

int bs_segment_dev(bs_ctx* ctx, const int32_t* d_xyz, int64_t n, const bs_params* p,
                   int32_t* d_neigh, double* d_normals, int32_t* d_plane_idx);

int bs_shift_to_origin_dev(bs_ctx* ctx, int32_t* d_xyz, int64_t n, int32_t* min_out);

int bs_ingest_dev(bs_ctx* ctx, const void* d_records, int64_t n, int32_t stride, int32_t off_x, int32_t off_y,
                  int32_t off_z, int32_t is_f64, double scale, int32_t shift_to_origin, int32_t* d_xyz,
                  int32_t* min_out);
int bs_plane_colors_dev(bs_ctx* ctx, const int32_t* plane_rgb, int32_t n_planes, int64_t n, uint16_t* d_colors);

int bs_grid_dims(const int32_t* extent, int32_t bin, int32_t* width, int32_t* height);
int bs_grid_picture(bs_ctx* ctx, const int32_t* xyz, int64_t n, const int32_t* extent, int32_t bin,
                    int32_t bin_height, double* image, double* ground_th);
int bs_grid_picture_dev(bs_ctx* ctx, const int32_t* d_xyz, int64_t n, const int32_t* extent, int32_t bin,
                        int32_t bin_height, double* d_image, double* ground_th);

int bs_selftest_center_div(bs_ctx* ctx, const int32_t* c, const uint32_t* n, int32_t* out, int64_t count);

int bs_selftest_forge_next(bs_ctx* ctx, int mode);

int bs_set_audit(bs_ctx* ctx, int on);

typedef struct bs_grow_limits {
  int64_t max_waves;
  int64_t pool_cap;
  int64_t max_pending;
  int64_t pstore_cap;
  int32_t retry_max_list;
  int32_t retry_big_round;
  int32_t full_refresh;
  int32_t reserved;
} bs_grow_limits;
int bs_selftest_grow_limits(bs_ctx* ctx, const bs_grow_limits* lim);

typedef struct bs_grow_counters {
  int64_t rounds;
  int64_t rounds_capped;
  int64_t rounds_big;
  int64_t attempts_nomem;
  int64_t waves_cut;
  int64_t max_waves_end;
  int64_t attempts_stolen;
  int64_t dropped_pend_count;
  int64_t dropped_pend_store;
  int64_t dropped_other;
  int64_t full_refreshes;
  int64_t pool_cap;
} bs_grow_counters;
int bs_get_grow_counters(const bs_ctx* ctx, bs_grow_counters* out);

int bs_planes_fetch(bs_ctx* ctx, bs_planes* planes);

int bs_segment_batch(bs_ctx* ctx, const int32_t* xyz, const int64_t* tile_offset, int32_t n_tiles, const bs_params* p,
                     int32_t* neigh, double* normals, int32_t* plane_idx, bs_planes* planes, int32_t* plane_offset);
int bs_segment_batch_dev(bs_ctx* ctx, const int32_t* d_xyz, const int64_t* tile_offset, int32_t n_tiles,
                         const bs_params* p, int32_t* d_neigh, double* d_normals, int32_t* d_plane_idx);
int bs_batch_planes_fetch(bs_ctx* ctx, bs_planes* planes, int32_t* plane_offset);
int bs_shift_tiles_to_origin_dev(bs_ctx* ctx, int32_t* d_xyz, const int64_t* tile_offset, int32_t n_tiles,
                                 int32_t* min_out);

int bs_cc_hook_dev(bs_ctx* ctx, const int32_t* d_rows, const int32_t* d_gidx, int64_t m, int32_t k, int32_t* d_parent,
                   int64_t n_total, int64_t* n_hooks);
int bs_owner_fetch_dev(bs_ctx* ctx, int32_t* d_owner);
int bs_plane_seeds_dev(bs_ctx* ctx, int32_t* d_seeds, int64_t cap, int32_t* n_planes);
int bs_stream_sync(bs_ctx* ctx);
int bs_labels_from_owner_dev(bs_ctx* ctx, const int32_t* d_owner, int64_t n, const int32_t* d_seeds, int32_t n_seeds,
                             int32_t* d_plane_idx);
int bs_remap_rows_dev(bs_ctx* ctx, const int32_t* d_rows, int64_t n_rows, int32_t k, const int32_t* d_sorted_gidx,
                      int64_t n, int32_t* d_out, int32_t* n_missing);

typedef enum bs_comm_dtype { BS_I32 = 0, BS_I64 = 1 } bs_comm_dtype;
typedef enum bs_comm_op { BS_MIN = 0, BS_MAX = 1, BS_SUM = 2 } bs_comm_op;
typedef struct bs_comm_ops {
  void* handle;
  int32_t rank, world;
  int (*all_reduce)(void* handle, void* d_buf, int64_t count, int dtype, int op, void* stream);
  int (*all_gather)(void* handle, const void* d_send, void* d_recv, int64_t bytes, void* stream);
  int (*all_to_all_v)(void* handle, const void* d_send, const int64_t* send_bytes, void* d_recv,
                      const int64_t* recv_bytes, void* stream);
} bs_comm_ops;

int bs_comm_rccl(void* nccl_comm, int32_t rank, int32_t world, bs_comm_ops* out);
int bs_comm_rccl_unique_id(char id[128]);
int bs_comm_rccl_init(bs_ctx* ctx, const char id[128], int32_t rank, int32_t world, void** nccl_comm);
int bs_comm_rccl_destroy(void* nccl_comm);

int bs_comm_local_create(int32_t world, bs_comm_ops* out );
void bs_comm_local_destroy(bs_comm_ops* ops );

typedef struct bs_shard_info {
  int64_t n_own;
  int64_t n_local;
  int64_t n_grow;
  int64_t components;
  int64_t planes_total;
  int32_t cc_iterations, halo_retries;
  double halo_mm;
  double ms_partition, ms_halo, ms_knn, ms_components, ms_redistribute, ms_grow, ms_labels;
} bs_shard_info;

int bs_segment_sharded(bs_ctx* ctx, const bs_comm_ops* comm, const int32_t* d_xyz, const int32_t* d_gidx, int64_t m,
                       int64_t n_total, const bs_params* p, double halo, int32_t* d_plane_idx, bs_shard_info* info);
int bs_sharded_planes_fetch(bs_ctx* ctx, bs_planes* planes);

typedef struct bs_contours {
  int32_t n_contours;
  int32_t width, height;
  int64_t* offset;
  int32_t* xy;
  double* area;
  double* perimeter;
} bs_contours;

typedef struct bs_footprint_info {
  double ms_mask, ms_close, ms_label, ms_trace, ms_total;
  int64_t fg_pixels;
  int64_t border_states;
  int64_t components;
  int64_t jump_rounds;
} bs_footprint_info;

int bs_footprints_dev(bs_ctx* ctx, const double* d_image, int32_t width, int32_t height, int32_t threshold,
                      int32_t kernel_size, int32_t iterations, uint8_t* d_mask, bs_contours* out,
                      bs_footprint_info* info);
int bs_footprints(bs_ctx* ctx, const double* image, int32_t width, int32_t height, int32_t threshold,
                  int32_t kernel_size, int32_t iterations, uint8_t* mask, bs_contours* out, bs_footprint_info* info);
void bs_contours_free(bs_contours* c);
int bs_contours_write_obj(const bs_contours* c, const char* path);


int bs_tile_boxes_dev(bs_ctx* ctx, const int32_t* d_xyz, const int64_t* tile_offset, int32_t n_tiles,
                      int32_t* box_out);

int bs_grid_dims_batch(const int32_t* extent, int32_t n_tiles, int32_t bin, int32_t* width, int32_t* height,
                       int64_t* pixel_offset);

int bs_grid_picture_batch_dev(bs_ctx* ctx, const int32_t* d_xyz, const int64_t* tile_offset, int32_t n_tiles,
                              const int32_t* extent, int32_t bin, int32_t bin_height, double* d_image,
                              double* ground_th);
int bs_grid_picture_batch(bs_ctx* ctx, const int32_t* xyz, const int64_t* tile_offset, int32_t n_tiles,
                          const int32_t* extent, int32_t bin, int32_t bin_height, double* image, double* ground_th);

int bs_footprints_batch_dev(bs_ctx* ctx, const double* d_image, const int32_t* width, const int32_t* height,
                            int32_t n_tiles, int32_t threshold, int32_t kernel_size, int32_t iterations,
                            uint8_t* d_mask, bs_contours* out, int32_t* contour_offset, bs_footprint_info* info);
int bs_footprints_batch(bs_ctx* ctx, const double* image, const int32_t* width, const int32_t* height,
                        int32_t n_tiles, int32_t threshold, int32_t kernel_size, int32_t iterations, uint8_t* mask,
                        bs_contours* out, int32_t* contour_offset, bs_footprint_info* info);

typedef struct bs_buildings {
  int32_t n_buildings;
  int32_t width, height;
  int32_t* start_xy;
  int32_t* bbox;
  int64_t* pixels;
  int64_t* fg_pixels;
  int64_t* n_points;
  int64_t* n_above;
  int32_t* z_min;
  int32_t* z_max;
  int64_t* z_sum;
  double ms_label_mask;
  double ms_label_fill;
  double ms_number;
  double ms_map;
  double ms_assign;
} bs_buildings;

int bs_building_map_dev(bs_ctx* ctx, const uint8_t* d_mask, int32_t width, int32_t height, int32_t* d_map,
                        bs_buildings* out);
int bs_building_map(bs_ctx* ctx, const uint8_t* mask, int32_t width, int32_t height, int32_t* map, bs_buildings* out);
void bs_buildings_free(bs_buildings* b);

int bs_assign_buildings_dev(bs_ctx* ctx, const int32_t* d_xyz, int64_t n, int32_t bin, double ground_th,
                            const int32_t* d_map, int32_t width, int32_t height, int32_t* d_building_idx,
                            bs_buildings* inout);
int bs_assign_buildings(bs_ctx* ctx, const int32_t* xyz, int64_t n, int32_t bin, double ground_th, const int32_t* map,
                        int32_t width, int32_t height, int32_t* building_idx, bs_buildings* inout);

int bs_plane_buildings_dev(bs_ctx* ctx, const int32_t* d_plane_idx, const int32_t* d_building_idx, int64_t n,
                           int32_t n_planes, int32_t n_buildings, int32_t* plane_building, int64_t* votes_in,
                           int64_t* votes_total, int64_t* votes_outside);
int bs_plane_buildings(bs_ctx* ctx, const int32_t* plane_idx, const int32_t* building_idx, int64_t n, int32_t n_planes,
                       int32_t n_buildings, int32_t* plane_building, int64_t* votes_in, int64_t* votes_total,
                       int64_t* votes_outside);

int bs_buildings_write_obj(const bs_contours* c, const bs_buildings* b, int32_t bin, const int32_t* origin,
                           double ground_th, double min_area, double min_perimeter, const char* path);

struct bs_roofs {
  int32_t n_planes;
  int32_t width, height;
  int32_t fill_rounds;
  int64_t seeded_pixels;
  int64_t filled_pixels;
  int64_t unroofed_pixels;
  int64_t* pixels;
  int64_t* seed_pixels;
  int32_t* bbox;
  int64_t* n_support;
  int32_t* z_min;
  int32_t* z_max;
  int64_t* z_sum;
  double ms_vote;
  double ms_fill;
  double ms_figures;
  double ms_height;
};

int bs_roof_homes(const double* normal, const int32_t* plane_building, const int64_t* votes_in, const int64_t* votes_total,
                  int32_t n_planes, double min_normal_z, int32_t* home_out);

int bs_roofs_dev(bs_ctx* ctx, const int32_t* d_xyz, int64_t n, int32_t bin, double ground_th, const int32_t* d_map,
                 int32_t width, int32_t height, const int32_t* d_plane_idx, int32_t n_planes, const int32_t* home,
                 const double* normal, const int32_t* center, int32_t min_votes, int32_t* d_roof, int32_t* d_support,
                 int32_t* d_height, struct bs_roofs* out);
int bs_roofs(bs_ctx* ctx, const int32_t* xyz, int64_t n, int32_t bin, double ground_th, const int32_t* map,
             int32_t width, int32_t height, const int32_t* plane_idx, int32_t n_planes, const int32_t* home,
             const double* normal, const int32_t* center, int32_t min_votes, int32_t* roof, int32_t* support,
             int32_t* height_out, struct bs_roofs* out);
void bs_roofs_free(struct bs_roofs* r);

int bs_roofs_write_obj(const int32_t* roof, const int32_t* map, int32_t width, int32_t height, const struct bs_roofs* r,
                       const double* normal, const int32_t* center, int32_t bin, const int32_t* origin, const char* path);

#ifdef __cplusplus
}
#endif
#endif
```

Measured before the change: 200.5 Mpoints/s.

## Speculate region-grow round tail to cut host syncs and rescan only live groups

```diff
diff --git a/buildingsegment_amd/_lib.py b/buildingsegment_amd/_lib.py
--- a/buildingsegment_amd/_lib.py
+++ b/buildingsegment_amd/_lib.py
@@ -61,7 +61,8 @@
 class GrowCounters(C.Structure):
     _fields_ = [(k, C.c_int64) for k in
                 ("rounds", "rounds_capped", "rounds_big", "attempts_nomem", "waves_cut", "max_waves_end", "attempts_stolen",
-                 "dropped_pend_count", "dropped_pend_store", "dropped_other", "full_refreshes", "pool_cap")]
+                 "dropped_pend_count", "dropped_pend_store", "dropped_other", "full_refreshes", "pool_cap",
+                 "host_syncs", "tails_redone", "cand_groups_scanned", "cand_scans", "owner_passes", "owner_settles")]
 
 
 API_VERSION = 5
diff --git a/buildingsegment_amd/csrc/bs_common.h b/buildingsegment_amd/csrc/bs_common.h
--- a/buildingsegment_amd/csrc/bs_common.h
+++ b/buildingsegment_amd/csrc/bs_common.h
@@ -201,7 +201,7 @@
   bs_grow_limits lim{0, 0, 0, 0, -1, -1, 0, 0};
   bs_grow_counters gc{};
   hipStream_t side = nullptr;
-  hipEvent_t sev[2] = {nullptr, nullptr};
+  hipEvent_t sev[4] = {nullptr, nullptr, nullptr, nullptr};
   bs::DevBuf rs_keys_in, rs_keys_out, rs_vals_in, rs_vals_out, rs_cnt, rs_img, rs_tmp;
   int64_t order_n = 0;
   const int32_t* order_xyz = nullptr;
diff --git a/buildingsegment_amd/csrc/bs_grow_spec.hip b/buildingsegment_amd/csrc/bs_grow_spec.hip
--- a/buildingsegment_amd/csrc/bs_grow_spec.hip
+++ b/buildingsegment_amd/csrc/bs_grow_spec.hip
@@ -657,61 +657,130 @@
     ps[i] = hmask[i] == full ? 0 : 2;
 }
 
+__device__ inline int cand_group(const int4* __restrict__ rec, int quads, int K, int64_t n, int32_t F,
+                                 const int32_t* __restrict__ prio, const uint8_t* __restrict__ ps, int all_seeds,
+                                 const int32_t* __restrict__ omega, int32_t* min_idx, unsigned long long* __restrict__ cand_out,
+                                 int32_t* cand_count, int64_t g)
+{
+  const int64_t i = (g << 8) + threadIdx.x;
+  bool c = false, alive = false;
+  const uint8_t f = i < n ? ps[i] : (uint8_t)2;
+  int32_t pi = 0;
+  if (!(f & 2)) {
+    pi = prio[i];
+    const int32_t oi = omega[i];
+    alive = !(oi < F);
+    if (pi >= F && oi >= pi && (all_seeds || !(f & 1))) {
+      c = true;
+      const int32_t* row = reinterpret_cast<const int32_t*>(rec + i * quads + 4);
+      for (int u = 1; u < K; u += OWN_TRIP) {
+        int32_t nb[OWN_TRIP];
+        int32_t ov[OWN_TRIP];
+#pragma unroll
+        for (int q = 0; q < OWN_TRIP; q++)
+          nb[q] = row[u + q < K ? u + q : K - 1];
+#pragma unroll
+        for (int q = 0; q < OWN_TRIP; q++)
+          ov[q] = omega[nb[q]];
+#pragma unroll
+        for (int q = 0; q < OWN_TRIP; q++)
+          c = c && ov[q] >= pi;
+      }
+    }
+  }
+  const int any_alive = __syncthreads_or(alive);
+  if (c && min_idx)
+    atomicMin(min_idx, pi);
+  if (c && cand_out)
+    cand_out[atomicAdd(cand_count, 1)] = ((unsigned long long)(uint32_t)pi << 32) | (uint32_t)i;
+  return any_alive;
+}
+
+__device__ inline void cand_finish(int32_t* work, int32_t* res, const int* surv, const int* nsurv_p, int32_t* __restrict__ live_out)
+{
+  asm volatile("s_waitcnt vmcnt(0)" ::: "memory");
+  __syncthreads();
+  __shared__ int live_base;
+  const int nsurv = *nsurv_p;
+  if (threadIdx.x == 0)
+    live_base = nsurv ? atomicAdd(&work[2], nsurv) : 0;
+  __syncthreads();
+  if ((int)threadIdx.x < nsurv)
+    live_out[live_base + threadIdx.x] = surv[threadIdx.x];
+  if (threadIdx.x == 0) {
+    if (atomicAdd(&work[3], 1) == (int)gridDim.x - 1) {
+      res[0] = atomicExch(&work[0], 0);
+      res[1] = atomicExch(&work[1], INF);
+      res[2] = atomicExch(&work[2], 0);
+      atomicExch(&work[3], 0);
+    }
+  }
+}
+
 __global__ void cand_flag_kernel(const int4* __restrict__ rec, int quads, int K,
                                  int64_t n, int32_t F, const int32_t* __restrict__ prio, const uint8_t* __restrict__ ps,
                                  int all_seeds, const int32_t* __restrict__ omega, int32_t* min_idx,
                                  unsigned long long* __restrict__ cand_out, int32_t* cand_count, uint8_t* __restrict__ bcand,
-                                 int sub)
+                                 int sub, int32_t* work, int32_t* res, int32_t* __restrict__ live_out)
 {
   __shared__ unsigned long long sub_mask;
+  __shared__ int surv[64];
+  __shared__ int nsurv;
   const int64_t nb256 = (n + 255) >> 8;
   const int64_t g0 = (int64_t)blockIdx.x * sub;
   if (threadIdx.x < 64) {
     const int64_t gidx = g0 + threadIdx.x;
     const bool live = (int)threadIdx.x < sub && gidx < nb256 && bcand[gidx] != 0;
     const unsigned long long m = ballot64(live);
-    if (threadIdx.x == 0)
+    if (threadIdx.x == 0) {
       sub_mask = m;
+      nsurv = 0;
+    }
   }
   __syncthreads();
   unsigned long long gm = sub_mask;
+  if (work) {
+    min_idx = work + 1;
+    cand_count = work;
+  }
   while (gm) {
     const int t = __ffsll(gm) - 1;
     gm &= gm - 1;
-    const int64_t i = ((g0 + t) << 8) + threadIdx.x;
-    bool c = false, alive = false;
-    const uint8_t f = i < n ? ps[i] : (uint8_t)2;
-    int32_t pi = 0;
-    if (!(f & 2)) {
-      pi = prio[i];
-      const int32_t oi = omega[i];
-      alive = !(oi < F);
-      if (pi >= F && oi >= pi && (all_seeds || !(f & 1))) {
-        c = true;
-        const int32_t* row = reinterpret_cast<const int32_t*>(rec + i * quads + 4);
-        for (int u = 1; u < K; u += OWN_TRIP) {
-          int32_t nb[OWN_TRIP];
-          int32_t ov[OWN_TRIP];
-#pragma unroll
-          for (int q = 0; q < OWN_TRIP; q++)
-            nb[q] = row[u + q < K ? u + q : K - 1];
-#pragma unroll
-          for (int q = 0; q < OWN_TRIP; q++)
-            ov[q] = omega[nb[q]];
-#pragma unroll
-          for (int q = 0; q < OWN_TRIP; q++)
-            c = c && ov[q] >= pi;
-        }
-      }
-    }
-    const int any_alive = __syncthreads_or(alive);
-    if (threadIdx.x == 0 && !any_alive)
-      bcand[g0 + t] = 0;
-    if (c && min_idx)
-      atomicMin(min_idx, pi);
-    if (c && cand_out)
-      cand_out[atomicAdd(cand_count, 1)] = ((unsigned long long)(uint32_t)pi << 32) | (uint32_t)i;
-  }
+    const int any_alive = cand_group(rec, quads, K, n, F, prio, ps, all_seeds, omega, min_idx, cand_out, cand_count, g0 + t);
+    if (threadIdx.x == 0) {
+      if (!any_alive)
+        bcand[g0 + t] = 0;
+      else if (work)
+        surv[nsurv++] = (int)(g0 + t);
+    }
+  }
+  if (work)
+    cand_finish(work, res, surv, &nsurv, live_out);
+}
+
+__global__ void cand_list_kernel(const int4* __restrict__ rec, int quads, int K, int64_t n, int32_t F,
+                                 const int32_t* __restrict__ prio, const uint8_t* __restrict__ ps,
+                                 const int32_t* __restrict__ omega, unsigned long long* __restrict__ cand_out,
+                                 uint8_t* __restrict__ bcand, int sub, const int32_t* __restrict__ live_in, int nlive,
+                                 int32_t* __restrict__ live_out, int speculative, int32_t* work, int32_t* res)
+{
+  __shared__ int surv[64];
+  __shared__ int nsurv;
+  if (threadIdx.x == 0)
+    nsurv = 0;
+  const int e0 = blockIdx.x * sub;
+  const int e1 = min(e0 + sub, nlive);
+  for (int e = e0; e < e1; e++) {
+    const int g = live_in[e];
+    const int any_alive = cand_group(rec, quads, K, n, F, prio, ps, 0, omega, work + 1, cand_out, work, g);
+    if (threadIdx.x == 0) {
+      if (any_alive)
+        surv[nsurv++] = g;
+      else if (!speculative)
+        bcand[g] = 0;
+    }
+  }
+  cand_finish(work, res, surv, &nsurv, live_out);
 }
 
 template <int KC>
@@ -1779,42 +1848,6 @@
 
 constexpr int VT = 1024;
 
-__global__ __launch_bounds__(VT) void validate1_kernel(PlaneOut* out, int ncand, const int32_t* __restrict__ pool,
-                                                       int4* rec, int quads, const int32_t* __restrict__ dead, int64_t n,
-                                                       int32_t* __restrict__ vmark, int32_t round_key, int* rejects)
-{
-  const int w = blockIdx.x;
-  if (w >= ncand || out[w].status != ST_DONE)
-    return;
-  const PlaneOut o = out[w];
-  const bool robbed = dead[o.seed] != 0 || o.list_n > n + 1;
-  bool bad = robbed, bad_tag = false, bad_dup = false;
-  const int32_t key = round_key + w + 1;
-  for (int64_t t = 1 + threadIdx.x; t < o.list_n; t += VT) {
-    const int32_t p = pool[o.list_off + t];
-    const bool tagbad = *rec_tag(rec, quads, p) != o.seed;
-    bad_tag = bad_tag || tagbad;
-    const bool dup = atomicExch(&vmark[p], key) == key;
-    if (dup)
-      atomicAdd(rejects, 1);
-    bad_dup = bad_dup || dup;
-    bad = bad || tagbad || dup;
-  }
-  const int b = __syncthreads_or(bad);
-  const int bt = __syncthreads_or(bad_tag), bd = __syncthreads_or(bad_dup);
-  if (threadIdx.x == 0) {
-    if (b) {
-      atomicAdd(rejects + (robbed ? 8 : (bd ? 10 : 9)), 1);
-      (void)bt;
-      out[w].status = ST_STOLEN;
-      if (rejects[1] == o.seed + 1)
-        rejects[2] = 1;
-    } else {
-      out[w].pad = 1;
-    }
-  }
-}
-
 constexpr int V3T = 256;
 constexpr int V3C = 1024;
 __global__ __launch_bounds__(V3T) void validate3_kernel(PlaneOut* out, int ncand, const int32_t* __restrict__ pool,
@@ -2017,6 +2050,74 @@
   }
 }
 
+__global__ __launch_bounds__(VT) void plane_round_kernel(PlaneOut* out, int ncand, const int32_t* __restrict__ pool, int4* rec,
+                                                         int quads, int K, const int32_t* __restrict__ dead, int64_t n,
+                                                         int32_t* __restrict__ vmark, int32_t round_key, int* rejects,
+                                                         int32_t* base, uint8_t* ps, uint8_t* dirty, uint8_t* bdirty,
+                                                         int32_t* omega, const uint32_t* __restrict__ occ)
+{
+  const int w = blockIdx.x;
+  if (w >= ncand)
+    return;
+  const PlaneOut o = out[w];
+  bool ins = false;
+  if (o.status == ST_DONE) {
+    const bool robbed = dead[o.seed] != 0 || o.list_n > n + 1;
+    bool bad = robbed, bad_tag = false, bad_dup = false;
+    const int32_t key = round_key + w + 1;
+    for (int64_t t = 1 + threadIdx.x; t < o.list_n; t += VT) {
+      const int32_t p = pool[o.list_off + t];
+      const bool tagbad = *rec_tag(rec, quads, p) != o.seed;
+      bad_tag = bad_tag || tagbad;
+      const bool dup = atomicExch(&vmark[p], key) == key;
+      if (dup)
+        atomicAdd(rejects, 1);
+      bad_dup = bad_dup || dup;
+      bad = bad || tagbad || dup;
+    }
+    const int b = __syncthreads_or(bad);
+    const int bd = __syncthreads_or(bad_dup);
+    if (threadIdx.x == 0) {
+      if (b) {
+        atomicAdd(rejects + (robbed ? 8 : (bd ? 10 : 9)), 1);
+        out[w].status = ST_STOLEN;
+        if (rejects[1] == o.seed + 1)
+          rejects[2] = 1;
+      } else {
+        out[w].pad = 1;
+      }
+    }
+    ins = !b;
+  }
+  if (ins && threadIdx.x == 0) {
+    ps[o.seed_pos] = 1;
+    dirty[o.seed_pos] = 1;
+    bdirty[o.seed_pos >> 8] = 1;
+  }
+  const bool put = ins && o.keep;
+  for (int64_t t = 1 + threadIdx.x; t < o.list_n; t += VT) {
+    const int32_t p = pool[o.list_off + t];
+    int32_t* tg = rec_tag(rec, quads, p);
+    if (*tg == o.seed)
+      *tg = INF;
+    if (put) {
+      atomicMin(&base[p], o.seed);
+      const int32_t old = atomicMin(&omega[p], o.seed);
+      if (old > o.seed)
+        reinterpret_cast<int32_t*>(rec + (int64_t)p * quads)[3] = o.seed;
+      if ((occ[p >> 5] >> (p & 31)) & 1u) {
+        dirty[p] = 1;
+        bdirty[p >> 8] = 1;
+      }
+    }
+  }
+  if (threadIdx.x >= 1 && threadIdx.x < K) {
+    int32_t* tg = rec_tag(rec, quads, reinterpret_cast<const int32_t*>(rec + (int64_t)o.seed_pos * quads + 4)[threadIdx.x]);
+    if (*tg == o.seed)
+      *tg = INF;
+  }
+}
+
 __global__ void verify_records_kernel(const int32_t* __restrict__ omega, int4* rec, int quads, int64_t n, int* nbad)
 {
   const int64_t i = blockIdx.x * (int64_t)blockDim.x + threadIdx.x;
@@ -2100,6 +2201,7 @@
   }
 }
 
+constexpr size_t DESC_CHUNK = 65536;
 struct CopyDesc {
   const int32_t* src;
   int32_t* dst;
@@ -2165,11 +2267,14 @@
   keys[w] = lvl * (uint32_t)MAX_WAVES + (uint32_t)w;
 }
 
-__global__ void reset_dead_kernel(const unsigned long long* __restrict__ cand, int ncand, int32_t* __restrict__ dead)
+__global__ void reset_dead_kernel(const unsigned long long* __restrict__ cand, int ncand, int32_t* __restrict__ dead,
+                                  unsigned long long* pool_top)
 {
   const int w = blockIdx.x * blockDim.x + threadIdx.x;
   if (w < ncand)
     dead[(int32_t)(cand[w] >> 32)] = 0;
+  if (w == 0 && pool_top)
+    *pool_top = 0;
 }
 
 __global__ void fill_i32_kernel(int32_t* p, int64_t n, int32_t v)
@@ -2235,7 +2340,7 @@
   BS_HIP(ctx, ctx->rg_stats.reserve(sizeof(GrowStats)));
   const size_t n_i32 = (size_t)(7 * n + planes_cap + 1024 + 128);
   const size_t nb256 = (size_t)((n + 255) / 256);
-  const size_t aux_bytes = sizeof(int32_t) * n_i32 + (size_t)5 * n + 3 * nb256 + 16 * nb256 + 8192 +
+  const size_t aux_bytes = sizeof(int32_t) * n_i32 + (size_t)5 * n + 3 * nb256 + 24 * nb256 + 8192 +
                            sizeof(PlaneOut) * ((size_t)wave_cap + MAX_PENDING) +
                            sizeof(CopyDesc) * ((size_t)wave_cap + MAX_PENDING);
   BS_HIP(ctx, ctx->rg_aux.reserve(aux_bytes));
@@ -2267,7 +2372,10 @@
   wl_list[1] = wl_list[0] + nb256;
   wl_flag[0] = (uint32_t*)(wl_list[1] + nb256);
   wl_flag[1] = wl_flag[0] + nb256;
-  PlaneOut* d_out = (PlaneOut*)(((uintptr_t)(wl_flag[1] + nb256) + 255) & ~(uintptr_t)255);
+  int32_t* live_list[2];
+  live_list[0] = reinterpret_cast<int32_t*>(wl_flag[1] + nb256);
+  live_list[1] = live_list[0] + nb256;
+  PlaneOut* d_out = (PlaneOut*)(((uintptr_t)(live_list[1] + nb256) + 255) & ~(uintptr_t)255);
   PlaneOut* d_pend = d_out + wave_cap;
   CopyDesc* d_copy = (CopyDesc*)(d_pend + MAX_PENDING);
   int32_t* radj = ctx->rg_radj.as<int32_t>();
@@ -2362,23 +2470,30 @@
   int64_t wl_pass = 0;
   bool wl_marked = false;
   const bool dbg = getenv("BS_DEBUG") != nullptr;
-  BS_HIP(ctx, ctx->rg_hout.reserve(sizeof(PlaneOut) * ((size_t)wave_cap + MAX_PENDING) + 256));
+  BS_HIP(ctx, ctx->rg_hout.reserve(sizeof(PlaneOut) * ((size_t)wave_cap + MAX_PENDING) + 512 +
+                                        2 * sizeof(CopyDesc) * DESC_CHUNK));
   PlaneOut* const h_out = ctx->rg_hout.as<PlaneOut>();
   PlaneOut* const h_pend = h_out + wave_cap;
   int32_t* const h_flags = reinterpret_cast<int32_t*>(h_pend + MAX_PENDING);
-  int32_t* const h_cnt = h_flags + 48;
+  int32_t* const h_cnt = h_flags + 64;
+  CopyDesc* const h_desc = reinterpret_cast<CopyDesc*>(h_flags + 128);
+  auto sync_main = [&]() -> hipError_t {
+    gc.host_syncs++;
+    return hipStreamSynchronize(st);
+  };
   {
     uint8_t* state = dirty1;
     uint8_t* bund = bdirty1;
     int32_t* const d_any = d_misc + 32;
     decide_init_kernel<<<nblk(n, 256), 256, 0, st>>>(hmask, n, state, bund);
+    gc.owner_settles++;
     for (int it = 0;; it++) {
       BS_HIP(ctx, hipMemsetAsync(d_any, 0, sizeof(int32_t) * PULL_GROUP, st));
       for (int g = 0; g < own_group; g++, passes++)
         decide_pass_kernel<<<(int)((nb256 + pull_sub - 1) / pull_sub), 256, 0, st>>>(n, pull_sub, prio, roff, radj, state, bund,
                                                                                     d_any + g, g ? d_any + g - 1 : nullptr);
       BS_HIP(ctx, hipMemcpyAsync(h_cnt, d_any + own_group - 1, sizeof(int32_t), hipMemcpyDeviceToHost, st));
-      BS_HIP(ctx, hipStreamSynchronize(st));
+      BS_HIP(ctx, sync_main());
       if (h_cnt[0] == 0)
         break;
       if (it > 4 * 1000 * 1000)
@@ -2401,12 +2516,12 @@
   int32_t* const d_flip = d_misc + 32;
   int32_t* const h_flip = h_flags + 32;
   int32_t* const d_pstat = d_misc + 128;
-  auto propagate = [&]() -> int {
+  auto launch_group = [&]() -> int {
     if (use_wl && wl_marked)
       wl_compact_kernel<<<(int)((nb256 + WL_CAP - 1) / WL_CAP), 256, 0, st>>>(bcur, (int)nb256, wl_flag[wl_pass & 1], wl_list[wl_pass & 1],
                                                                       wl_cnt + wl_pass % 3);
     wl_marked = false;
-    for (int it = 0; it < 1000000; it++) {
+    {
       BS_HIP(ctx, hipMemsetAsync(d_flip, 0, sizeof(int32_t) * PULL_GROUP, st));
       if (dbg)
         BS_HIP(ctx, hipMemsetAsync(d_pstat, 0, sizeof(int32_t) * 4 * PULL_GROUP, st));
@@ -2429,6 +2544,24 @@
         std::swap(dcur, dnext);
         std::swap(bcur, bnext);
       }
+    }
+    return BS_OK;
+  };
+  auto verify_fixpoint = [&]() -> int {
+    BS_HIP(ctx, hipMemsetAsync(d_misc + 3, 0, sizeof(int), st));
+    verify_fixpoint_kernel<<<nblk(n, 256), 256, 0, st>>>(n, hmask, prio, ps, base, roff, radj, omega, occ, d_misc + 3);
+    int nb = 0;
+    BS_HIP(ctx, hipMemcpyAsync(&nb, d_misc + 3, sizeof nb, hipMemcpyDeviceToHost, st));
+    BS_HIP(ctx, hipStreamSynchronize(st));
+    if (nb)
+      fprintf(stderr, "[bs] VERIFY: owner structure is not a fixed point at %d points (pass %ld)\n", nb, (long)passes);
+    return BS_OK;
+  };
+  auto propagate = [&]() -> int {
+    for (int it = 0; it < 1000000; it++) {
+      const int lrc = launch_group();
+      if (lrc != BS_OK)
+        return lrc;
       BS_HIP(ctx, hipMemcpyAsync(h_flip, d_flip, sizeof(int32_t) * PULL_GROUP, hipMemcpyDeviceToHost, st));
       if (dbg) {
         int32_t hs[4 * PULL_GROUP];
@@ -2439,22 +2572,13 @@
             fprintf(stderr, "[bs] owner pass %ld: dirty groups %d, dirty points %d, walked their list %d, most groups in one workgroup %d\n",
                     (long)(passes - own_group + g), hs[4 * g], hs[4 * g + 1], hs[4 * g + 2], hs[4 * g + 3]);
       }
-      BS_HIP(ctx, hipStreamSynchronize(st));
-      if (!h_flip[own_group - 1]) {
-        if (getenv("BS_VERIFY")) {
-          BS_HIP(ctx, hipMemsetAsync(d_misc + 3, 0, sizeof(int), st));
-          verify_fixpoint_kernel<<<nblk(n, 256), 256, 0, st>>>(n, hmask, prio, ps, base, roff, radj, omega, occ, d_misc + 3);
-          int nb = 0;
-          BS_HIP(ctx, hipMemcpyAsync(&nb, d_misc + 3, sizeof nb, hipMemcpyDeviceToHost, st));
-          BS_HIP(ctx, hipStreamSynchronize(st));
-          if (nb)
-            fprintf(stderr, "[bs] VERIFY: owner structure is not a fixed point at %d points (pass %ld)\n", nb, (long)passes);
-        }
-        return BS_OK;
-      }
+      BS_HIP(ctx, sync_main());
+      if (!h_flip[own_group - 1])
+        return getenv("BS_VERIFY") ? verify_fixpoint() : BS_OK;
     }
     return fail(ctx, BS_ERR_INTERNAL, "orphan fixed point did not converge");
   };
+  gc.owner_settles++;
   int rc = propagate();
   if (rc != BS_OK)
     return rc;
@@ -2500,12 +2624,23 @@
     largest = std::max<int64_t>(largest, o.list_n);
     return BS_OK;
   };
+  int desc_turn = 0;
+  bool desc_used[2] = {false, false};
   auto flush_copies = [&]() -> int {
-    for (size_t off = 0; off < copies.size(); off += (size_t)wave_cap + MAX_PENDING) {
-      const int nd = (int)std::min<size_t>(copies.size() - off, (size_t)wave_cap + MAX_PENDING);
-      BS_HIP(ctx, hipMemcpyAsync(d_copy, copies.data() + off, sizeof(CopyDesc) * nd, hipMemcpyHostToDevice, st));
+    for (size_t off = 0; off < copies.size(); off += DESC_CHUNK) {
+      const int nd = (int)std::min<size_t>(copies.size() - off, DESC_CHUNK);
+      const int b = desc_turn;
+      desc_turn ^= 1;
+      if (desc_used[b] && hipEventQuery(ctx->sev[2 + b]) != hipSuccess) {
+        gc.host_syncs++;
+        BS_HIP(ctx, hipEventSynchronize(ctx->sev[2 + b]));
+      }
+      CopyDesc* hd = h_desc + (size_t)b * DESC_CHUNK;
+      memcpy(hd, copies.data() + off, sizeof(CopyDesc) * nd);
+      BS_HIP(ctx, hipMemcpyAsync(d_copy, hd, sizeof(CopyDesc) * nd, hipMemcpyHostToDevice, st));
       copy_lists_kernel<<<dim3(nd, 8), 256, 0, st>>>(d_copy, nd);
-      BS_HIP(ctx, hipStreamSynchronize(st));
+      BS_HIP(ctx, hipEventRecord(ctx->sev[2 + b], st));
+      desc_used[b] = true;
     }
     copies.clear();
     return BS_OK;
@@ -2527,6 +2662,8 @@
     BS_HIP(ctx, hipStreamCreateWithFlags(&ctx->side, hipStreamNonBlocking));
     BS_HIP(ctx, hipEventCreateWithFlags(&ctx->sev[0], hipEventDisableTiming));
     BS_HIP(ctx, hipEventCreateWithFlags(&ctx->sev[1], hipEventDisableTiming));
+    BS_HIP(ctx, hipEventCreateWithFlags(&ctx->sev[2], hipEventDisableTiming));
+    BS_HIP(ctx, hipEventCreateWithFlags(&ctx->sev[3], hipEventDisableTiming));
   }
   int32_t rejects_seen = 0;
   int refused_rounds = 0;
@@ -2544,18 +2681,58 @@
     else
       grow_spec_kernel<32><<<cnt, 64, 0, st>>>(a, cd, cnt, rec, dead, pool, o, cap, rml, ord);
   };
-  BS_HIP(ctx, hipMemsetAsync(d_misc + 4, 0, 12 * sizeof(int), st));
+  BS_HIP(ctx, hipMemsetAsync(d_misc + 4, 0, 14 * sizeof(int), st));
+  int32_t* const d_cwork = d_misc + 96;
+  int32_t* const d_cres = d_misc + 48;
+  {
+    const int32_t init4[4] = {0, INF, 0, 0};
+    memcpy(h_cnt + 4, init4, sizeof init4);
+    BS_HIP(ctx, hipMemcpyAsync(d_cwork, h_cnt + 4, sizeof init4, hipMemcpyHostToDevice, st));
+  }
+  int live_cur = 0;
+  int32_t nlive = -1;
+  bool scan_launched = false;
+  const int live_sub = 4;
+  auto enqueue_scan = [&](int32_t Fs, bool speculative) {
+    gc.cand_scans++;
+    scan_launched = nlive != 0;
+    if (nlive < 0) {
+      gc.cand_groups_scanned += (int64_t)nb256;
+      cand_flag_kernel<<<(int)((nb256 + cand_sub - 1) / cand_sub), 256, 0, st>>>(rec, quads, K, n, Fs, prio, ps, 0, omega, nullptr, cand_raw,
+                                                                                nullptr, bcand, cand_sub, d_cwork, d_cres,
+                                                                                live_list[live_cur ^ 1]);
+    } else if (nlive > 0) {
+      gc.cand_groups_scanned += nlive;
+      cand_list_kernel<<<(nlive + live_sub - 1) / live_sub, 256, 0, st>>>(rec, quads, K, n, Fs, prio, ps, omega, cand_raw, bcand, live_sub,
+                                                                          live_list[live_cur], nlive, live_list[live_cur ^ 1],
+                                                                          speculative ? 1 : 0, d_cwork, d_cres);
+    }
+  };
+  int32_t scan_ncand = 0, scan_min = INF;
+  auto accept_scan = [&]() {
+    if (scan_launched) {
+      scan_ncand = h_flags[48];
+      scan_min = h_flags[49];
+      nlive = h_flags[50];
+      live_cur ^= 1;
+    } else {
+      scan_ncand = 0;
+      scan_min = INF;
+    }
+  };
+  const bool speculate = !dbg;
+  const bool verify_env = getenv("BS_VERIFY") != nullptr;
   for (;;) {
     rounds++;
     gc.rounds = rounds;
     a.F = F;
     const int npend = (int)pending.size();
     if (!cand_listed) {
-      BS_HIP(ctx, hipMemsetAsync(d_misc + 1, 0, sizeof(int32_t), st));
-      cand_flag_kernel<<<(int)((nb256 + cand_sub - 1) / cand_sub), 256, 0, st>>>(rec, quads, K, n, F, prio, ps, 0, omega, nullptr, cand_raw, d_misc + 1, bcand, cand_sub);
-      BS_HIP(ctx, hipMemcpyAsync(h_flags + 11, d_misc + 1, sizeof(int32_t), hipMemcpyDeviceToHost, st));
-      BS_HIP(ctx, hipStreamSynchronize(st));
-      ncand_all = h_flags[11];
+      enqueue_scan(F, false);
+      BS_HIP(ctx, hipMemcpyAsync(h_flags + 48, d_cres, 3 * sizeof(int32_t), hipMemcpyDeviceToHost, st));
+      BS_HIP(ctx, sync_main());
+      accept_scan();
+      ncand_all = scan_ncand;
     }
     cand_listed = false;
     if (ncand_all == 0 && npend == 0)
@@ -2569,8 +2746,10 @@
     const int ncand = std::min<int>(ncand_all, max_waves);
     gc.rounds_capped += ncand_all > max_waves ? 1 : 0;
     gc.rounds_big += ncand >= 4096 ? 1 : 0;
-    if (npend)
-      BS_HIP(ctx, hipMemcpyAsync(d_pend, pending.data(), sizeof(PlaneOut) * npend, hipMemcpyHostToDevice, st));
+    if (npend) {
+      memcpy(h_pend, pending.data(), sizeof(PlaneOut) * npend);
+      BS_HIP(ctx, hipMemcpyAsync(d_pend, h_pend, sizeof(PlaneOut) * npend, hipMemcpyHostToDevice, st));
+    }
     if (ncand > 0) {
       if (full_refresh) {
         refresh_records_kernel<<<nblk(n, 256), 256, 0, st>>>(omega, rec, quads, n);
@@ -2589,7 +2768,6 @@
         BS_HIP(ctx, hipMemsetAsync(dead, 0, sizeof(int32_t) * n, st));
         dead_dirty = false;
       }
-      BS_HIP(ctx, hipMemsetAsync(d_pool_top, 0, sizeof(unsigned long long), st));
       const uint32_t* d_order = nullptr;
       if (dispatch_order && ncand >= 4096) {
         BS_HIP(ctx, hipMemsetAsync(tmin1, 0xff, sizeof(unsigned long long) * (nt1 + nt2), st));
@@ -2611,8 +2789,9 @@
         forge_kernel<<<1, 64, 0, st>>>(d_out, ncand, pool.base, forge_mode, d_misc + 5);
         forge_mode = 0;
       }
-      validate1_kernel<<<ncand, VT, 0, st>>>(d_out, ncand, pool.base, rec, quads, dead, n, vmark,
-                                             (int32_t)((rounds & 0x3ff) << 20), d_misc + 4);
+      plane_round_kernel<<<ncand, VT, 0, st>>>(d_out, ncand, pool.base, rec, quads, K, dead, n, vmark, (int32_t)((rounds & 0x3ff) << 20),
+                                               d_misc + 4, base, ps, dcur, bcur, omega, occ);
+      wl_marked = true;
       if (do_validate3) {
         BS_HIP(ctx, hipEventRecord(ctx->sev[0], st));
         BS_HIP(ctx, hipStreamWaitEvent(ctx->side, ctx->sev[0], 0));
@@ -2620,45 +2799,74 @@
         BS_HIP(ctx, hipEventRecord(ctx->sev[1], ctx->side));
         v3_pending = true;
       }
-      reset_tags_kernel<<<ncand, VT, 0, st>>>(d_out, ncand, pool.base, rec, quads, K);
-      reset_dead_kernel<<<nblk(ncand, 256), 256, 0, st>>>(d_cand, ncand, dead);
-      plane_apply_kernel<<<ncand, VT, 0, st>>>(d_out, ncand, pool.base, base, ps, dcur, bcur, omega, occ, rec, quads);
-      wl_marked = true;
-      rc = propagate();
-      if (rc != BS_OK)
-        return rc;
-      validate2_kernel<<<ncand, VT, 0, st>>>(d_out, ncand, pool.base, omega, rec, quads, K);
-    }
-    if (npend)
-      validate2_kernel<<<npend, VT, 0, st>>>(d_pend, npend, pstore, omega, rec, quads, K);
-    const int32_t init2[2] = {0, INF};
-    BS_HIP(ctx, hipMemcpyAsync(d_misc + 1, init2, sizeof init2, hipMemcpyHostToDevice, st));
-    cand_flag_kernel<<<(int)((nb256 + cand_sub - 1) / cand_sub), 256, 0, st>>>(rec, quads, K, n, F, prio, ps, 0, omega, d_misc + 2, cand_raw, d_misc + 1, bcand, cand_sub);
-    BS_HIP(ctx, hipMemcpyAsync(h_flags + 8, d_misc + 1, 2 * sizeof(int32_t), hipMemcpyDeviceToHost, st));
-    if (v3_pending) {
-      BS_HIP(ctx, hipStreamWaitEvent(st, ctx->sev[1], 0));
-      v3_pending = false;
-    }
-    BS_HIP(ctx, hipMemcpyAsync(h_flags + 10, d_misc + 4, sizeof(int32_t), hipMemcpyDeviceToHost, st));
+      reset_dead_kernel<<<nblk(ncand, 256), 256, 0, st>>>(d_cand, ncand, dead, d_pool_top);
+    }
     const bool compact = ncand >= 4096 && !dbg;
     int nh = ncand;
     PlaneOut* d_outh = d_out;
+    auto enqueue_tail = [&](bool speculative) -> int {
+      if (ncand > 0)
+        validate2_kernel<<<ncand, VT, 0, st>>>(d_out, ncand, pool.base, omega, rec, quads, K);
+      if (npend)
+        validate2_kernel<<<npend, VT, 0, st>>>(d_pend, npend, pstore, omega, rec, quads, K);
+      enqueue_scan(F, speculative);
+      if (v3_pending) {
+        BS_HIP(ctx, hipStreamWaitEvent(st, ctx->sev[1], 0));
+        v3_pending = false;
+      }
+      BS_HIP(ctx, hipMemcpyAsync(h_flags + 10, d_misc + 4, sizeof(int32_t), hipMemcpyDeviceToHost, st));
+      if (compact) {
+        size_t tb = 0;
+        BS_HIP(ctx, hipcub::DeviceSelect::If(nullptr, tb, d_out, d_outc, d_misc + 51, ncand, KeepForHost(), st));
+        BS_HIP(ctx, ctx->cub_tmp.reserve(tb));
+        BS_HIP(ctx, hipcub::DeviceSelect::If(ctx->cub_tmp.p, tb, d_out, d_outc, d_misc + 51, ncand, KeepForHost(), st));
+      } else if (ncand > 0) {
+        BS_HIP(ctx, hipMemcpyAsync(h_out, d_out, sizeof(PlaneOut) * ncand, hipMemcpyDeviceToHost, st));
+      }
+      if (npend)
+        BS_HIP(ctx, hipMemcpyAsync(h_pend, d_pend, sizeof(PlaneOut) * npend, hipMemcpyDeviceToHost, st));
+      BS_HIP(ctx, hipMemcpyAsync(h_flags + 32, d_misc + 32, 20 * sizeof(int32_t), hipMemcpyDeviceToHost, st));
+      return BS_OK;
+    };
+    bool tail_done = false;
+    if (ncand > 0) {
+      gc.owner_settles++;
+      if (speculate) {
+        rc = launch_group();
+        if (rc != BS_OK)
+          return rc;
+        rc = enqueue_tail(true);
+        if (rc != BS_OK)
+          return rc;
+        BS_HIP(ctx, sync_main());
+        tail_done = h_flip[own_group - 1] == 0;
+        if (!tail_done)
+          gc.tails_redone++;
+        else if (verify_env && (rc = verify_fixpoint()) != BS_OK)
+          return rc;
+      }
+      if (!tail_done) {
+        rc = propagate();
+        if (rc != BS_OK)
+          return rc;
+      }
+    }
+    if (!tail_done) {
+      rc = enqueue_tail(false);
+      if (rc != BS_OK)
+        return rc;
+      BS_HIP(ctx, sync_main());
+    }
+    accept_scan();
     if (compact) {
-      size_t tb = 0;
-      BS_HIP(ctx, hipcub::DeviceSelect::If(nullptr, tb, d_out, d_outc, d_misc + 20, ncand, KeepForHost(), st));
-      BS_HIP(ctx, ctx->cub_tmp.reserve(tb));
-      BS_HIP(ctx, hipcub::DeviceSelect::If(ctx->cub_tmp.p, tb, d_out, d_outc, d_misc + 20, ncand, KeepForHost(), st));
-      BS_HIP(ctx, hipMemcpyAsync(h_flags + 14, d_misc + 20, sizeof(int32_t), hipMemcpyDeviceToHost, st));
-      BS_HIP(ctx, hipStreamSynchronize(st));
-      nh = h_flags[14];
+      nh = h_flags[51];
       d_outh = d_outc;
-    }
-    if (nh)
-      BS_HIP(ctx, hipMemcpyAsync(h_out, d_outh, sizeof(PlaneOut) * nh, hipMemcpyDeviceToHost, st));
-    if (npend)
-      BS_HIP(ctx, hipMemcpyAsync(h_pend, d_pend, sizeof(PlaneOut) * npend, hipMemcpyDeviceToHost, st));
-    BS_HIP(ctx, hipStreamSynchronize(st));
-    const int32_t next_ncand_all = h_flags[8], new_min = h_flags[9], rejects_now = h_flags[10];
+      if (nh) {
+        BS_HIP(ctx, hipMemcpyAsync(h_out, d_outh, sizeof(PlaneOut) * nh, hipMemcpyDeviceToHost, st));
+        BS_HIP(ctx, sync_main());
+      }
+    }
+    const int32_t next_ncand_all = scan_ncand, new_min = scan_min, rejects_now = h_flags[10];
     if (timed_round) {
       float ms = 0.f;
       if (hipEventElapsedTime(&ms, ctx->ev[6], ctx->ev[7]) == hipSuccess)
@@ -2842,24 +3050,6 @@
     rc = flush_copies();
     if (rc != BS_OK)
       return rc;
-    if (dropped) {
-      if (nh) {
-        BS_HIP(ctx, hipMemcpyAsync(d_outh, h_out, sizeof(PlaneOut) * nh, hipMemcpyHostToDevice, st));
-        plane_apply_kernel<<<nh, VT, 0, st>>>(d_outh, nh, pool.base, base, ps, dcur, bcur, omega, occ, rec, quads);
-        wl_marked = true;
-      }
-      if (npend) {
-        BS_HIP(ctx, hipMemcpyAsync(d_pend, h_pend, sizeof(PlaneOut) * npend, hipMemcpyHostToDevice, st));
-        plane_apply_kernel<<<npend, VT, 0, st>>>(d_pend, npend, pstore, base, ps, dcur, bcur, omega, occ, rec, quads);
-        wl_marked = true;
-      }
-      rc = propagate();
-      if (rc != BS_OK)
-        return rc;
-    } else {
-      cand_listed = true;
-      ncand_all = next_ncand_all;
-    }
     pending.swap(next_pending);
     if (pending.empty())
       pstore_top = 0;
@@ -2874,6 +3064,46 @@
     F = first_bad;
     if (rounds > 4 * n + 16)
       return fail(ctx, BS_ERR_INTERNAL, "region grow (speculative): round limit");
+    cand_listed = true;
+    if (dropped) {
+      if (nh) {
+        BS_HIP(ctx, hipMemcpyAsync(d_outh, h_out, sizeof(PlaneOut) * nh, hipMemcpyHostToDevice, st));
+        plane_apply_kernel<<<nh, VT, 0, st>>>(d_outh, nh, pool.base, base, ps, dcur, bcur, omega, occ, rec, quads);
+        wl_marked = true;
+      }
+      if (npend) {
+        BS_HIP(ctx, hipMemcpyAsync(d_pend, h_pend, sizeof(PlaneOut) * npend, hipMemcpyHostToDevice, st));
+        plane_apply_kernel<<<npend, VT, 0, st>>>(d_pend, npend, pstore, base, ps, dcur, bcur, omega, occ, rec, quads);
+        wl_marked = true;
+      }
+      bool scan_done = false;
+      gc.owner_settles++;
+      if (speculate) {
+        rc = launch_group();
+        if (rc != BS_OK)
+          return rc;
+        enqueue_scan(F, true);
+        BS_HIP(ctx, hipMemcpyAsync(h_flags + 32, d_misc + 32, 20 * sizeof(int32_t), hipMemcpyDeviceToHost, st));
+        BS_HIP(ctx, sync_main());
+        scan_done = h_flip[own_group - 1] == 0;
+        if (!scan_done)
+          gc.tails_redone++;
+        else if (verify_env && (rc = verify_fixpoint()) != BS_OK)
+          return rc;
+      }
+      if (!scan_done) {
+        rc = propagate();
+        if (rc != BS_OK)
+          return rc;
+        enqueue_scan(F, false);
+        BS_HIP(ctx, hipMemcpyAsync(h_flags + 32, d_misc + 32, 20 * sizeof(int32_t), hipMemcpyDeviceToHost, st));
+        BS_HIP(ctx, sync_main());
+      }
+      accept_scan();
+      ncand_all = scan_ncand;
+    } else {
+      ncand_all = next_ncand_all;
+    }
   }
   int32_t* owner_final = omega;
   const int np = (int)recs.size();
@@ -2891,8 +3121,9 @@
   hs.seed_attempts = attempts;
   hs.largest = largest;
   hs.steps = passes;
+  gc.owner_passes = passes;
   BS_HIP(ctx, hipMemcpyAsync(ctx->rg_stats.p, &hs, sizeof hs, hipMemcpyHostToDevice, st));
-  BS_HIP(ctx, hipStreamSynchronize(st));
+  BS_HIP(ctx, sync_main());
   BS_HIP(ctx, hipGetLastError());
   ctx->rg_n = n;
   ctx->rg_valid = true;
@@ -2929,7 +3160,7 @@
     BS_HIP(ctx, hipMemsetAsync(d_misc + 1, 0, sizeof(int32_t), st));
     BS_HIP(ctx, hipMemsetAsync(d_misc + 8, 0, 2 * sizeof(int32_t), st));
     cand_flag_kernel<<<(int)((nb256 + cand_sub - 1) / cand_sub), 256, 0, st>>>(rec, quads, K, n, 0, prio, ps, 1, omega, nullptr,
-                                                                              cand_raw, d_misc + 1, bcand, cand_sub);
+                                                                              cand_raw, d_misc + 1, bcand, cand_sub, nullptr, nullptr, nullptr);
     BS_HIP(ctx, hipMemcpyAsync(h_flags + 11, d_misc + 1, sizeof(int32_t), hipMemcpyDeviceToHost, st));
     BS_HIP(ctx, hipStreamSynchronize(st));
     const int na = h_flags[11];
@@ -2976,11 +3207,11 @@
           const int cnt = (int)std::min<size_t>(pend.size() - off, (size_t)wave_cap);
           BS_HIP(ctx, hipMemcpyAsync(d_cand, pend.data() + off, sizeof(unsigned long long) * cnt, hipMemcpyHostToDevice, st));
           BS_HIP(ctx, hipMemsetAsync(d_pool_top, 0, sizeof(unsigned long long), st));
-          reset_dead_kernel<<<nblk(cnt, 256), 256, 0, st>>>(d_cand, cnt, dead);
+          reset_dead_kernel<<<nblk(cnt, 256), 256, 0, st>>>(d_cand, cnt, dead, nullptr);
           grow_n(0, cnt, d_out);
           compare_n(cnt, d_retry);
           reset_tags_kernel<<<cnt, VT, 0, st>>>(d_out, cnt, pool.base, rec, quads, K);
-          reset_dead_kernel<<<nblk(cnt, 256), 256, 0, st>>>(d_cand, cnt, dead);
+          reset_dead_kernel<<<nblk(cnt, 256), 256, 0, st>>>(d_cand, cnt, dead, nullptr);
           h_retry.resize((size_t)cnt);
           BS_HIP(ctx, hipMemcpyAsync(h_retry.data(), d_retry, sizeof(int32_t) * cnt, hipMemcpyDeviceToHost, st));
           BS_HIP(ctx, hipStreamSynchronize(st));
diff --git a/include/bs_api.h b/include/bs_api.h
--- a/include/bs_api.h
+++ b/include/bs_api.h
@@ -155,6 +155,12 @@
   int64_t dropped_other;
   int64_t full_refreshes;
   int64_t pool_cap;
+  int64_t host_syncs;
+  int64_t tails_redone;
+  int64_t cand_groups_scanned;
+  int64_t cand_scans;
+  int64_t owner_passes;
+  int64_t owner_settles;
 } bs_grow_counters;
 int bs_get_grow_counters(const bs_ctx* ctx, bs_grow_counters* out);
 
```

Result: slower. 194.2 Mpoints/s (-3.2%).
